# stemangiola/ppcseq

Hardware: AMD Instinct MI355X
Metric: effective samples/sec (whole node) for NB hierarchical fit (higher is better)
Workload: dtype f64; 1 GPU; BASELINE cfg3: synthetic 20000 genes x 200 samples (seed 20253), C=2, K=1000; NUTS (Stan defaults) warm-up 150 + 250 kept draws/chain, 8 chains per GPU (cfg3 names 8 chains; chains are the sharded unit, so N GPUs run 8N chains); mode=chains, chains_total=8, lanes_per_gene=4, loglik_workgroups=939, ess_estimator=rank-normalised split-chain bulk-ESS, min over 6 hyper-parameters and lp__, grad_evals=1471121, divergent_after_warmup=0, round_structure=pipelined: merged log-likelihood / state-machine launch + gene kernel, stream_groups=library default (3 from eight chains on, 2 from four), rounds_last_step_all_groups=115040

## Files before the change

### ppcseq_amd/_lib.py

```python
from __future__ import annotations

import ctypes as C
import os
from dataclasses import dataclass

import numpy as np

_HERE = os.path.dirname(os.path.abspath(__file__))
LIB_PATH = os.environ.get("PPCX_LIB", os.path.join(_HERE, "libppcx.so"))

EXPORTS = [
    "ppcx_version", "ppcx_device_count", "ppcx_last_error", "ppcx_model_create", "ppcx_model_set_exclusions",
    "ppcx_model_set_launch", "ppcx_model_get_launch", "ppcx_model_get_plan", "ppcx_model_dim", "ppcx_model_destroy", "ppcx_log_prob_grad",
    "ppcx_nuts_config_default", "ppcx_fit_nuts", "ppcx_fit_info", "ppcx_fit_from_draws", "ppcx_fit_get_draws", "ppcx_fit_get_columns",
    "ppcx_fit_get_diagnostics", "ppcx_fit_get_timing", "ppcx_fit_get_kernel_times", "ppcx_fit_ppc", "ppcx_fit_free", "ppcx_do_inference_C", "ppcx_model_set_rounds", "ppcx_model_get_rounds", "ppcx_model_set_progress",
    "ppcx_model_create_shard", "ppcx_model_create_shard_strided", "ppcx_fit_nuts_shards", "ppcx_comm_unique_id", "ppcx_comm_create", "ppcx_comm_destroy",
    "ppcx_fit_nuts_comm", "ppcx_advi_config_default", "ppcx_fit_advi", "ppcx_fit_advi_info", "ppcx_fit_advi_iterative",
    "ppcx_guard_decision", "ppcx_device_memory", "ppcx_fit_get_ppc_timing",
    "ppcx_xchg_create", "ppcx_xchg_handle", "ppcx_xchg_connect", "ppcx_xchg_connect_local", "ppcx_xchg_set_timeout", "ppcx_xchg_destroy",
    "ppcx_fit_nuts_xchg", "ppcx_fit_get_xchg_timing", "ppcx_fit_get_inv_metric", "ppcx_fit_summary",
    "ppcx_fit_get_approximation", "ppcx_fit_get_log_ratios", "ppcx_fit_psis", "ppcx_fit_get_log_lik", "ppcx_fit_loo",
    "ppcx_fit_loo_predict", "ppcx_fit_relative_eff", "ppcx_fit_loo_mcse", "ppcx_fit_loo_approx", "ppcx_fit_loo_predict_approx",
]
ABI_VERSION = 400
SUMMARY_FIELDS = ("mean", "sd", "q05", "q50", "q95", "rhat", "ess_bulk", "ess_tail")
LOO_FIELDS = ("elpd_loo", "p_loo", "looic", "khat")
LOO_MCSE_FIELDS = LOO_FIELDS + ("mcse_elpd_loo", "n_eff")
LOO_PREDICT_FIELDS = ("mean", "lower", "upper", "pit_lt", "pit_le", "khat")


class PpcxError(RuntimeError):
    pass


class NutsConfig(C.Structure):
    _fields_ = [("chains", C.c_int), ("iter", C.c_int), ("warmup", C.c_int), ("seed", C.c_ulonglong),
                ("adapt_delta", C.c_double), ("max_treedepth", C.c_int), ("init_radius", C.c_double),
                ("stepsize0", C.c_double), ("init_buffer", C.c_int), ("term_buffer", C.c_int), ("window", C.c_int),
                ("chain_id_offset", C.c_int)]


class AdviConfig(C.Structure):
    _fields_ = [("output_samples", C.c_int), ("iter", C.c_int), ("tol_rel_obj", C.c_double), ("grad_samples", C.c_int),
                ("elbo_samples", C.c_int), ("eval_elbo", C.c_int), ("adapt_iter", C.c_int), ("seed", C.c_ulonglong),
                ("init_radius", C.c_double)]


PROGRESS_FN = C.CFUNCTYPE(C.c_int, C.c_void_p, C.c_int, C.c_int, C.c_int, C.c_longlong, C.c_double)
_lib = None


def use_library(path=None):
    global _lib, LIB_PATH
    _lib = None
    LIB_PATH = path if path else os.environ.get("PPCX_LIB", os.path.join(_HERE, "libppcx.so"))


def load() -> C.CDLL:
    global _lib
    if _lib is not None:
        return _lib
    if not os.path.exists(LIB_PATH):
        raise PpcxError(f"{LIB_PATH} not found: run `python -m ppcseq_amd.build` (hipcc, gfx950) first; "
                        "there is no CPU fallback")
    lib = C.CDLL(LIB_PATH)
    lib.ppcx_version.restype = C.c_int
    if lib.ppcx_version() != ABI_VERSION:
        raise PpcxError(f"{LIB_PATH} has ABI version {lib.ppcx_version()}, this binding needs {ABI_VERSION}: rebuild it "
                        "(`python -m ppcseq_amd.build --force`)")
    dp, ip = C.POINTER(C.c_double), C.POINTER(C.c_int32)
    lib.ppcx_guard_decision.argtypes = [dp, C.c_int]
    lib.ppcx_device_memory.argtypes = [C.c_int, C.POINTER(C.c_ulonglong), C.POINTER(C.c_ulonglong)]
    lib.ppcx_fit_get_ppc_timing.argtypes = [C.c_void_p, dp, C.POINTER(C.c_longlong)]
    lib.ppcx_last_error.restype = C.c_char_p
    lib.ppcx_model_create.argtypes = [C.c_int] * 5 + [ip, dp, dp, C.c_double, C.c_int, ip, C.POINTER(C.c_void_p)]
    lib.ppcx_model_set_exclusions.argtypes = [C.c_void_p, C.c_int, ip]
    lib.ppcx_model_set_launch.argtypes = [C.c_void_p, C.c_int, C.c_int]
    lib.ppcx_model_get_launch.argtypes = [C.c_void_p, C.POINTER(C.c_int), C.POINTER(C.c_int)]
    lib.ppcx_model_get_plan.argtypes = [C.c_void_p, C.c_int, C.POINTER(C.c_int), C.POINTER(C.c_int), C.POINTER(C.c_int32), C.c_int]
    lib.ppcx_model_dim.argtypes = [C.c_void_p]
    lib.ppcx_model_destroy.argtypes = [C.c_void_p]
    lib.ppcx_model_destroy.restype = None
    lib.ppcx_log_prob_grad.argtypes = [C.c_void_p, C.c_int, dp, dp, dp]
    lib.ppcx_nuts_config_default.argtypes = [C.POINTER(NutsConfig)]
    lib.ppcx_nuts_config_default.restype = None
    lib.ppcx_fit_nuts.argtypes = [C.c_void_p, C.POINTER(NutsConfig), C.POINTER(C.c_void_p)]
    lib.ppcx_fit_info.argtypes = [C.c_void_p] + [C.POINTER(C.c_int)] * 4
    lib.ppcx_fit_from_draws.argtypes = [C.c_void_p, C.c_int, C.c_int, dp, C.POINTER(C.c_void_p)]
    lib.ppcx_fit_get_draws.argtypes = [C.c_void_p, dp]
    lib.ppcx_fit_get_columns.argtypes = [C.c_void_p, C.c_int, ip, dp]
    lib.ppcx_fit_summary.argtypes = [C.c_void_p, C.c_int, ip, dp]
    lib.ppcx_fit_get_approximation.argtypes = [C.c_void_p, dp, dp]
    lib.ppcx_fit_get_log_ratios.argtypes = [C.c_void_p, dp, dp]
    lib.ppcx_fit_psis.argtypes = [C.c_void_p, C.c_int, ip, dp]
    lib.ppcx_fit_get_log_lik.argtypes = [C.c_void_p, C.c_int, ip, dp]
    lib.ppcx_fit_loo.argtypes = [C.c_void_p, C.c_int, ip, dp, dp]
    lib.ppcx_fit_loo_mcse.argtypes = [C.c_void_p, C.c_int, ip, dp, dp]
    lib.ppcx_fit_loo_predict.argtypes = [C.c_void_p, C.c_int, ip, dp, C.c_double, C.c_double, C.c_double, C.c_ulonglong, dp]
    lib.ppcx_fit_relative_eff.argtypes = [C.c_void_p, C.c_int, ip, dp]
    lib.ppcx_fit_loo_approx.argtypes = [C.c_void_p, C.c_int, ip, dp]
    lib.ppcx_fit_loo_predict_approx.argtypes = [C.c_void_p, C.c_int, ip, C.c_double, C.c_double, C.c_double, C.c_ulonglong, dp]
    lib.ppcx_fit_get_diagnostics.argtypes = [C.c_void_p, dp, dp, ip, ip, ip, dp]
    lib.ppcx_fit_get_timing.argtypes = [C.c_void_p, dp, C.POINTER(C.c_longlong), dp, C.POINTER(C.c_longlong), dp]
    lib.ppcx_fit_get_kernel_times.argtypes = [C.c_void_p, dp, dp, dp, C.POINTER(C.c_longlong)]
    lib.ppcx_fit_get_inv_metric.argtypes = [C.c_void_p, dp]
    lib.ppcx_fit_ppc.argtypes = [C.c_void_p, C.c_double, C.c_double, C.c_double, C.c_ulonglong, C.c_int, C.c_int, dp, ip]
    lib.ppcx_fit_free.argtypes = [C.c_void_p]
    lib.ppcx_model_set_rounds.argtypes = [C.c_void_p, C.c_int, C.c_int]
    lib.ppcx_xchg_create.argtypes = [C.c_int, C.c_int, C.c_int, C.c_int, C.POINTER(C.c_void_p)]
    lib.ppcx_xchg_handle.argtypes = [C.c_void_p, C.c_char_p]
    lib.ppcx_xchg_connect.argtypes = [C.c_void_p, C.c_char_p]
    lib.ppcx_xchg_connect_local.argtypes = [C.POINTER(C.c_void_p), C.c_int]
    lib.ppcx_xchg_set_timeout.argtypes = [C.c_void_p, C.c_double]
    lib.ppcx_xchg_destroy.argtypes = [C.c_void_p]
    lib.ppcx_xchg_destroy.restype = None
    lib.ppcx_fit_nuts_xchg.argtypes = [C.c_void_p, C.POINTER(NutsConfig), C.c_void_p, C.POINTER(C.c_void_p)]
    lib.ppcx_fit_get_xchg_timing.argtypes = [C.c_void_p, dp, C.POINTER(C.c_longlong)]
    lib.ppcx_model_get_rounds.argtypes = [C.c_void_p, C.c_int, C.POINTER(C.c_int), C.POINTER(C.c_int)]
    lib.ppcx_model_set_progress.argtypes = [C.c_void_p, PROGRESS_FN, C.c_void_p, C.c_double]
    if hasattr(lib, "ppcx_testing_set"):
        lib.ppcx_testing_set.argtypes = [C.c_char_p, C.c_longlong]
        lib.ppcx_testing_set_nccl_provider.argtypes = [C.c_char_p]
        lib.ppcx_testing_bench_kernel.argtypes = [C.c_void_p, C.c_int, C.c_int, C.c_int, C.c_int, C.c_int, dp, C.POINTER(C.c_int)]
    if hasattr(lib, "ppcx_testing_eval_math"):
        lib.ppcx_testing_eval_math.argtypes = [C.c_int, C.c_int, dp, dp, ip, dp, dp]
    if hasattr(lib, "ppcx_testing_get_disp_table"):
        lib.ppcx_testing_get_disp_table.argtypes = [C.c_void_p, dp]
    if hasattr(lib, "ppcx_testing_psis"):
        lib.ppcx_testing_psis.argtypes = [C.c_int, C.c_int, dp, dp, dp]
    if hasattr(lib, "ppcx_testing_loo"):
        lib.ppcx_testing_loo.argtypes = [C.c_int, C.c_int, dp, ip, dp, dp]
    if hasattr(lib, "ppcx_testing_loo_mcse"):
        lib.ppcx_testing_loo_mcse.argtypes = [C.c_int, C.c_int, dp, ip, dp, dp]
    if hasattr(lib, "ppcx_testing_loo_predict"):
        lib.ppcx_testing_loo_predict.argtypes = [dp, ip, C.c_int, C.c_int, ip, ip, dp, C.c_double, C.c_double, dp]
    if hasattr(lib, "ppcx_testing_loo_approx"):
        lib.ppcx_testing_loo_approx.argtypes = [C.c_int, C.c_int, dp, dp, ip, dp]
        lib.ppcx_testing_loo_predict_approx.argtypes = [dp, dp, ip, C.c_int, C.c_int, ip, ip, C.c_double, C.c_double, dp]
    if hasattr(lib, "ppcx_testing_relative_eff"):
        lib.ppcx_testing_relative_eff.argtypes = [C.c_int, C.c_int, C.c_int, dp, dp]
    lib.ppcx_fit_free.restype = None
    lib.ppcx_advi_config_default.argtypes = [C.POINTER(AdviConfig)]
    lib.ppcx_advi_config_default.restype = None
    lib.ppcx_fit_advi.argtypes = [C.c_void_p, C.POINTER(AdviConfig), C.POINTER(C.c_void_p)]
    lib.ppcx_fit_advi_iterative.argtypes = [C.c_void_p, C.POINTER(AdviConfig), C.c_int, C.POINTER(C.c_void_p)]
    lib.ppcx_fit_advi_info.argtypes = [C.c_void_p, C.POINTER(C.c_int), C.POINTER(C.c_int), C.POINTER(C.c_double), C.POINTER(C.c_double)]
    lib.ppcx_model_create_shard.argtypes = [C.c_int] * 7 + [ip, dp, dp, C.c_double, C.c_int, ip, C.POINTER(C.c_void_p)]
    lib.ppcx_model_create_shard_strided.argtypes = [C.c_int] * 8 + [ip, dp, dp, C.c_double, C.c_int, ip, C.POINTER(C.c_void_p)]
    lib.ppcx_fit_nuts_shards.argtypes = [C.POINTER(C.c_void_p), C.c_int, C.POINTER(NutsConfig), C.POINTER(C.c_void_p)]
    lib.ppcx_comm_unique_id.argtypes = [C.c_char_p]
    lib.ppcx_comm_create.argtypes = [C.c_int, C.c_int, C.c_int, C.c_char_p, C.POINTER(C.c_void_p)]
    lib.ppcx_comm_destroy.argtypes = [C.c_void_p]
    lib.ppcx_comm_destroy.restype = None
    lib.ppcx_fit_nuts_comm.argtypes = [C.c_void_p, C.POINTER(NutsConfig), C.c_void_p, C.POINTER(C.c_void_p)]
    _lib = lib
    return lib


def _check(rc: int):
    if rc != 0:
        raise PpcxError(f"ppcx error {rc}: {load().ppcx_last_error().decode()}")


def _p(a, t):
    return a.ctypes.data_as(C.POINTER(t)) if a is not None else None


def testing_set(key: str, value: int):
    lib = load()
    if not hasattr(lib, "ppcx_testing_set"):
        raise PpcxError(f"{LIB_PATH} is not the testing build")
    _check(lib.ppcx_testing_set(key.encode(), int(value)))


def testing_set_nccl_provider(path: str):
    lib = load()
    if not hasattr(lib, "ppcx_testing_set_nccl_provider"):
        raise PpcxError(f"{LIB_PATH} is not the testing build")
    _check(lib.ppcx_testing_set_nccl_provider(path.encode() if path else None))


TESTING_MATH = ("fast_rcp", "fast_log", "fast_exp", "table_log", "window_log", "stirling_tails", "stirling_excess",
                "log_erfc_ratio", "cell", "cell_win", "cell_y", "cell_win_y")


def testing_eval_math(fn: str, a, b=None, y=None):
    lib = load()
    if not hasattr(lib, "ppcx_testing_eval_math"):
        raise PpcxError(f"{LIB_PATH} is not the testing build, or one built before ppcx_testing_math.hip existed: rebuild it "
                        "(`python -m ppcseq_amd.build --testing --force`)")
    a = np.ascontiguousarray(a, dtype=np.float64).ravel()
    n = a.size
    b = np.ascontiguousarray(np.zeros(n) if b is None else np.broadcast_to(b, (n,)), dtype=np.float64)
    y = np.ascontiguousarray(np.zeros(n) if y is None else np.broadcast_to(y, (n,)), dtype=np.int32)
    o0, o1 = np.zeros(n), np.zeros(n)
    rc = lib.ppcx_testing_eval_math(TESTING_MATH.index(fn), n, _p(a, C.c_double), _p(b, C.c_double), _p(y, C.c_int32),
                                    _p(o0, C.c_double), _p(o1, C.c_double))
    if rc != 0:
        raise PpcxError(f"ppcx_testing_eval_math({fn}) failed with code {rc}")
    return o0, o1


def testing_psis(lr, cols=None):
    lib = load()
    if not hasattr(lib, "ppcx_testing_psis"):
        raise PpcxError(f"{LIB_PATH} is not the testing build, or one built before ppcx_testing_psis existed: rebuild it "
                        "(`python -m ppcseq_amd.build --testing --force`)")
    lr = np.ascontiguousarray(lr, dtype=np.float64).ravel()
    n = lr.size
    cols = np.zeros((n, 0)) if cols is None else np.ascontiguousarray(cols, dtype=np.float64).reshape(n, -1)
    out = np.zeros(cols.shape[1] + 1)
    _check(lib.ppcx_testing_psis(n, int(cols.shape[1]), _p(lr, C.c_double), _p(cols, C.c_double) if cols.size else None,
                                 _p(out, C.c_double)))
    return out


def testing_loo(ll, excluded=None, r_eff=None):
    return _testing_loo("ppcx_testing_loo", LOO_FIELDS, ll, excluded, r_eff)


def testing_loo_mcse(ll, excluded=None, r_eff=None):
    return _testing_loo("ppcx_testing_loo_mcse", LOO_MCSE_FIELDS, ll, excluded, r_eff)


def _testing_loo(entry, fields, ll, excluded, r_eff):
    lib = load()
    if not hasattr(lib, entry):
        raise PpcxError(f"{LIB_PATH} is not the testing build, or one built before {entry} existed: rebuild it "
                        "(`python -m ppcseq_amd.build --testing --force`)")
    ll = np.asarray(ll, dtype=np.float64)
    ll = ll.reshape(ll.shape[0], -1)
    n, nc = ll.shape
    cols = np.ascontiguousarray(ll.T)
    ex = None if excluded is None else np.ascontiguousarray(excluded, dtype=np.int32).ravel()
    re = None if r_eff is None else np.ascontiguousarray(r_eff, dtype=np.float64).ravel()
    out = np.zeros((nc, len(fields)))
    _check(getattr(lib, entry)(n, nc, _p(cols, C.c_double), _p(ex, C.c_int32) if ex is not None else None,
                               _p(re, C.c_double) if re is not None else None, _p(out, C.c_double)))
    return out


def testing_loo_predict(ll, x, y, excluded=None, r_eff=None, p_lo=0.025, p_hi=0.975):
    lib = load()
    if not hasattr(lib, "ppcx_testing_loo_predict"):
        raise PpcxError(f"{LIB_PATH} is not the testing build, or one built before ppcx_testing_loo_predict existed: rebuild it "
                        "(`python -m ppcseq_amd.build --testing --force`)")
    ll = np.asarray(ll, dtype=np.float64)
    ll = ll.reshape(ll.shape[0], -1)
    n, nc = ll.shape
    cols = np.ascontiguousarray(ll.T)
    xs = np.ascontiguousarray(np.asarray(x).reshape(n, nc).T, dtype=np.int32)
    ys = np.ascontiguousarray(np.broadcast_to(np.asarray(y), (nc,)), dtype=np.int32)
    ex = None if excluded is None else np.ascontiguousarray(excluded, dtype=np.int32).ravel()
    re = None if r_eff is None else np.ascontiguousarray(r_eff, dtype=np.float64).ravel()
    out = np.zeros((nc, len(LOO_PREDICT_FIELDS)))
    _check(lib.ppcx_testing_loo_predict(_p(cols, C.c_double), _p(xs, C.c_int32), n, nc, _p(ys, C.c_int32),
                                        _p(ex, C.c_int32) if ex is not None else None,
                                        _p(re, C.c_double) if re is not None else None, float(p_lo), float(p_hi),
                                        _p(out, C.c_double)))
    return out


def _testing_approx_columns(entry, ll, log_ratio, excluded):
    lib = load()
    if not hasattr(lib, entry):
        raise PpcxError(f"{LIB_PATH} is not the testing build, or one built before {entry} existed: rebuild it "
                        "(`python -m ppcseq_amd.build --testing --force`)")
    ll = np.asarray(ll, dtype=np.float64)
    ll = ll.reshape(ll.shape[0], -1)
    lr = np.ascontiguousarray(log_ratio, dtype=np.float64).ravel()
    if lr.size != ll.shape[0]:
        raise ValueError("log_ratio must hold one value per draw")
    ex = None if excluded is None else np.ascontiguousarray(excluded, dtype=np.int32).ravel()
    return lib, np.ascontiguousarray(ll.T), lr, ex


def testing_loo_approx(ll, log_ratio, excluded=None):
    lib, cols, lr, ex = _testing_approx_columns("ppcx_testing_loo_approx", ll, log_ratio, excluded)
    nc, n = cols.shape
    out = np.zeros((nc, len(LOO_FIELDS)))
    _check(lib.ppcx_testing_loo_approx(n, nc, _p(cols, C.c_double), _p(lr, C.c_double),
                                       _p(ex, C.c_int32) if ex is not None else None, _p(out, C.c_double)))
    return out


def testing_loo_predict_approx(ll, log_ratio, x, y, excluded=None, p_lo=0.025, p_hi=0.975):
    lib, cols, lr, ex = _testing_approx_columns("ppcx_testing_loo_predict_approx", ll, log_ratio, excluded)
    nc, n = cols.shape
    xs = np.ascontiguousarray(np.asarray(x).reshape(n, nc).T, dtype=np.int32)
    ys = np.ascontiguousarray(np.broadcast_to(np.asarray(y), (nc,)), dtype=np.int32)
    out = np.zeros((nc, len(LOO_PREDICT_FIELDS)))
    _check(lib.ppcx_testing_loo_predict_approx(_p(cols, C.c_double), _p(lr, C.c_double), _p(xs, C.c_int32), n, nc, _p(ys, C.c_int32),
                                               _p(ex, C.c_int32) if ex is not None else None, float(p_lo), float(p_hi),
                                               _p(out, C.c_double)))
    return out


def testing_relative_eff(ll, chains):
    lib = load()
    if not hasattr(lib, "ppcx_testing_relative_eff"):
        raise PpcxError(f"{LIB_PATH} is not the testing build, or one built before ppcx_testing_relative_eff existed: rebuild it "
                        "(`python -m ppcseq_amd.build --testing --force`)")
    ll = np.asarray(ll, dtype=np.float64)
    ll = ll.reshape(ll.shape[0], -1)
    rows, nc = ll.shape
    chains = int(chains)
    if chains < 1 or rows % chains:
        raise ValueError("ll must hold chains * n rows")
    cols = np.ascontiguousarray(ll.T)
    out = np.zeros(nc)
    _check(lib.ppcx_testing_relative_eff(chains, rows // chains, nc, _p(cols, C.c_double), _p(out, C.c_double)))
    return out


def loo_estimates(pointwise, excluded):
    keep = ~np.asarray(excluded, bool)
    out = {}
    for name in LOO_FIELDS[:3]:
        v = np.asarray(pointwise[name], dtype=np.float64)[keep]
        se = float(np.sqrt(v.size * np.var(v, ddof=1))) if v.size > 1 else float("nan")
        out[name] = (float(np.sum(v)), se)
    return out


def device_count() -> int:
    return int(load().ppcx_device_count())


def device_memory(device=0):
    f, t = C.c_ulonglong(), C.c_ulonglong()
    _check(load().ppcx_device_memory(int(device), C.byref(f), C.byref(t)))
    return int(f.value), int(t.value)


def shard_genes(G_total, g0, stride):
    return list(range(int(g0), int(G_total), int(stride)))


class Model:

    def __init__(self, counts, X, exposure_rate, K, lambda_mu_mu=5.612671, excl=None, device=0, shard=None):
        lib = load()
        counts = np.ascontiguousarray(counts, dtype=np.int32)
        if counts.ndim != 2:
            raise ValueError("counts must be G x S")
        self.G, self.S = counts.shape
        X = np.asfortranarray(np.asarray(X, dtype=np.float64).reshape(self.S, -1))
        self.C = X.shape[1]
        self.K = int(K)
        exposure_rate = np.ascontiguousarray(exposure_rate, dtype=np.float64)
        if exposure_rate.shape != (self.S,):
            raise ValueError("exposure_rate must have length S")
        excl = np.ascontiguousarray(excl if excl is not None else np.zeros(0), dtype=np.int32)
        self.X, self.exposure_rate = X, exposure_rate
        self.excl = excl.copy()
        self.counts = counts
        h = C.c_void_p()
        self.shard = shard
        if shard is None:
            _check(lib.ppcx_model_create(int(device), self.G, self.S, self.C, self.K, _p(counts, C.c_int32),
                                         _p(X, C.c_double), _p(exposure_rate, C.c_double), float(lambda_mu_mu),
                                         int(excl.size), _p(excl, C.c_int32), C.byref(h)))
        else:
            if len(shard) == 5:
                Gt, Kt, g0, stride = int(shard[0]), int(shard[1]), int(shard[2]), int(shard[4])
                if len(shard_genes(Gt, g0, stride)) != self.G:
                    raise ValueError("counts must hold exactly the genes of the shard")
                self.K = len([g for g in shard_genes(Gt, g0, stride) if g < Kt])
                _check(lib.ppcx_model_create_shard_strided(int(device), Gt, self.S, self.C, Kt, g0, stride, self.G, _p(counts, C.c_int32),
                                                           _p(X, C.c_double), _p(exposure_rate, C.c_double), float(lambda_mu_mu),
                                                           int(excl.size), _p(excl, C.c_int32), C.byref(h)))
            else:
                Gt, Kt, g0, g1 = (int(v) for v in shard)
                if g1 - g0 != self.G:
                    raise ValueError("counts must hold exactly the genes of the shard")
                self.K = max(0, min(g1, Kt) - min(g0, Kt))
                _check(lib.ppcx_model_create_shard(int(device), Gt, self.S, self.C, Kt, g0, g1, _p(counts, C.c_int32),
                                                   _p(X, C.c_double), _p(exposure_rate, C.c_double), float(lambda_mu_mu),
                                                   int(excl.size), _p(excl, C.c_int32), C.byref(h)))
        self._h = h
        self.D = int(lib.ppcx_model_dim(h))

    def set_exclusions(self, excl):
        excl = np.ascontiguousarray(excl if excl is not None else np.zeros(0), dtype=np.int32)
        _check(load().ppcx_model_set_exclusions(self._h, int(excl.size), _p(excl, C.c_int32)))
        self.excl = excl.copy()

    def set_launch(self, lanes_per_gene=0, workgroups=0):
        _check(load().ppcx_model_set_launch(self._h, int(lanes_per_gene), int(workgroups)))

    def get_plan(self, nchains):
        lanes, nb = C.c_int(), C.c_int()
        _check(load().ppcx_model_get_plan(self._h, int(nchains), C.byref(lanes), C.byref(nb), None, 0))
        b = np.zeros(4 * nb.value + 1, np.int32)
        _check(load().ppcx_model_get_plan(self._h, int(nchains), C.byref(lanes), C.byref(nb), _p(b, C.c_int32), int(b.size)))
        return lanes.value, nb.value, b

    def get_launch(self):
        a, b = C.c_int(), C.c_int()
        _check(load().ppcx_model_get_launch(self._h, C.byref(a), C.byref(b)))
        return a.value, b.value

    def testing_disp_table(self):
        lib = load()
        if not hasattr(lib, "ppcx_testing_get_disp_table"):
            raise PpcxError(f"{LIB_PATH} is not the testing build, or one built before ppcx_testing_get_disp_table existed: "
                            "rebuild it (`python -m ppcseq_amd.build --testing --force`)")
        out = np.zeros((self.G, 32, 2, 12))
        _check(lib.ppcx_testing_get_disp_table(self._h, _p(out, C.c_double)))
        return out

    def log_prob_grad(self, u):
        u = np.ascontiguousarray(u, dtype=np.float64)
        one = u.ndim == 1
        u2 = u.reshape(-1, self.D)
        lp = np.zeros(u2.shape[0])
        g = np.zeros_like(u2)
        _check(load().ppcx_log_prob_grad(self._h, u2.shape[0], _p(u2, C.c_double), _p(lp, C.c_double), _p(g, C.c_double)))
        return (float(lp[0]), g[0]) if one else (lp, g)

    def fit_nuts(self, chains=3, iter=300, warmup=150, seed=1, adapt_delta=0.8, max_treedepth=10, init_radius=2.0,
                 stepsize0=1.0, init_buffer=75, term_buffer=50, window=25, chain_id_offset=0) -> "Fit":
        cfg = NutsConfig(chains, iter, warmup, seed, adapt_delta, max_treedepth, init_radius, stepsize0,
                         init_buffer, term_buffer, window, chain_id_offset)
        h = C.c_void_p()
        _check(load().ppcx_fit_nuts(self._h, C.byref(cfg), C.byref(h)))
        return Fit(self, h)

    def fit_advi(self, output_samples=1000, iter=50000, tol_rel_obj=0.005, elbo_samples=100, eval_elbo=100, adapt_iter=50,
                 seed=1, init_radius=2.0, max_attempts=1) -> "Fit":
        cfg = AdviConfig(output_samples, iter, tol_rel_obj, 1, elbo_samples, eval_elbo, adapt_iter, seed, init_radius)
        h = C.c_void_p()
        if max_attempts > 1:
            _check(load().ppcx_fit_advi_iterative(self._h, C.byref(cfg), int(max_attempts), C.byref(h)))
        else:
            _check(load().ppcx_fit_advi(self._h, C.byref(cfg), C.byref(h)))
        return Fit(self, h)

    def fit_from_draws(self, draws) -> "Fit":
        draws = np.ascontiguousarray(draws, dtype=np.float64)
        if draws.ndim != 3 or draws.shape[2] != self.D:
            raise ValueError("draws must be [chains, n_keep, D]")
        h = C.c_void_p()
        _check(load().ppcx_fit_from_draws(self._h, draws.shape[0], draws.shape[1], _p(draws, C.c_double), C.byref(h)))
        return Fit(self, h)

    def fit_nuts_comm(self, comm: "Comm", **kw) -> "Fit":
        cfg = _make_cfg(**kw)
        h = C.c_void_p()
        _check(load().ppcx_fit_nuts_comm(self._h, C.byref(cfg), comm._h, C.byref(h)))
        return Fit(self, h)

    def fit_nuts_xchg(self, xchg: "Xchg", **kw) -> "Fit":
        cfg = _make_cfg(**kw)
        h = C.c_void_p()
        _check(load().ppcx_fit_nuts_xchg(self._h, C.byref(cfg), xchg._h, C.byref(h)))
        return Fit(self, h)

    def set_rounds(self, pipelined=-2, stream_groups=-1):
        _check(load().ppcx_model_set_rounds(self._h, int(pipelined), int(stream_groups)))

    def set_progress(self, fn=None, every_seconds=1.0):
        self._progress_cb = PROGRESS_FN((lambda user, c0, n, done, rounds, sec: 1 if fn(c0, n, done, rounds, sec) else 0) if fn else 0)
        _check(load().ppcx_model_set_progress(self._h, self._progress_cb, None, float(every_seconds)))

    def get_rounds(self, nchains=1):
        a, b = C.c_int(), C.c_int()
        _check(load().ppcx_model_get_rounds(self._h, int(nchains), C.byref(a), C.byref(b)))
        return bool(a.value), b.value

    def bench_kernel(self, which=0, nchains=1, warm_rounds=40, reps=50, n_merge=1):
        lib = load()
        if not hasattr(lib, "ppcx_testing_bench_kernel"):
            raise PpcxError(f"{LIB_PATH} is not the testing build")
        ms, t = C.c_double(), C.c_int()
        _check(lib.ppcx_testing_bench_kernel(self._h, int(which), nchains, warm_rounds, reps, n_merge, C.byref(ms), C.byref(t)))
        return ms.value, t.value

    def close(self):
        if getattr(self, "_h", None):
            load().ppcx_model_destroy(self._h)
            self._h = None

    def __del__(self):
        try:
            self.close()
        except Exception:
            pass


def _make_cfg(chains=3, iter=300, warmup=150, seed=1, adapt_delta=0.8, max_treedepth=10, init_radius=2.0,
              stepsize0=1.0, init_buffer=75, term_buffer=50, window=25, chain_id_offset=0):
    return NutsConfig(chains, iter, warmup, seed, adapt_delta, max_treedepth, init_radius, stepsize0,
                      init_buffer, term_buffer, window, chain_id_offset)


def fit_nuts_shards(models, **kw):
    cfg = _make_cfg(**kw)
    n = len(models)
    hm = (C.c_void_p * n)(*[m._h for m in models])
    hf = (C.c_void_p * n)()
    _check(load().ppcx_fit_nuts_shards(hm, n, C.byref(cfg), hf))
    return [Fit(m, C.c_void_p(h)) for m, h in zip(models, hf)]


class Comm:

    @staticmethod
    def unique_id() -> bytes:
        buf = C.create_string_buffer(128)
        _check(load().ppcx_comm_unique_id(buf))
        return buf.raw

    def __init__(self, nranks, rank, unique_id: bytes, device=0):
        h = C.c_void_p()
        _check(load().ppcx_comm_create(int(device), int(nranks), int(rank), unique_id, C.byref(h)))
        self._h = h

    def close(self):
        if getattr(self, "_h", None):
            load().ppcx_comm_destroy(self._h)
            self._h = None


class Xchg:

    def __init__(self, nranks, rank, max_chains, device=0):
        h = C.c_void_p()
        _check(load().ppcx_xchg_create(int(device), int(nranks), int(rank), int(max_chains), C.byref(h)))
        self._h, self.nranks, self.rank = h, int(nranks), int(rank)

    def handle(self) -> bytes:
        buf = C.create_string_buffer(64)
        _check(load().ppcx_xchg_handle(self._h, buf))
        return buf.raw

    def connect(self, handles):
        blob = b"".join(handles)
        if len(blob) != 64 * self.nranks:
            raise ValueError("need one 64-byte handle per rank")
        _check(load().ppcx_xchg_connect(self._h, blob))

    @staticmethod
    def local_group(n, max_chains, devices=None):
        xs = [Xchg(n, k, max_chains, device=(devices[k] if devices else 0)) for k in range(n)]
        arr = (C.c_void_p * n)(*[x._h for x in xs])
        _check(load().ppcx_xchg_connect_local(arr, n))
        return xs

    def set_timeout(self, seconds):
        _check(load().ppcx_xchg_set_timeout(self._h, float(seconds)))

    def close(self):
        if getattr(self, "_h", None):
            load().ppcx_xchg_destroy(self._h)
            self._h = None


@dataclass
class Timing:
    seconds: float
    grad_evals: int
    gene_kernel_ms_mean: float
    gene_kernel_samples: int
# ... 201 lines not shown
```

### ppcseq_amd/build.py

```python
from __future__ import annotations

import os
import subprocess
import sys

HERE = os.path.dirname(os.path.abspath(__file__))
CSRC = os.path.join(HERE, "csrc")
LIB = os.path.join(HERE, "libppcx.so")
TESTING_LIB = os.path.join(os.path.dirname(HERE), "tests", "libppcx_testing.so")
SOURCES = ["ppcx_kernels.hip", "ppcx_summary.hip", "ppcx_psis.hip", "ppcx_loo.hip", "ppcx_loo_predict.hip", "ppcx_reff.hip", "ppcx_capi.hip"]
TESTING_SOURCES = ["ppcx_testing_math.hip"]
HEADERS = ["ppcx_math.h", "ppcx_disp.h", "ppcx_model.h", "ppcx_nuts.h", "ppcx_gene.h", "ppcx_kernels.h", "ppcx_summary.h", "ppcx_summary_dev.h", "ppcx_psis.h", "ppcx_psis_dev.h", "ppcx_loo.h", "ppcx_loo_ap.h", "ppcx_loo_dev.h", "ppcx_loo_predict.h", "ppcx_reff.h", "ppcx_block.h", "ppcx_columns.h", "ppcx_testing.h",
           os.path.join("..", "..", "include", "ppcx.h")]


CODEGEN_FLAGS = ["-fno-slp-vectorize"]


def _sources(extra):
    return SOURCES + (TESTING_SOURCES if "-DPPCX_TESTING" in extra else [])


def _stale(lib: str, extra=()) -> bool:
    if not os.path.exists(lib):
        return True
    t = os.path.getmtime(lib)
    return any(os.path.getmtime(os.path.join(CSRC, f)) > t for f in _sources(extra) + HEADERS)


def _compile(lib: str, extra, verbose: bool) -> None:
    hipcc = os.environ.get("HIPCC", "/opt/rocm/bin/hipcc")
    objs = []
    procs = []
    for s in _sources(extra):
        o = lib + "." + s + ".o"
        objs.append(o)
        cmd = [hipcc, "-O3", "-std=c++17", "--offload-arch=gfx950", "-fPIC", "-fvisibility=hidden", "-Wno-unused-result"] + CODEGEN_FLAGS + extra + \
              ["-c", "-o", o, os.path.join(CSRC, s)]
        if verbose:
            print(" ".join(cmd), file=sys.stderr)
        procs.append(subprocess.Popen(cmd))
    for p in procs:
        if p.wait() != 0:
            raise subprocess.CalledProcessError(p.returncode, p.args)
    subprocess.check_call([hipcc, "--offload-arch=gfx950", "-shared", "-fPIC", "-o", lib] + objs)
    for o in objs:
        os.remove(o)


def build(force: bool = False, verbose: bool = False) -> str:
    if force or _stale(LIB):
        _compile(LIB, [], verbose)
    return LIB


def build_testing(force: bool = False, verbose: bool = False) -> str:
    if force or _stale(TESTING_LIB, ["-DPPCX_TESTING"]):
        _compile(TESTING_LIB, ["-DPPCX_TESTING"], verbose)
    return TESTING_LIB


def build_all(force: bool = False, verbose: bool = False):
    import threading
    jobs = []
    if force or _stale(LIB):
        jobs.append((LIB, []))
    if force or _stale(TESTING_LIB, ["-DPPCX_TESTING"]):
        jobs.append((TESTING_LIB, ["-DPPCX_TESTING"]))
    errs = []

    def run(lib, extra):
        try:
            _compile(lib, extra, verbose)
        except Exception as e:
            errs.append(e)
    th = [threading.Thread(target=run, args=j) for j in jobs]
    for t in th:
        t.start()
    for t in th:
        t.join()
    if errs:
        raise errs[0]
    return LIB, TESTING_LIB


if __name__ == "__main__":
    if "--testing" in sys.argv:
        print(*build_all(force="--force" in sys.argv, verbose=True))
    else:
        print(build(force="--force" in sys.argv, verbose=True))
```

### ppcseq_amd/csrc/ppcx_capi.hip

```cpp
#include <hip/hip_runtime.h>
#include <math.h>
#include <stdio.h>
#include <string.h>
#include <algorithm>
#include <chrono>
#include <dlfcn.h>
#include <map>
#include <mutex>
#include <stdlib.h>
#include <string>
#include <thread>
#include <atomic>
#include <vector>
#include "../../include/ppcx.h"
#include "ppcx_kernels.h"
#include "ppcx_summary.h"
#include "ppcx_psis.h"
#include "ppcx_loo.h"
#include "ppcx_columns.h"

using namespace ppcx;

static thread_local std::string g_err;
static int fail(int code, const std::string& msg) { g_err = msg; return code; }
static int hip_fail(hipError_t e, const char* what) { return fail(PPCX_ERR_HIP, std::string(what) + ": " + hipGetErrorString(e)); }
#define HIPCHK(expr)                                                                       \
  do {                                                                                     \
    hipError_t e_ = (expr);                                                                \
    if (e_ != hipSuccess) return hip_fail(e_, #expr);                                      \
  } while (0)

#ifdef PPCX_TESTING
#include "ppcx_testing.h"
struct TestHooks {
  long long fail_at_round = 0; int fail_rank = -1;
  int force_generic = 0;
  int slope_cost_permille = 0;
  int trim_slack_permille = -1;
  int trim_extra_passes = 0;
  int psis_slots = 0;
  long long psis_scratch_bytes = 0;
  long long loo_scratch_bytes = 0;
  std::string rccl_lib;
};
static TestHooks g_test;
#endif

#ifdef PPCX_TRACE
static unsigned long long* g_trace_dev = nullptr;
#endif
struct ppcx_model {
  int device;
  Dims d;
  int CM, L = 64;
  int L_override = 0, wgs_override = 0;
  int n_cu = 256, wgs_per_cu = 4;
  int ls_wgs_per_cu = 0;
  int nblocks_chosen = 0;
  int opt_pipelined = -1, opt_stream_groups = 0;
  ppcx_progress_fn progress = nullptr; void* progress_user = nullptr; double progress_every = 1.0;
  std::vector<char> pos_slope;
  struct Plan { int nbpc = 0; int* d_bounds = nullptr; };
  std::map<std::pair<int, int>, Plan> plans;
  std::mutex plan_mutex;
  std::vector<int32_t> counts_host;
  std::vector<char> excluded_host;
  std::vector<double> X_host, expo_host;
  int* d_counts = nullptr;
  double *d_E = nullptr, *d_expo = nullptr, *d_X = nullptr, *d_Sy = nullptr, *d_SyE = nullptr, *d_SyX = nullptr, *d_SX = nullptr, *d_ncell = nullptr, *d_Lg1 = nullptr;
  double* d_disp = nullptr;
  unsigned char* d_gflags = nullptr;
  DispFit fit;
  double *d_logtab = nullptr, *d_wintab = nullptr;
  double e_min = 1.0, e_max = 1.0;
  int* d_order = nullptr;
  hipStream_t stream = nullptr;
  int live_fits = 0;
  bool destroy_requested = false;
};

struct ppcx_fit {
  ppcx_model* m;
  NutsConfig cfg;
  int chains, n_keep, iter;
  DeviceBuffer<double> d_draws;
  DeviceBuffer<double> d_lp, d_stepsize, d_accept;
  DeviceBuffer<int> d_treedepth, d_nleap, d_div;
  double seconds = 0; long long grad_evals = 0;
  double kA_ms_mean = 0; long long kA_samples = 0; double kA_chain_launches_mean = 0;
  double kC_ms_mean = 0, kU_ms_mean = 0; long long launch_triples = 0;
  double advi_elbo = 0, advi_eta = 0; int advi_converged = 0;
  double ppc_ms = 0; long long ppc_draws = 0;
  long long xchg_ticks = 0, xchg_count = 0;
  std::vector<double> inv_metric;
  bool advi = false;
  DeviceBuffer<double> d_mu, d_omega;
  DeviceBuffer<double> d_log_p, d_log_g, d_r;
};

extern "C" int ppcx_version(void) { return PPCX_VERSION; }
extern "C" int ppcx_device_count(void) { int n = 0; if (hipGetDeviceCount(&n) != hipSuccess) return 0; return n; }
extern "C" const char* ppcx_last_error(void) { return g_err.c_str(); }
extern "C" int ppcx_device_memory(int device, unsigned long long* free_bytes, unsigned long long* total_bytes) {
  int ndev = 0;
  HIPCHK(hipGetDeviceCount(&ndev));
  if (device < 0 || device >= ndev) return fail(PPCX_ERR_ARG, "no such HIP device");
  HIPCHK(hipSetDevice(device));
  size_t f = 0, t = 0;
  HIPCHK(hipMemGetInfo(&f, &t));
  if (free_bytes) *free_bytes = (unsigned long long)f;
  if (total_bytes) *total_bytes = (unsigned long long)t;
  return PPCX_OK;
}

static double pass_cost(const ppcx_model* m, int L, int p, int n) {
  const int S = m->d.S;
  bool slope = false;
  for (int i = p; i < p + n; ++i) slope = slope || m->pos_slope[i];
  double slope_w = m->d.C > 2 ? 1.0 : 1.15;
#ifdef PPCX_TESTING
  if (g_test.slope_cost_permille > 0) slope_w = 1e-3 * g_test.slope_cost_permille;
#endif
  double lin_w = 2.5;
#ifdef PPCX_TESTING
  if (g_test.slope_cost_permille > 0) lin_w = 1e-3 * g_test.slope_cost_permille;
#endif
  const double sweep = (double)((S + L - 1) / L) * (!m->d.x0_is_one ? 2.5 : (slope && !m->d.x1_binary ? lin_w : (slope ? slope_w : 1.0)));
  return 5.8 + sweep;
}
static int resident_workgroups(const ppcx_model* m, int reserve) {
  int n = m->wgs_override > 0 ? m->wgs_override : m->n_cu * (reserve > 0 ? m->ls_wgs_per_cu : m->wgs_per_cu);
  n -= reserve;
  return n < 1 ? 1 : n;
}
constexpr double kTrimSlack = 0.0;
static int workgroups_per_chain(const ppcx_model* m, int L, int nch, int n_res, bool whole_runs = true, bool trim = false) {
  int nbpc = n_res / (nch < 1 ? 1 : nch);
  if (nbpc >= 8 && whole_runs) nbpc = nbpc / 8 * 8;
  if (nbpc < 1) nbpc = 1;
  const int gpw = 64 / L, npass = (m->d.G + gpw - 1) / gpw;
  if (nbpc > (npass + 3) / 4) nbpc = (npass + 3) / 4;
  if (trim) {
    double slack = kTrimSlack;
#ifdef PPCX_TESTING
    if (g_test.trim_slack_permille >= 0) slack = 1e-3 * g_test.trim_slack_permille;
#endif
    int maxp = (npass + 4 * nbpc - 1) / (4 * nbpc);
#ifdef PPCX_TESTING
    maxp += g_test.trim_extra_passes;
#endif
    int nb2 = (int)ceil((double)npass * (1.0 + slack) / (4.0 * maxp));
    if (nb2 >= 8 && whole_runs) nb2 = (nb2 + 7) / 8 * 8;
    if (nb2 < nbpc) nbpc = nb2;
  }
  return nbpc;
}
static int default_stream_groups(int nch) { return nch >= 8 ? 3 : (nch >= 4 ? 2 : 1); }
static int fit_launch_chains(const ppcx_model* m, int nch) {
  int g = default_stream_groups(nch);
  if (m->opt_stream_groups >= 1) g = m->opt_stream_groups < nch ? m->opt_stream_groups : nch;
  return (nch + g - 1) / g;
}
static void choose_launch(ppcx_model* m, int nchains) {
  const int G = m->d.G, S = m->d.S;
  int bestL = 64; double best = 1e300;
  for (int L = 64; L >= 1; L >>= 1) {
    const int gpw = 64 / L;
    const double npass = ceil((double)G / gpw), c_pass = (8.0 + (double)((S + L - 1) / L)) * (L <= 2 ? 1.2 : 1.0);
    const int wpc = 4 * workgroups_per_chain(m, L, nchains, resident_workgroups(m, 0));
    const double t = ceil(npass / wpc) * c_pass;
    if (t < best) { best = t; bestL = L; }
  }
  const int L = m->L_override > 0 ? m->L_override : bestL;
  if (L != m->L) {
    std::lock_guard<std::mutex> lk(m->plan_mutex);
    for (auto& kv : m->plans) (void)hipFree(kv.second.d_bounds);
    m->plans.clear();
    m->L = L;
  }
  m->nblocks_chosen = workgroups_per_chain(m, m->L, nchains, resident_workgroups(m, 0)) * nchains;
}
static void drop_plans(ppcx_model* m) {
  std::lock_guard<std::mutex> lk(m->plan_mutex);
  for (auto& kv : m->plans) (void)hipFree(kv.second.d_bounds);
  m->plans.clear();
}
static int plan_launch(ppcx_model* m, int nch, int reserve, ppcx_model::Plan* out, bool trim = false) {
  std::lock_guard<std::mutex> lk(m->plan_mutex);
  const int n_res = resident_workgroups(m, reserve);
  const auto key = std::make_pair(nch, trim ? -n_res : n_res);
  auto it = m->plans.find(key);
  if (it != m->plans.end()) { *out = it->second; return PPCX_OK; }
  const int G = m->d.G, L = m->L, gpw = 64 / L;
  const int nbpc = workgroups_per_chain(m, L, nch, n_res, reserve == 0, trim), wpc = 4 * nbpc, npass = (G + gpw - 1) / gpw;
  std::vector<double> cost(npass);
  double total = 0;
  for (int k = 0; k < npass; ++k) {
    const int p = k * gpw;
    cost[k] = pass_cost(m, L, p, G - p < gpw ? G - p : gpw);
    total += cost[k];
  }
  std::vector<int> bounds(wpc + 1, G);
  bounds[0] = 0;
  {
    int k = 0; double cum = 0.0;
    for (int j = 1; j < wpc; ++j) {
      const double target = total * (double)j / (double)wpc;
      while (k < npass && cum + 0.5 * cost[k] < target) cum += cost[k++];
      bounds[j] = k * gpw < G ? k * gpw : G;
    }
  }
  {
    const long pmax = ((long)(npass + wpc - 1) / wpc) * gpw;
    for (int j = 0; j < wpc; ++j) if (bounds[j + 1] - bounds[j] > pmax) bounds[j + 1] = (int)(bounds[j] + pmax);
    bounds[wpc] = G;
    for (int j = wpc - 1; j >= 0; --j) if (bounds[j + 1] - bounds[j] > pmax) bounds[j] = (int)(bounds[j + 1] - pmax);
  }
  ppcx_model::Plan pl; pl.nbpc = nbpc;
  HIPCHK(hipMalloc(&pl.d_bounds, sizeof(int) * (size_t)(wpc + 1)));
  HIPCHK(hipMemcpy(pl.d_bounds, bounds.data(), sizeof(int) * (size_t)(wpc + 1), hipMemcpyHostToDevice));
  m->plans[key] = pl;
  *out = pl;
  return PPCX_OK;
}

static int upload_counts(ppcx_model* m, int n_excl, const int32_t* excl) {
  const int G = m->d.G, S = m->d.S, C = m->d.C;
  std::vector<int32_t> cnt(m->counts_host);
  for (int e = 0; e < n_excl; ++e) {
    if (excl[e] < 0 || excl[e] >= G * S) return fail(PPCX_ERR_ARG, "excluded cell id out of range");
    cnt[excl[e]] = -1;
  }
  std::vector<double> Sy(G, 0.0), SyE(G, 0.0), SyX((size_t)C * G, 0.0), SX((size_t)C * G, 0.0), ncell(G, 0.0), Lg1(G, 0.0);
  std::vector<unsigned char> gflags(G, 0);
  for (int g = 0; g < G; ++g) {
    double sy = 0, sye = 0, nc = 0, lg1 = 0;
    for (int s = 0; s < S; ++s) {
      const int y = cnt[(size_t)g * S + s];
      if (y < 0) { gflags[g] |= 1; continue; }
      sy += y; sye += (double)y * m->expo_host[s]; nc += 1.0; lg1 += lgamma((double)y + 1.0);
      for (int c = 0; c < C; ++c) { SyX[(size_t)c * G + g] += (double)y * m->X_host[(size_t)c * S + s]; SX[(size_t)c * G + g] += m->X_host[(size_t)c * S + s]; }
    }
    Sy[g] = sy; SyE[g] = sye; ncell[g] = nc; Lg1[g] = lg1;
  }
  HIPCHK(hipMemcpy(m->d_gflags, gflags.data(), (size_t)G, hipMemcpyHostToDevice));
  {
    std::vector<int> ord(G);
    for (int g = 0; g < G; ++g) ord[g] = g;
    const int K = m->d.K;
    std::stable_sort(ord.begin(), ord.end(), [&](int a, int b) {
      const bool sa = a < K && C >= 2, sb = b < K && C >= 2;
      if (sa != sb) return sa;
      return gflags[a] > gflags[b];
    });
    {
      int ns = 0;
      while (ns < G && ord[ns] < K && C >= 2) ++ns;
      constexpr int kOrderBlock = 16;
      const int nbs = (ns + kOrderBlock - 1) / kOrderBlock, nb = (G + kOrderBlock - 1) / kOrderBlock;
      const bool dear_slopes = m->d.x0_is_one && !m->d.x1_binary;
      if (ns > 0 && ns < G && nbs < nb && dear_slopes) {
        std::vector<int> mixed; mixed.reserve(G);
        int is = 0, ip = ns, sb = 0;
        for (int b = 0; b < nb; ++b) {
          const bool slope_block = sb < nbs && b == (int)((long long)sb * nb / nbs);
          if (slope_block && is < ns) { for (int k = 0; k < kOrderBlock && is < ns; ++k) mixed.push_back(ord[is++]); ++sb; }
          else { for (int k = 0; k < kOrderBlock && ip < G; ++k) mixed.push_back(ord[ip++]); }
        }
        while (is < ns) mixed.push_back(ord[is++]);
        while (ip < G) mixed.push_back(ord[ip++]);
        ord.swap(mixed);
      }
    }
    HIPCHK(hipMemcpy(m->d_order, ord.data(), sizeof(int) * (size_t)G, hipMemcpyHostToDevice));
    m->pos_slope.resize(G);
    for (int p = 0; p < G; ++p) m->pos_slope[p] = ord[p] < K && C >= 2;
    drop_plans(m);
  }
  HIPCHK(hipMemcpy(m->d_counts, cnt.data(), sizeof(int32_t) * cnt.size(), hipMemcpyHostToDevice));
  m->excluded_host.assign(cnt.size(), 0);
  for (size_t i = 0; i < cnt.size(); ++i) m->excluded_host[i] = cnt[i] < 0;
  {
    const hipError_t e = launch_disp_build_kernel(m->d_counts, G, S, nullptr, G, m->fit, m->d_disp, m->stream);
    if (e != hipSuccess) return fail(PPCX_ERR_HIP, std::string("dispersion-table kernel: ") + hipGetErrorString(e));
  }
  HIPCHK(hipMemcpy(m->d_Sy, Sy.data(), sizeof(double) * G, hipMemcpyHostToDevice));
  HIPCHK(hipMemcpy(m->d_SyE, SyE.data(), sizeof(double) * G, hipMemcpyHostToDevice));
  HIPCHK(hipMemcpy(m->d_SyX, SyX.data(), sizeof(double) * SyX.size(), hipMemcpyHostToDevice));
  HIPCHK(hipMemcpy(m->d_SX, SX.data(), sizeof(double) * SX.size(), hipMemcpyHostToDevice));
  HIPCHK(hipMemcpy(m->d_ncell, ncell.data(), sizeof(double) * G, hipMemcpyHostToDevice));
  HIPCHK(hipMemcpy(m->d_Lg1, Lg1.data(), sizeof(double) * G, hipMemcpyHostToDevice));
  HIPCHK(hipStreamSynchronize(m->stream));
  return PPCX_OK;
}

extern "C" int ppcx_model_create(int device, int G, int S, int C, int K, const int32_t* counts, const double* X,
                                 const double* exposure, double lambda_mu_mu, int n_excl, const int32_t* excl,
                                 ppcx_model** out) {
  if (!out) return fail(PPCX_ERR_ARG, "out is NULL");
  *out = nullptr;
  if (G < 1 || S < 1 || C < 1 || K < 0 || K > G) return fail(PPCX_ERR_ARG, "need G>=1, S>=1, C>=1, 0<=K<=G");
  if (C > kMaxC) return fail(PPCX_ERR_LIMIT, "C exceeds the 16 design columns this build supports");
  if ((long long)G * S > 2000000000LL) return fail(PPCX_ERR_LIMIT, "G*S exceeds int32 cell ids");
  if (!counts || !X || !exposure || (n_excl > 0 && !excl)) return fail(PPCX_ERR_ARG, "NULL input buffer");
  for (long long i = 0; i < (long long)G * S; ++i) if (counts[i] < 0) return fail(PPCX_ERR_ARG, "negative count");
  int ndev = 0;
  HIPCHK(hipGetDeviceCount(&ndev));
  if (device < 0 || device >= ndev) return fail(PPCX_ERR_ARG, "no such HIP device");
  HIPCHK(hipSetDevice(device));
  ppcx_model* m = new ppcx_model();
  m->device = device;
  m->d = make_dims(G, S, C, K, lambda_mu_mu);
  m->CM = C <= 2 ? 2 : (C <= 4 ? 4 : (C <= 8 ? 8 : 16));
  {
    hipDeviceProp_t prop;
    HIPCHK(hipGetDeviceProperties(&prop, device));
    m->n_cu = prop.multiProcessorCount > 0 ? prop.multiProcessorCount : 256;
  }
  m->counts_host.assign(counts, counts + (size_t)G * S);
  m->X_host.assign(X, X + (size_t)S * C);
  m->expo_host.assign(exposure, exposure + S);
  int x0 = 1;
  for (int s = 0; s < S; ++s) if (X[s] != 1.0) x0 = 0;
  m->d.x0_is_one = x0;
  int x1b = (C >= 2);
  for (size_t i = (size_t)S; i < (size_t)S * C && x1b; ++i) if (X[i] != 0.0 && X[i] != 1.0) x1b = 0;
#ifdef PPCX_TESTING
  if (g_test.force_generic) x1b = 0;
#endif
  m->d.x1_binary = x1b;
  m->d.raw_consts = (!x0 || (C >= 2 && K > 0 && !x1b)) ? 1 : 0;
  if (C > 8 && (!x0 || (K > 0 && !x1b))) {
    delete m;
    return fail(PPCX_ERR_LIMIT, "more than 8 design columns are supported for designs of a column of ones and 0 / 1 indicator columns only");
  }
  if (const char* e = getenv("PPCX_PIPELINE")) if (atoi(e) == 0) m->opt_pipelined = 0;
  if (const char* e = getenv("PPCX_STREAM_GROUPS")) { const int v = atoi(e); if (v >= 1) m->opt_stream_groups = v; }
  if (loglik_lds_bytes(m->d) > 160u * 1024u) {
    delete m;
    return fail(PPCX_ERR_LIMIT, "the per-sample constants (S * C doubles; S * (2 + C) for a design without a column of ones) do not fit the 160 KB of LDS of a compute unit beside the 20 KB of tables");
  }
  m->wgs_per_cu = loglik_resident_workgroups_per_cu(m->CM, m->d);
  if (m->wgs_per_cu < 1) { delete m; return fail(PPCX_ERR_LIMIT, "the log-likelihood kernel cannot be resident with S * (2 + C) doubles of per-sample constants in LDS"); }
  m->ls_wgs_per_cu = ls_resident_workgroups_per_cu(m->CM, m->d);
  std::vector<double> E(S);
  for (int s = 0; s < S; ++s) E[s] = exp(exposure[s]);
#define MCHK(expr) do { int rc_ = (expr); if (rc_ != PPCX_OK) { ppcx_model_destroy(m); return rc_; } } while (0)
#define MHIP(expr) do { hipError_t e_ = (expr); if (e_ != hipSuccess) { ppcx_model_destroy(m); return fail(PPCX_ERR_HIP, std::string(#expr) + ": " + hipGetErrorString(e_)); } } while (0)
  MHIP(hipStreamCreateWithFlags(&m->stream, hipStreamNonBlocking));
  MHIP(hipMalloc(&m->d_counts, sizeof(int32_t) * ((size_t)G * S + 512)));
  MHIP(hipMemset(m->d_counts, 0, sizeof(int32_t) * ((size_t)G * S + 512)));
  MHIP(hipMalloc(&m->d_E, sizeof(double) * S));
  MHIP(hipMalloc(&m->d_expo, sizeof(double) * S));
  MHIP(hipMalloc(&m->d_X, sizeof(double) * (size_t)S * C));
  MHIP(hipMalloc(&m->d_Sy, sizeof(double) * G));
  MHIP(hipMalloc(&m->d_SyE, sizeof(double) * G));
  MHIP(hipMalloc(&m->d_SyX, sizeof(double) * (size_t)C * G));
  MHIP(hipMalloc(&m->d_SX, sizeof(double) * (size_t)C * G));
  MHIP(hipMalloc(&m->d_ncell, sizeof(double) * G));
  MHIP(hipMalloc(&m->d_disp, sizeof(double) * (size_t)G * kDispGeneDoubles));
  MHIP(hipMalloc(&m->d_gflags, (size_t)G));
  disp_fit_init(m->fit);
  MHIP(hipMalloc(&m->d_Lg1, sizeof(double) * G));
  MHIP(hipMalloc(&m->d_logtab, sizeof(double) * 2 * kLogTabSize));
  { double tab[2 * kLogTabSize]; fill_log_table(tab); MHIP(hipMemcpy(m->d_logtab, tab, sizeof(tab), hipMemcpyHostToDevice)); }
  MHIP(hipMalloc(&m->d_wintab, sizeof(double) * 2 * kWinTabSize));
  { std::vector<double> wt(2 * kWinTabSize); fill_window_log_table(wt.data()); MHIP(hipMemcpy(m->d_wintab, wt.data(), sizeof(double) * wt.size(), hipMemcpyHostToDevice)); }
  m->e_min = m->e_max = E[0];
  for (int s = 1; s < S; ++s) { if (E[s] < m->e_min) m->e_min = E[s]; if (E[s] > m->e_max) m->e_max = E[s]; }
  MHIP(hipMalloc(&m->d_order, sizeof(int) * (size_t)G));
  MHIP(hipMemcpy(m->d_E, E.data(), sizeof(double) * S, hipMemcpyHostToDevice));
  MHIP(hipMemcpy(m->d_expo, exposure, sizeof(double) * S, hipMemcpyHostToDevice));
  MHIP(hipMemcpy(m->d_X, X, sizeof(double) * (size_t)S * C, hipMemcpyHostToDevice));
  MCHK(upload_counts(m, n_excl, excl));
  choose_launch(m, 1);
  *out = m;
  return PPCX_OK;
}

extern "C" int ppcx_model_set_exclusions(ppcx_model* m, int n_excl, const int32_t* excl) {
  if (!m || (n_excl > 0 && !excl) || n_excl < 0) return fail(PPCX_ERR_ARG, "bad arguments");
  HIPCHK(hipSetDevice(m->device));
  return upload_counts(m, n_excl, excl);
}
extern "C" int ppcx_model_set_launch(ppcx_model* m, int lanes_per_gene, int workgroups) {
  if (!m) return fail(PPCX_ERR_ARG, "model is NULL");
  if (lanes_per_gene != 0 && (lanes_per_gene < 1 || lanes_per_gene > 64 || (lanes_per_gene & (lanes_per_gene - 1))))
    return fail(PPCX_ERR_ARG, "lanes_per_gene must be 0 or a power of two <= 64");
  if (workgroups < 0 || workgroups > (1 << 20)) return fail(PPCX_ERR_ARG, "workgroups must be 0 (automatic) or a positive count");
  HIPCHK(hipSetDevice(m->device));
  m->L_override = lanes_per_gene; m->wgs_override = workgroups;
  drop_plans(m);
  choose_launch(m, 1);
  return PPCX_OK;
}
extern "C" int ppcx_model_set_rounds(ppcx_model* m, int pipelined, int stream_groups) {
  if (!m) return fail(PPCX_ERR_ARG, "model is NULL");
  if (pipelined < -2 || pipelined > 1 || stream_groups < -1 || stream_groups > 64) return fail(PPCX_ERR_ARG, "pipelined must be -2 .. 1 and stream_groups -1 .. 64");
  if (pipelined != -2) m->opt_pipelined = pipelined;
  if (stream_groups != -1) m->opt_stream_groups = stream_groups;
  return PPCX_OK;
}
static bool model_pipelines(const ppcx_model* m) {
  return m->opt_pipelined != 0 && m->ls_wgs_per_cu >= 1;
}
extern "C" int ppcx_model_set_progress(ppcx_model* m, ppcx_progress_fn fn, void* user, double every_seconds) {
  if (!m || !(every_seconds >= 0)) return fail(PPCX_ERR_ARG, "bad arguments");
  m->progress = fn; m->progress_user = user; m->progress_every = every_seconds;
  return PPCX_OK;
}
extern "C" int ppcx_model_get_rounds(const ppcx_model* m, int nchains, int* pipelined, int* stream_groups) {
  if (!m || nchains < 1) return fail(PPCX_ERR_ARG, "bad arguments");
  if (pipelined) *pipelined = model_pipelines(m) ? 1 : 0;
  if (stream_groups) {
    int g = default_stream_groups(nchains);
    if (m->opt_stream_groups >= 1) g = m->opt_stream_groups < nchains ? m->opt_stream_groups : nchains;
    *stream_groups = g;
  }
  return PPCX_OK;
}
extern "C" int ppcx_model_get_launch(const ppcx_model* m, int* lanes_per_gene, int* nblocks) {
  if (!m) return fail(PPCX_ERR_ARG, "model is NULL");
  if (lanes_per_gene) *lanes_per_gene = m->L;
  if (nblocks) *nblocks = m->nblocks_chosen;
  return PPCX_OK;
}
extern "C" int ppcx_model_get_plan(ppcx_model* m, int nchains, int* lanes_per_gene, int* workgroups_per_chain, int* bounds, int cap) {
  if (!m || nchains == 0) return fail(PPCX_ERR_ARG, "bad arguments");
  HIPCHK(hipSetDevice(m->device));
  const bool trim = nchains < 0;
  if (trim) nchains = -nchains; else choose_launch(m, nchains);
  ppcx_model::Plan pl;
  const int rc = plan_launch(m, nchains, 0, &pl, trim);
  if (rc != PPCX_OK) return rc;
  if (lanes_per_gene) *lanes_per_gene = m->L;
  if (workgroups_per_chain) *workgroups_per_chain = pl.nbpc;
  if (bounds) {
    const int n = 4 * pl.nbpc + 1;
    if (cap < n) return fail(PPCX_ERR_ARG, "bounds buffer too small");
    HIPCHK(hipMemcpy(bounds, pl.d_bounds, sizeof(int) * (size_t)n, hipMemcpyDeviceToHost));
  }
  return PPCX_OK;
}
extern "C" int ppcx_model_dim(const ppcx_model* m) { return m ? m->d.D : PPCX_ERR_ARG; }
extern "C" void ppcx_model_destroy(ppcx_model* m) {
  if (!m) return;
  if (m->live_fits > 0) { m->destroy_requested = true; return; }
  (void)hipSetDevice(m->device);
  drop_plans(m);
  (void)hipFree(m->d_counts); (void)hipFree(m->d_E); (void)hipFree(m->d_expo); (void)hipFree(m->d_X);
  (void)hipFree(m->d_Sy); (void)hipFree(m->d_SyE); (void)hipFree(m->d_SyX); (void)hipFree(m->d_SX); (void)hipFree(m->d_ncell); (void)hipFree(m->d_disp); (void)hipFree(m->d_gflags); (void)hipFree(m->d_Lg1); (void)hipFree(m->d_logtab); (void)hipFree(m->d_wintab); (void)hipFree(m->d_order);
  if (m->stream) (void)hipStreamDestroy(m->stream);
  delete m;
}

extern "C" void ppcx_nuts_config_default(ppcx_nuts_config* c) {
  if (!c) return;
  c->chains = 3; c->iter = 300; c->warmup = 150; c->seed = 1; c->adapt_delta = 0.8; c->max_treedepth = 10;
  c->init_radius = 2.0; c->stepsize0 = 1.0; c->init_buffer = 75; c->term_buffer = 50; c->window = 25;
  c->chain_id_offset = 0;
}

struct Work {
  double *vecs = nullptr, *hyper_vecs[2] = {nullptr, nullptr}, *partials = nullptr, *t0[2] = {nullptr, nullptr}, *sums = nullptr, *red = nullptr;
  Cmd* cmds[2] = {nullptr, nullptr}; ChainState* states[2] = {nullptr, nullptr}; int* done = nullptr;
  int* done_host = nullptr;
  long Dpad = 0; int nb_update = 1, nb_close = 1; long launches = 0;
  hipStream_t stream = nullptr; bool own_stream = false;
  bool pipelined = false;
  bool shared_chip = false;
  std::atomic<int>* stop = nullptr;
  int *active = nullptr, *active_host = nullptr; int n_active = 0;
  const XchgArgs* xchg = nullptr; int xchg_chain0 = 0;
  ~Work() {
    (void)hipFree(vecs); (void)hipFree(partials); (void)hipFree(done); (void)hipFree(sums); (void)hipFree(red);
    for (int i = 0; i < 2; ++i) { (void)hipFree(hyper_vecs[i]); (void)hipFree(t0[i]); (void)hipFree(cmds[i]); (void)hipFree(states[i]); }
    if (done_host) (void)hipHostFree(done_host);
    (void)hipFree(active); if (active_host) (void)hipHostFree(active_host);
    if (own_stream && stream) (void)hipStreamDestroy(stream);
  }
};

static int work_alloc(Work& w, ppcx_model* m, int nchains) {
  const int D = m->d.D;
  if (!w.stream) w.stream = m->stream;
  w.Dpad = ((long)D + 31) / 32 * 32;
  w.nb_update = (D + 255) / 256;
  if (w.nb_update > 80) w.nb_update = 80;
  if (w.nb_update < 1) w.nb_update = 1;
  HIPCHK(hipMalloc(&w.vecs, sizeof(double) * (size_t)nchains * V_COUNT * w.Dpad));
  w.nb_close = (m->d.G + 255) / 256;
  HIPCHK(hipMalloc(&w.partials, sizeof(double) * (size_t)nchains * w.nb_close * PT_COUNT));
  HIPCHK(hipMalloc(&w.sums, sizeof(double) * (size_t)nchains * (3 + m->CM) * m->d.G));
  HIPCHK(hipMemsetAsync(w.sums, 0, sizeof(double) * (size_t)nchains * (3 + m->CM) * m->d.G, w.stream));
  HIPCHK(hipMalloc(&w.done, sizeof(int) * nchains));
  HIPCHK(hipMalloc(&w.red, sizeof(double) * (size_t)nchains * PT_COUNT));
  HIPCHK(hipMemsetAsync(w.red, 0, sizeof(double) * (size_t)nchains * PT_COUNT, w.stream));
  HIPCHK(hipHostMalloc(&w.done_host, sizeof(int) * 2 * nchains));
  HIPCHK(hipHostMalloc(&w.active_host, sizeof(int) * nchains));
  HIPCHK(hipMalloc(&w.active, sizeof(int) * nchains));
  for (int i = 0; i < 2; ++i) {
    HIPCHK(hipMalloc(&w.hyper_vecs[i], sizeof(double) * (size_t)nchains * V_COUNT * 8));
    HIPCHK(hipMalloc(&w.t0[i], sizeof(double) * (size_t)nchains * w.nb_update));
    HIPCHK(hipMalloc(&w.cmds[i], sizeof(Cmd) * nchains));
    HIPCHK(hipMalloc(&w.states[i], sizeof(ChainState) * nchains));
    HIPCHK(hipMemsetAsync(w.hyper_vecs[i], 0, sizeof(double) * (size_t)nchains * V_COUNT * 8, w.stream));
    HIPCHK(hipMemsetAsync(w.t0[i], 0, sizeof(double) * (size_t)nchains * w.nb_update, w.stream));
    HIPCHK(hipMemsetAsync(w.cmds[i], 0, sizeof(Cmd) * nchains, w.stream));
    HIPCHK(hipMemsetAsync(w.states[i], 0, sizeof(ChainState) * nchains, w.stream));
  }
  HIPCHK(hipMemsetAsync(w.vecs, 0, sizeof(double) * (size_t)nchains * V_COUNT * w.Dpad, w.stream));
  HIPCHK(hipMemsetAsync(w.partials, 0, sizeof(double) * (size_t)nchains * w.nb_close * PT_COUNT, w.stream));
  HIPCHK(hipMemsetAsync(w.done, 0, sizeof(int) * nchains, w.stream));
  for (int c = 0; c < nchains; ++c) {
    HIPCHK(launch_fill_kernel(w.vecs + ((size_t)c * V_COUNT + V_MINV) * w.Dpad, w.Dpad, 1.0, w.stream));
    HIPCHK(launch_fill_kernel(w.hyper_vecs[0] + ((size_t)c * V_COUNT + V_MINV) * 8, 8, 1.0, w.stream));
  }
  w.launches = 0;
  HIPCHK(hipStreamSynchronize(w.stream));
  return PPCX_OK;
}

struct RunIO {
  double* draws = nullptr; long draws_stride = 0; int n_keep = 0, iter = 0;
  double *lp = nullptr, *stepsize = nullptr, *accept = nullptr; int *treedepth = nullptr, *nleap = nullptr, *div = nullptr;
};

static void step_args(ppcx_model* m, Work& w, const RunIO& io, int phases, bool with_update, StepArgs* o) {
  const int in = (int)(w.launches & 1), out = in ^ 1;
  StepArgs& sa = *o;
  sa.d = m->d; sa.phases = phases;
  sa.states_in = w.states[in]; sa.states_out = w.states[out];
  sa.cmds_in = w.cmds[in]; sa.cmds_out = w.cmds[out];
  sa.hyper_in = w.hyper_vecs[in]; sa.hyper_out = w.hyper_vecs[out];
  sa.partials = w.partials; sa.nblocks_close = w.nb_close; sa.slab_stride = w.nb_close; sa.t0 = w.t0[in]; sa.nblocks_update = w.nb_update; sa.red = w.red;
  sa.draws = io.draws; sa.draws_chain_stride = io.draws_stride; sa.n_keep = io.n_keep; sa.iter = io.iter;
  sa.out_lp = io.lp; sa.out_stepsize = io.stepsize; sa.out_treedepth = io.treedepth; sa.out_n_leapfrog = io.nleap;
  sa.out_divergent = io.div; sa.out_accept = io.accept; sa.done = w.done;
  sa.upd_vecs = nullptr; sa.upd_Dpad = 0; sa.upd_t0_out = nullptr;
  sa.x = XchgArgs();
  if (w.xchg) {
    sa.x = *w.xchg;
    sa.x.chain0 = w.xchg_chain0;
  }
  if (with_update && (phases & STEP_ADVANCE)) { sa.upd_vecs = w.vecs; sa.upd_Dpad = w.Dpad; sa.upd_t0_out = w.t0[out]; }
}
static int launch_step(ppcx_model* m, Work& w, int nchains, const RunIO& io, int phases, bool with_update = false) {
  StepArgs sa;
  step_args(m, w, io, phases, with_update, &sa);
  hipError_t e = launch_step_kernel(sa, w.nb_update, nchains, w.stream);
  if (e != hipSuccess) return fail(PPCX_ERR_HIP, std::string("step kernel: ") + hipGetErrorString(e));
  if (phases & STEP_ADVANCE) w.launches++;
  return PPCX_OK;
}
static int launch_update(ppcx_model* m, Work& w, int nchains, const RunIO& io) {
  UpdateArgs ua;
  ua.d = m->d; ua.cmds = w.cmds[w.launches & 1]; ua.vecs = w.vecs; ua.Dpad = w.Dpad;
  ua.draws = io.draws; ua.draws_chain_stride = io.draws_stride; ua.t0_out = w.t0[w.launches & 1];
  hipError_t e = launch_update_kernel(ua, w.nb_update, nchains, w.stream);
  if (e != hipSuccess) return fail(PPCX_ERR_HIP, std::string("update kernel: ") + hipGetErrorString(e));
  return PPCX_OK;
}
static int step_runs(int nchains, int nact) { return (nchains + nact - 1) / nact; }
static int loglik_args(ppcx_model* m, Work& w, int nchains, int reserve, LoglikArgs* out) {
  const int nact = w.n_active > 0 ? w.n_active : nchains;
  ppcx_model::Plan pl;
  int rc = plan_launch(m, nact, reserve, &pl, w.shared_chip);
  if (rc != PPCX_OK) return rc;
  LoglikArgs& la = *out;
  la.d = m->d; la.cd.counts = m->d_counts; la.cd.disp = m->d_disp; la.cd.gflags = m->d_gflags; la.cd.Sy = m->d_Sy; la.cd.ncell = m->d_ncell; la.cd.e_min = m->e_min; la.cd.e_max = m->e_max; la.sampleE = m->d_E; la.exposure = m->d_expo; la.X = m->d_X;
  la.vecs = w.vecs; la.Dpad = w.Dpad; la.cmds = w.cmds[w.launches & 1]; la.sums = w.sums; la.logtab = m->d_logtab; la.wintab = m->d_wintab; la.order = m->d_order;
  la.lgL = 0; while ((1 << la.lgL) < m->L) ++la.lgL;
  la.nchains = nact; la.active = w.n_active > 0 ? w.active : nullptr; la.nbpc = pl.nbpc; la.bounds = pl.d_bounds;
#ifdef PPCX_TRACE
  la.trace = g_trace_dev;
#endif
  return PPCX_OK;
}
static int launch_loglik(ppcx_model* m, Work& w, int nchains) {
  LoglikArgs la;
  int rc = loglik_args(m, w, nchains, 0, &la);
  if (rc != PPCX_OK) return rc;
  hipError_t e = launch_loglik_kernel(m->CM, la, w.stream);
  if (e != hipSuccess) return fail(PPCX_ERR_HIP, std::string("loglik kernel: ") + hipGetErrorString(e));
  return PPCX_OK;
}
static void close_args(ppcx_model* m, Work& w, CloseArgs* o);
static int launch_ls(ppcx_model* m, Work& w, int nchains, const RunIO& io, hipEvent_t ev_start = nullptr, hipEvent_t ev_stop = nullptr) {
  const int nact = w.n_active > 0 ? w.n_active : nchains;
  const int n_srun = step_runs(nchains, nact);
  LoglikArgs la;
  int rc = loglik_args(m, w, nchains, n_srun * nact, &la);
  if (rc != PPCX_OK) return rc;
  StepArgs sa;
  step_args(m, w, io, STEP_REDUCE | STEP_ADVANCE, false, &sa);
  hipError_t e = launch_ls_kernel(m->CM, la, sa, n_srun, nchains, 1, w.stream, ev_start, ev_stop);
  if (e != hipSuccess) return fail(PPCX_ERR_HIP, std::string("merged log-likelihood / step kernel: ") + hipGetErrorString(e));
  w.launches++;
  return PPCX_OK;
}
static int launch_gene_round(ppcx_model* m, Work& w, int nchains, const RunIO& io, int spec = 1) {
  GeneArgs ga;
  close_args(m, w, &ga.c);
  ga.draws = io.draws; ga.draws_chain_stride = io.draws_stride; ga.spec = spec;
  hipError_t e = launch_gene_kernel(m->CM, ga, w.nb_close, nchains, w.stream);
  if (e != hipSuccess) return fail(PPCX_ERR_HIP, std::string("gene kernel: ") + hipGetErrorString(e));
  return PPCX_OK;
}
static void close_args(ppcx_model* m, Work& w, CloseArgs* o) {
  CloseArgs& ca = *o;
  ca.d = m->d; ca.Sy = m->d_Sy; ca.SyE = m->d_SyE; ca.SyX = m->d_SyX; ca.SX = m->d_SX; ca.ncell = m->d_ncell; ca.Lg1 = m->d_Lg1;
  ca.sums = w.sums; ca.vecs = w.vecs; ca.Dpad = w.Dpad; ca.cmds = w.cmds[w.launches & 1]; ca.partials = w.partials;
}
static int launch_close(ppcx_model* m, Work& w, int nchains) {
  CloseArgs ca;
  ca.d = m->d; ca.Sy = m->d_Sy; ca.SyE = m->d_SyE; ca.SyX = m->d_SyX; ca.SX = m->d_SX; ca.ncell = m->d_ncell; ca.Lg1 = m->d_Lg1;
  ca.sums = w.sums; ca.vecs = w.vecs; ca.Dpad = w.Dpad; ca.cmds = w.cmds[w.launches & 1]; ca.partials = w.partials;
  hipError_t e = launch_close_kernel(m->CM, ca, w.nb_close, nchains, w.stream);
  if (e != hipSuccess) return fail(PPCX_ERR_HIP, std::string("close kernel: ") + hipGetErrorString(e));
  return PPCX_OK;
}
static int launch_gene(ppcx_model* m, Work& w, int nchains) {
  int rc = launch_loglik(m, w, nchains);
  return rc != PPCX_OK ? rc : launch_close(m, w, nchains);
}
static ChainState* current_states(Work& w) { return w.states[w.launches & 1]; }
static double* current_hyper(Work& w) { return w.hyper_vecs[w.launches & 1]; }

struct PumpStats { double kA_ms_sum = 0, kC_ms_sum = 0, kU_ms_sum = 0; long long kA_samples = 0; double chain_launches = 0; long long pairs = 0; };

typedef struct ncclComm* ncclComm_t;
typedef struct { char internal[128]; } ncclUniqueId_t;
struct RcclApi {
  void* h = nullptr;
  int (*GetUniqueId)(ncclUniqueId_t*) = nullptr;
  int (*CommInitRank)(ncclComm_t*, int, ncclUniqueId_t, int) = nullptr;
  int (*CommDestroy)(ncclComm_t) = nullptr;
  int (*AllReduce)(const void*, void*, size_t, int, int, ncclComm_t, hipStream_t) = nullptr;
  const char* (*GetErrorString)(int) = nullptr;
};
static RcclApi g_rccl;
static int rccl_load() {
  if (g_rccl.h) return PPCX_OK;
#ifdef PPCX_TESTING
  if (!g_test.rccl_lib.empty()) {
    g_rccl.h = dlopen(g_test.rccl_lib.c_str(), RTLD_NOW | RTLD_LOCAL);
    if (!g_rccl.h) return fail(PPCX_ERR_HIP, std::string("cannot load the nccl provider ") + g_test.rccl_lib + ": " + dlerror());
  }
#endif
  if (!g_rccl.h) {
    const char* names[] = {"librccl.so.1", "librccl.so", "/opt/rocm/lib/librccl.so.1"};
    for (const char* n : names) { g_rccl.h = dlopen(n, RTLD_NOW | RTLD_GLOBAL); if (g_rccl.h) break; }
  }
  if (!g_rccl.h) return fail(PPCX_ERR_HIP, "cannot load librccl.so");
  g_rccl.GetUniqueId = (int (*)(ncclUniqueId_t*))dlsym(g_rccl.h, "ncclGetUniqueId");
  g_rccl.CommInitRank = (int (*)(ncclComm_t*, int, ncclUniqueId_t, int))dlsym(g_rccl.h, "ncclCommInitRank");
  g_rccl.CommDestroy = (int (*)(ncclComm_t))dlsym(g_rccl.h, "ncclCommDestroy");
  g_rccl.AllReduce = (int (*)(const void*, void*, size_t, int, int, ncclComm_t, hipStream_t))dlsym(g_rccl.h, "ncclAllReduce");
  g_rccl.GetErrorString = (const char* (*)(int))dlsym(g_rccl.h, "ncclGetErrorString");
  if (!g_rccl.GetUniqueId || !g_rccl.CommInitRank || !g_rccl.CommDestroy || !g_rccl.AllReduce) return fail(PPCX_ERR_HIP, "librccl.so lacks the expected symbols");
  return PPCX_OK;
}
struct ppcx_comm { ncclComm_t comm = nullptr; int nranks = 1, rank = 0, device = 0; double* d_guard = nullptr; double* h_guard = nullptr; };
static int guard_decision(const double* g, int local_rc);
static int comm_guard(ppcx_comm* c, hipStream_t st, long long pairs, int n_done, int local_rc, int* all_rc) {
  double* v = c->h_guard;
  v[0] = (double)pairs; v[1] = -(double)pairs; v[2] = (double)n_done; v[3] = -(double)n_done; v[4] = local_rc != PPCX_OK ? (double)(-local_rc) : 0.0;
  const std::string local_msg = g_err;
  hipError_t he = hipMemcpyAsync(c->d_guard, v, sizeof(double) * 5, hipMemcpyHostToDevice, st);
  const int e = g_rccl.AllReduce(c->d_guard, c->d_guard, 5,  8,  2, c->comm, st);
  if (e != 0) return fail(PPCX_ERR_HIP, std::string("ncclAllReduce (guard): ") + (g_rccl.GetErrorString ? g_rccl.GetErrorString(e) : "error"));
  if (he == hipSuccess) he = hipMemcpyAsync(c->h_guard + 8, c->d_guard, sizeof(double) * 5, hipMemcpyDeviceToHost, st);
  if (he == hipSuccess) he = hipStreamSynchronize(st);
  if (he != hipSuccess) return fail(PPCX_ERR_HIP, std::string("guard exchange: ") + hipGetErrorString(he));
  const int d = guard_decision(c->h_guard + 8, local_rc);
  *all_rc = d;
  if (d != PPCX_OK) {
    if (local_rc != PPCX_OK) g_err = local_msg;
    else if (d == PPCX_ERR_STALL) g_err = "the ranks of the gene-sharded run disagree on the rounds issued or the chains finished";
    else g_err = "another rank of the gene-sharded run reported an error";
  }
  return PPCX_OK;
}

struct Shard { ppcx_model* m; Work* w; RunIO io; };

static int guard_decision(const double* g, int local_rc) {
  if (g[4] != 0.0) return local_rc != PPCX_OK ? local_rc : -(int)g[4];
  if (g[0] != -g[1] || g[2] != -g[3]) return PPCX_ERR_STALL;
  return PPCX_OK;
}
extern "C" int ppcx_guard_decision(const double* reduced5, int local_rc) { return reduced5 ? guard_decision(reduced5, local_rc) : PPCX_ERR_ARG; }

static int pump(std::vector<Shard>& sh, int nchains, ppcx_comm* comm, long long max_pairs, bool time_kernels,
                PumpStats* stats) {
  const int ns = (int)sh.size();
  hipStream_t st = sh[0].w->stream;
  int rc = PPCX_OK;
  const bool guarded = comm && comm->comm && comm->nranks > 1;
  const bool piped = ns == 1 && !(comm && comm->comm) && sh[0].w->pipelined;
  int local_rc = PPCX_OK;
#define PUMP_TRY(expr) do { if (local_rc == PPCX_OK) { const int r_ = (expr); if (r_ != PPCX_OK) { if (!guarded) return r_; local_rc = r_; } } } while (0)
#define PUMP_HIP(expr) do { if (local_rc == PPCX_OK) { const hipError_t e_ = (expr); if (e_ != hipSuccess) { const int r_ = fail(PPCX_ERR_HIP, std::string(#expr) + ": " + hipGetErrorString(e_)); if (!guarded) return r_; local_rc = r_; } } } while (0)
  if (!piped) for (int k = 0; k < ns; ++k) {
    PUMP_TRY(launch_step(sh[k].m, *sh[k].w, nchains, sh[k].io, STEP_REDUCE | STEP_ADVANCE));
    PUMP_TRY(launch_update(sh[k].m, *sh[k].w, nchains, sh[k].io));
  }
  const int batch = 32, sample_every = 16;
  struct Events {
    hipEvent_t e[6] = {nullptr, nullptr, nullptr, nullptr, nullptr, nullptr};
    ~Events() { for (hipEvent_t x : e) if (x) (void)hipEventDestroy(x); }
  } evs;
  if (time_kernels) for (int i = 0; i < 4; ++i) if (hipEventCreate(&evs.e[i]) != hipSuccess) { evs.e[i] = nullptr; time_kernels = false; }
  hipEvent_t &ev0 = evs.e[0], &ev1 = evs.e[1], &ev2 = evs.e[2], &ev3 = evs.e[3];
  bool lookahead = piped && !guarded;
  if (lookahead) for (int i = 4; i < 6; ++i) if (hipEventCreateWithFlags(&evs.e[i], hipEventDisableTiming) != hipSuccess) { evs.e[i] = nullptr; lookahead = false; }
  long long pairs = 0; int n_done = 0, n_done_applied = 0;
  const auto t_start = std::chrono::steady_clock::now(); auto t_report = t_start;
  Work& w0 = *sh[0].w;
  int cur = 0; bool have_prev = false, sampled_prev = false;
  while (true) {
    bool sampled = false;
    for (int i = 0; i < batch; ++i, ++pairs) {
// ... 47 lines not shown
    }
    if (sampled_chk && n_done == 0 && local_rc == PPCX_OK) {
      float ms = 0;
      if (hipEventElapsedTime(&ms, ev0, ev1) == hipSuccess) {
        stats->kA_ms_sum += ms; stats->kA_samples++; stats->chain_launches += nchains;
        if (hipEventElapsedTime(&ms, ev1, ev2) == hipSuccess) stats->kC_ms_sum += ms;
        if (hipEventElapsedTime(&ms, ev2, ev3) == hipSuccess) stats->kU_ms_sum += ms;
      }
    }
    n_done = 0;
    rc = local_rc;
    if (local_rc == PPCX_OK) for (int c = 0; c < nchains; ++c) {
      if (flags[c]) ++n_done;
      if (flags[c] == 2) rc = fail(PPCX_ERR_INIT, "no finite initial point after 100 attempts");
      if (flags[c] == 3) rc = fail(PPCX_ERR_STEPSIZE, "step-size heuristic diverged");
      if (flags[c] == 5) rc = fail(PPCX_ERR_STALL, "gene-shard exchange: a peer rank left the fit or did not arrive within the timeout");
    }
    if (pairs > max_pairs && n_done < nchains && rc == PPCX_OK) rc = fail(PPCX_ERR_STALL, "launch budget exhausted before the chains finished");
    if (guarded) {
      int all_rc = PPCX_OK;
      const int grc = comm_guard(comm, st, pairs, n_done, rc, &all_rc);
      if (grc != PPCX_OK) return grc;
      if (all_rc != PPCX_OK) { rc = all_rc; break; }
    } else if (rc != PPCX_OK) break;
    if (sh[0].m->progress && local_rc == PPCX_OK) {
      const auto now = std::chrono::steady_clock::now();
      if (std::chrono::duration<double>(now - t_report).count() >= sh[0].m->progress_every || n_done == nchains) {
        t_report = now;
        const int stop = sh[0].m->progress(sh[0].m->progress_user, sh[0].w->xchg_chain0, nchains, n_done, pairs, std::chrono::duration<double>(now - t_start).count());
        if (stop != 0 && n_done < nchains) {
          local_rc = fail(PPCX_ERR_CANCELLED, "the progress callback ended the fit");
          if (w0.stop) w0.stop->store(1);
          if (!guarded) { rc = local_rc; break; }
        }
      }
    }
    if (w0.stop && w0.stop->load() && local_rc == PPCX_OK && n_done < nchains) {
      local_rc = fail(PPCX_ERR_CANCELLED, "the progress callback ended the fit");
      if (!guarded) { rc = local_rc; break; }
    }
    if (n_done == nchains) break;
    if (n_done > n_done_applied) {
      if (lookahead) {
        PUMP_HIP(hipStreamSynchronize(st));
        flags = w0.done_host + cur * nchains;
        have_prev = false;
      }
      int na = 0;
      for (int c = 0; c < nchains; ++c) if (!flags[c]) w0.active_host[na++] = c;
      n_done_applied = nchains - na;
      if (na == 0) { n_done = nchains; break; }
      for (int k = 0; k < ns; ++k) {
        Work& wk = *sh[k].w;
        PUMP_HIP(hipMemcpyAsync(wk.active, w0.active_host, sizeof(int) * na, hipMemcpyHostToDevice, st));
        wk.n_active = na;
      }
      PUMP_HIP(hipStreamSynchronize(st));
    }
    if (lookahead) cur ^= 1;
  }
  if (lookahead) (void)hipStreamSynchronize(st);
#undef PUMP_TRY
#undef PUMP_HIP
  stats->pairs = pairs;
  return rc;
}
static int pump(ppcx_model* m, Work& w, int nchains, const RunIO& io, long long max_pairs, bool time_kernels,
                PumpStats* stats, ppcx_comm* comm = nullptr) {
  std::vector<Shard> sh(1);
  sh[0].m = m; sh[0].w = &w; sh[0].io = io;
  return pump(sh, nchains, comm, max_pairs, time_kernels, stats);
}

extern "C" int ppcx_log_prob_grad(ppcx_model* m, int n_points, const double* u, double* lp, double* grad) {
  if (!m || n_points < 1 || !u || !lp) return fail(PPCX_ERR_ARG, "bad arguments");
  HIPCHK(hipSetDevice(m->device));
  const int D = m->d.D;
  const int maxb = 256;
  for (int p0 = 0; p0 < n_points; p0 += maxb) {
    const int nb = n_points - p0 < maxb ? n_points - p0 : maxb;
    choose_launch(m, nb);
    Work w;
    int rc = work_alloc(w, m, nb);
    if (rc != PPCX_OK) return rc;
    std::vector<ChainState> states(nb);
    NutsConfig cfg; memset(&cfg, 0, sizeof cfg);
    cfg.chains = nb; cfg.iter = 0; cfg.warmup = 0; cfg.seed = 0; cfg.adapt_delta = 0.8; cfg.max_treedepth = 10;
    cfg.init_radius = 2; cfg.stepsize0 = 1; cfg.init_buffer = 75; cfg.term_buffer = 50; cfg.window = 25; cfg.chain_id_offset = 0;
    for (int c = 0; c < nb; ++c) state_init(states[c], cfg, c, 1);
    HIPCHK(hipMemcpyAsync(w.states[0], states.data(), sizeof(ChainState) * nb, hipMemcpyHostToDevice, m->stream));
    std::vector<double> hq((size_t)nb * V_COUNT * 8, 0.0);
    for (int c = 0; c < nb; ++c) {
      const double* uc = u + (size_t)(p0 + c) * D;
      HIPCHK(hipMemcpyAsync(w.vecs + ((size_t)c * V_COUNT + V_Q1) * w.Dpad, uc, sizeof(double) * D, hipMemcpyHostToDevice, m->stream));
      for (int k = 0; k < 6; ++k) hq[((size_t)c * V_COUNT + V_Q1) * 8 + k] = uc[hyper_index(m->d, k)];
      for (int k = 0; k < 8; ++k) hq[((size_t)c * V_COUNT + V_MINV) * 8 + k] = 1.0;
    }
    HIPCHK(hipMemcpyAsync(w.hyper_vecs[0], hq.data(), sizeof(double) * hq.size(), hipMemcpyHostToDevice, m->stream));
    RunIO io;
    PumpStats ps;
    rc = pump(m, w, nb, io, 64, false, &ps);
    if (rc != PPCX_OK) return rc;
    HIPCHK(hipMemcpy(states.data(), current_states(w), sizeof(ChainState) * nb, hipMemcpyDeviceToHost));
    HIPCHK(hipMemcpy(hq.data(), current_hyper(w), sizeof(double) * hq.size(), hipMemcpyDeviceToHost));
    for (int c = 0; c < nb; ++c) {
      lp[p0 + c] = states[c].sc.lp_eval;
      if (grad) {
        double* gc = grad + (size_t)(p0 + c) * D;
        HIPCHK(hipMemcpy(gc, w.vecs + ((size_t)c * V_COUNT + V_G1) * w.Dpad, sizeof(double) * D, hipMemcpyDeviceToHost));
        for (int k = 0; k < 6; ++k) gc[hyper_index(m->d, k)] = hq[((size_t)c * V_COUNT + V_G1) * 8 + k];
      }
    }
  }
  return PPCX_OK;
}

#ifdef PPCX_TESTING
extern "C" int ppcx_testing_set(const char* key, long long value) {
  if (!key) return fail(PPCX_ERR_ARG, "key is NULL");
  const std::string k(key);
  if (k == "fail_at_round") g_test.fail_at_round = value;
  else if (k == "fail_rank") g_test.fail_rank = (int)value;
  else if (k == "force_generic") g_test.force_generic = (int)value;
  else if (k == "slope_cost_permille") g_test.slope_cost_permille = (int)value;
  else if (k == "trim_slack_permille") g_test.trim_slack_permille = (int)value;
  else if (k == "trim_extra_passes") g_test.trim_extra_passes = (int)value;
  else if (k == "psis_slots") g_test.psis_slots = (int)value;
  else if (k == "psis_scratch_bytes") g_test.psis_scratch_bytes = value;
  else if (k == "loo_scratch_bytes") g_test.loo_scratch_bytes = value;
  else return fail(PPCX_ERR_ARG, "unknown test hook " + k);
  return PPCX_OK;
}
extern "C" int ppcx_testing_set_nccl_provider(const char* path) {
  if (g_rccl.h) return fail(PPCX_ERR_ARG, "the nccl entry points are bound already");
  g_test.rccl_lib = path ? path : "";
  return PPCX_OK;
}
static std::mutex g_sm_mutex; static long long g_sm_ticks[6] = {0, 0, 0, 0, 0, 0}; static long long g_sm_rounds = 0;
extern "C" int ppcx_testing_sm_trace(double* out6) {
  std::lock_guard<std::mutex> lk(g_sm_mutex);
  for (int k = 0; k < 5; ++k) out6[k] = g_sm_rounds ? 1e-2 * (double)g_sm_ticks[k] / (double)g_sm_rounds : 0.0;
  out6[5] = (double)g_sm_rounds;
  for (int k = 0; k < 6; ++k) g_sm_ticks[k] = 0;
  g_sm_rounds = 0;
  return PPCX_OK;
}
extern "C" int ppcx_testing_get_disp_table(ppcx_model* m, double* out) {
  if (!m || !out) return fail(PPCX_ERR_ARG, "bad arguments");
  HIPCHK(hipSetDevice(m->device));
  HIPCHK(hipStreamSynchronize(m->stream));
  HIPCHK(hipMemcpy(out, m->d_disp, sizeof(double) * (size_t)m->d.G * kDispGeneDoubles, hipMemcpyDeviceToHost));
  return PPCX_OK;
}
extern "C" int ppcx_testing_bench_kernel(ppcx_model* m, int which, int nchains, int warm_rounds, int reps, int n_merge,
                                         double* ms_per_launch, int* cmd_type) {
  if (!m || nchains < 1 || reps < 1 || !ms_per_launch || which < 0 || which > PPCX_BENCH_GENE_NEW_TRANSITION) return fail(PPCX_ERR_ARG, "bad arguments");
  HIPCHK(hipSetDevice(m->device));
  choose_launch(m, nchains);
  Work w;
  int rc = work_alloc(w, m, nchains);
  if (rc != PPCX_OK) return rc;
  NutsConfig nc; memset(&nc, 0, sizeof nc);
  nc.chains = nchains; nc.iter = 1000000; nc.warmup = 1000000; nc.seed = 1; nc.adapt_delta = 0.8; nc.max_treedepth = 10;
  nc.init_radius = 2; nc.stepsize0 = 1; nc.init_buffer = 75; nc.term_buffer = 50; nc.window = 25;
  std::vector<ChainState> states(nchains);
  for (int c = 0; c < nchains; ++c) state_init(states[c], nc, c, 0);
  HIPCHK(hipMemcpyAsync(w.states[0], states.data(), sizeof(ChainState) * nchains, hipMemcpyHostToDevice, m->stream));
  RunIO io; io.iter = nc.iter;
  hipStream_t st = m->stream;
  if ((rc = launch_step(m, w, nchains, io, STEP_REDUCE | STEP_ADVANCE)) != PPCX_OK) return rc;
  if ((rc = launch_update(m, w, nchains, io)) != PPCX_OK) return rc;
  for (int i = 0; i < warm_rounds; ++i) {
    if ((rc = launch_gene(m, w, nchains)) != PPCX_OK) return rc;
    if ((rc = launch_step(m, w, nchains, io, STEP_REDUCE | STEP_ADVANCE)) != PPCX_OK) return rc;
    if ((rc = launch_update(m, w, nchains, io)) != PPCX_OK) return rc;
  }
  HIPCHK(hipStreamSynchronize(st));
  Cmd* dcmds = w.cmds[w.launches & 1];
  std::vector<Cmd> cmds(nchains);
  HIPCHK(hipMemcpy(cmds.data(), dcmds, sizeof(Cmd) * nchains, hipMemcpyDeviceToHost));
  if (cmd_type) *cmd_type = cmds[0].type;
  if (n_merge >= 0) for (int c = 0; c < nchains; ++c) {
    if (which >= PPCX_BENCH_GENE && cmds[c].type == CMD_EPS_TRY) { cmds[c].type = CMD_LEAF; cmds[c].pre_dir = cmds[c].dir; cmds[c].next_dir = cmds[c].dir; cmds[c].leaf_n = 1; }
    if (cmds[c].type != CMD_LEAF) continue;
    cmds[c].n_merge = n_merge; cmds[c].subtree_complete = 0;
    cmds[c].eps *= 1e-3;
  }
  if (which >= PPCX_BENCH_GENE) for (int c = 0; c < nchains; ++c) {
    cmds[c].evaluated = 1; cmds[c].updated = 0;
    if (cmds[c].type == CMD_LEAF) { cmds[c].pre_flags = PRE_PROP; cmds[c].prop_slot = n_merge >= 0 ? n_merge : 0; cmds[c].prop_src = -1; }
    if (which == PPCX_BENCH_GENE_NEW_TRANSITION && cmds[c].type == CMD_LEAF) { cmds[c].pre_flags = PRE_NEW_TRANSITION | PRE_SAVE_NEAR; cmds[c].rng_c1 = 7; }
    if (which == PPCX_BENCH_GENE_NO_PROP) cmds[c].pre_flags &= ~PRE_PROP;
    if (which == PPCX_BENCH_GENE_UPDATE_ONLY) cmds[c].evaluated = 0;
  }
  HIPCHK(hipMemcpy(dcmds, cmds.data(), sizeof(Cmd) * nchains, hipMemcpyHostToDevice));
  auto one = [&]() -> int {
    switch (which) {
      case PPCX_BENCH_CLOSE: return launch_close(m, w, nchains);
      case PPCX_BENCH_LOGLIK_CLOSE: return launch_gene(m, w, nchains);
      case PPCX_BENCH_STEP: return launch_step(m, w, nchains, io, STEP_REDUCE | STEP_ADVANCE);
      case PPCX_BENCH_UPDATE: return launch_update(m, w, nchains, io);
      case PPCX_BENCH_STEP_REDUCE: return launch_step(m, w, nchains, io, STEP_REDUCE);
      case PPCX_BENCH_STEP_ADVANCE: return launch_step(m, w, nchains, io, STEP_ADVANCE);
      case PPCX_BENCH_STEP_UPDATE: return launch_step(m, w, nchains, io, STEP_REDUCE | STEP_ADVANCE, true);
      case PPCX_BENCH_GENE: case PPCX_BENCH_GENE_NO_PROP: case PPCX_BENCH_GENE_UPDATE_ONLY: case PPCX_BENCH_GENE_NEW_TRANSITION:
        return launch_gene_round(m, w, nchains, io);
      case PPCX_BENCH_GENE_NO_SPEC: return launch_gene_round(m, w, nchains, io, 0);
      default: return launch_loglik(m, w, nchains);
    }
  };
  struct Ev { hipEvent_t e0 = nullptr, e1 = nullptr; ~Ev() { if (e0) (void)hipEventDestroy(e0); if (e1) (void)hipEventDestroy(e1); } } ev;
  HIPCHK(hipEventCreate(&ev.e0)); HIPCHK(hipEventCreate(&ev.e1));
  for (int i = 0; i < 3; ++i) if ((rc = launch_gene(m, w, nchains)) != PPCX_OK) return rc;
  HIPCHK(hipEventRecord(ev.e0, st));
  for (int i = 0; i < reps; ++i) if ((rc = one()) != PPCX_OK) return rc;
  HIPCHK(hipEventRecord(ev.e1, st));
  HIPCHK(hipStreamSynchronize(st));
  float ms = 0; HIPCHK(hipEventElapsedTime(&ms, ev.e0, ev.e1));
  *ms_per_launch = (double)ms / reps;
#ifdef PPCX_TRACE
  if (const char* path = getenv("PPCX_TRACE_FILE")) {
    const size_t n = (size_t)kTraceBlocks * 4 * kTracePasses * kTraceStamps;
    HIPCHK(hipMalloc(&g_trace_dev, sizeof(unsigned long long) * n));
    HIPCHK(hipMemset(g_trace_dev, 0, sizeof(unsigned long long) * n));
    rc = one();
    HIPCHK(hipStreamSynchronize(st));
    std::vector<unsigned long long> h(n);
    HIPCHK(hipMemcpy(h.data(), g_trace_dev, sizeof(unsigned long long) * n, hipMemcpyDeviceToHost));
    (void)hipFree(g_trace_dev); g_trace_dev = nullptr;
    if (FILE* f = fopen(path, "wb")) { fwrite(h.data(), sizeof(unsigned long long), n, f); fclose(f); }
    if (rc != PPCX_OK) return rc;
  }
#endif
  return PPCX_OK;
}
#endif

static void fit_attach(ppcx_fit* f, ppcx_model* m) { f->m = m; m->live_fits++; }
extern "C" void ppcx_fit_free(ppcx_fit* f) {
  if (!f) return;
  ppcx_model* m = f->m;
  (void)hipSetDevice(m->device);
  delete f;
  if (--m->live_fits == 0 && m->destroy_requested) ppcx_model_destroy(m);
}

struct ppcx_xchg {
  int device = 0, nranks = 1, rank = 0, max_chains = 0;
  void* local = nullptr; size_t bytes = 0;
  void* peer[kMaxRanks] = {};
  bool opened[kMaxRanks] = {};
  bool connected = false;
  unsigned epoch = 0;
  double timeout_s = 20.0;
  std::mutex* mu = nullptr;
};
static size_t xchg_bytes(int nranks, int max_chains) { return sizeof(double) * xchg_recv_doubles(nranks, max_chains) + sizeof(unsigned long long) * xchg_flag_words(nranks, max_chains); }
extern "C" int ppcx_xchg_create(int device, int nranks, int rank, int max_chains, ppcx_xchg** out) {
  if (!out || nranks < 1 || nranks > kMaxRanks || rank < 0 || rank >= nranks || max_chains < 1 || max_chains > 1024)
    return fail(PPCX_ERR_ARG, "need 1 <= nranks <= 16, 0 <= rank < nranks, 1 <= max_chains <= 1024");
  *out = nullptr;
  HIPCHK(hipSetDevice(device));
  ppcx_xchg* x = new ppcx_xchg();
  x->device = device; x->nranks = nranks; x->rank = rank; x->max_chains = max_chains; x->bytes = xchg_bytes(nranks, max_chains);
  hipError_t e = hipExtMallocWithFlags(&x->local, x->bytes, hipDeviceMallocUncached);
  if (e == hipSuccess) e = hipMemset(x->local, 0, x->bytes);
  if (e == hipSuccess) e = hipDeviceSynchronize();
  if (e != hipSuccess) { (void)hipFree(x->local); delete x; return fail(PPCX_ERR_HIP, std::string("exchange buffer: ") + hipGetErrorString(e)); }
  x->peer[rank] = x->local;
  if (nranks == 1) x->connected = true;
  *out = x;
  return PPCX_OK;
}
extern "C" int ppcx_xchg_handle(ppcx_xchg* x, char* out64) {
  if (!x || !out64) return fail(PPCX_ERR_ARG, "NULL argument");
  HIPCHK(hipSetDevice(x->device));
  hipIpcMemHandle_t h;
  HIPCHK(hipIpcGetMemHandle(&h, x->local));
  static_assert(sizeof(h) == 64, "hipIpcMemHandle_t is 64 bytes");
  memcpy(out64, &h, 64);
  return PPCX_OK;
}
extern "C" int ppcx_xchg_connect(ppcx_xchg* x, const char* handles) {
  if (!x || !handles) return fail(PPCX_ERR_ARG, "NULL argument");
  if (x->connected) return fail(PPCX_ERR_ARG, "the exchange group is connected already");
  HIPCHK(hipSetDevice(x->device));
  for (int k = 0; k < x->nranks; ++k) {
    if (k == x->rank) continue;
    hipIpcMemHandle_t h; memcpy(&h, handles + (size_t)k * 64, 64);
    void* p = nullptr;
    hipError_t e = hipIpcOpenMemHandle(&p, h, hipIpcMemLazyEnablePeerAccess);
    if (e != hipSuccess) return fail(PPCX_ERR_HIP, "hipIpcOpenMemHandle (rank " + std::to_string(k) + "): " + hipGetErrorString(e));
    x->peer[k] = p; x->opened[k] = true;
  }
  x->connected = true;
  return PPCX_OK;
}
extern "C" int ppcx_xchg_connect_local(ppcx_xchg** group, int n) {
  if (!group || n < 1 || n > kMaxRanks) return fail(PPCX_ERR_ARG, "bad group");
  for (int k = 0; k < n; ++k) if (!group[k] || group[k]->nranks != n || group[k]->rank != k || group[k]->connected || group[k]->max_chains != group[0]->max_chains)
    return fail(PPCX_ERR_ARG, "group[k] must be the unconnected rank k of n, all with the same max_chains");
  for (int k = 0; k < n; ++k) {
    for (int j = 0; j < n; ++j) {
      if (group[k]->device != group[j]->device) {
        (void)hipSetDevice(group[k]->device);
        hipError_t e = hipDeviceEnablePeerAccess(group[j]->device, 0);
// ... 1043 lines not shown
```

### ppcseq_amd/csrc/ppcx_gene.h

```cpp
#pragma once
#include "ppcx_nuts.h"


namespace ppcx {

template <int CM>
struct GeneCtx {
  static constexpr int NCM = CM + 1;
  int gg, ncoord;
  bool active, has_slopes, fast, two;
  int idx[NCM];
  double q[NCM];
  GeneParams<CM> gp;
};

PPCX_HD void coord_consts(const Dims& d, const VecRef& v, int i, double q) {
  if (i >= d.off_sigma_raw && i < d.off_tail) {
    v.at(V_C0, i) = fast_exp(-q); v.at(V_C2, i) = q;
  } else if (i >= d.off_intercept && i < d.off_sigma_raw) {
    v.at(V_C0, i) = fast_exp(q);
    if (d.raw_consts) v.at(V_C2, i) = q;
  }
}

template <int CM>
PPCX_HD void gene_index(const Dims& d, int g, GeneCtx<CM>& x) {
  constexpr int NCM = CM + 1;
  x.active = g < d.G;
  x.gg = x.active ? g : 0;
  const int C = d.C;
  const int nslope = x.gg < d.K ? (C - 1 > 1 ? C - 1 : 1) : 0;
  x.ncoord = x.active ? 2 + nslope : 0;
#pragma unroll
  for (int j = 0; j < NCM; ++j)
    x.idx[j] = j == 0 ? d.off_intercept + x.gg : (j == 1 ? d.off_sigma_raw + x.gg : coef_index(d, j - 1, x.gg));
  x.has_slopes = x.active && x.gg < d.K && C >= 2;
  x.two = x.has_slopes && d.x0_is_one && d.x1_binary;
  x.fast = d.x0_is_one && (!x.has_slopes || x.two);
}
template <int CM>
PPCX_HD void gene_params(const Dims& d, const VecRef& v, GeneCtx<CM>& x) {
  x.gp.coef[0] = x.q[0];
#pragma unroll
  for (int cc = 1; cc < CM; ++cc) x.gp.coef[cc] = (x.has_slopes && cc < d.C) ? x.q[cc + 1] : 0.0;
  x.gp.sigma_raw = x.q[1];
  x.gp.phi = x.active ? v.at(V_C0, x.idx[1]) : 1.0;
  x.gp.invphi = 0.0;
}
template <int CM>
PPCX_HD void gene_load(const Dims& d, const Cmd& c, const VecRef& v, int g, GeneCtx<CM>& x) {
  constexpr int NCM = CM + 1;
  gene_index<CM>(d, g, x);
#pragma unroll
  for (int j = 0; j < NCM; ++j) x.q[j] = j < x.ncoord ? v.at(V_Q0 + 3 * c.dir, x.idx[j]) : 0.0;
  gene_params<CM>(d, v, x);
}

struct CellData {
  const int* counts;
  const double* disp;
  const unsigned char* gflags;
  const double* Sy;
  const double* ncell;
  double e_min, e_max;
};

struct GenePre { double phi, sigma, a0, Sy, n; int flags; };
PPCX_HD GenePre gene_pre_load(const Dims& d, const VecRef& v, const CellData& m, int g) {
  GenePre r;
  r.phi = v.at(V_C0, d.off_sigma_raw + g);
  r.sigma = v.at(V_C2, d.off_sigma_raw + g);
  r.a0 = v.at(V_C0, d.off_intercept + g);
  r.Sy = m.Sy[g]; r.n = m.ncell[g]; r.flags = m.gflags[g];
  return r;
}
template <int L> struct DispDeal {
  static constexpr int NL = L >= 8 ? 4 : (L >= 4 ? 2 : 1);
  static constexpr int CH = kDispStride / NL;
};

template <int CM, int L, int MODE, bool MASKED, bool WIN>
PPCX_HD void sweep_cells(int S, const int* row, const double* sE, const double* sX1, int sub, double A, double A1, double one,
                         const GeneParams<CM>& gp, const double* tab, CellAcc<CM>& acc, const double* ec = nullptr, int C = 2) {
  const int nmin = S / L;
  const int nlane = nmin + (sub < S - nmin * L ? 1 : 0);
  const int* p = row + sub;
  const double* q = sE + sub;
  const double* qx = sX1 + sub;
  int y0 = p[0], y1 = p[L], y2 = p[2 * L], y3 = p[3 * L];
  int k = 0;
#define PPCX_SWEEP_CELL(Y, E, XB, OFF, COND)                                                    \
  if ((COND) && (!MASKED || (Y) >= 0)) {                                                        \
    if (MODE == 1) { const double a1_ = (XB) != 0.0 ? A1 : A;                                   \
                     const double rho_ = WIN ? cell_eval_win<CM, true>(Y, E, a1_, one, gp, tab, acc) : cell_eval<CM, true>(Y, E, a1_, gp, tab, acc); \
                     acc.Tx[1] = fma(XB, rho_, acc.Tx[1]); }                                    \
    else if (MODE == 2) {                                                                       \
      double a_ = (XB) != 0.0 ? A1 : A; double xk_[CM];                                         \
      _Pragma("unroll") for (int cc = 2; cc < CM; ++cc) { xk_[cc] = cc < C ? qx[(cc - 1) * S + (OFF)] : 0.0; a_ = xk_[cc] != 0.0 ? a_ * ec[cc] : a_; } \
      const double rho_ = WIN ? cell_eval_win<CM, true>(Y, E, a_, one, gp, tab, acc) : cell_eval<CM, true>(Y, E, a_, gp, tab, acc); \
      acc.Tx[1] = fma(XB, rho_, acc.Tx[1]);                                                     \
      _Pragma("unroll") for (int cc = 2; cc < CM; ++cc) acc.Tx[cc] = fma(xk_[cc], rho_, acc.Tx[cc]); \
    }                                                                                           \
    else if (MODE == 3) {                                                                       \
      double t_ = (XB) * ec[1]; double xk_[CM];                                                 \
      _Pragma("unroll") for (int cc = 2; cc < CM; ++cc) { xk_[cc] = cc < C ? qx[(cc - 1) * S + (OFF)] : 0.0; t_ = fma(xk_[cc], ec[cc], t_); } \
      const double rho_ = cell_eval<CM, true>(Y, E, A * fast_exp(t_), gp, tab, acc);           \
      acc.Tx[1] = fma(XB, rho_, acc.Tx[1]);                                                     \
      _Pragma("unroll") for (int cc = 2; cc < CM; ++cc) acc.Tx[cc] = fma(xk_[cc], rho_, acc.Tx[cc]); \
    }                                                                                           \
    else if (WIN) (void)cell_eval_win<CM, false>(Y, E, A, one, gp, tab, acc);                   \
    else (void)cell_eval<CM, false>(Y, E, A, gp, tab, acc);                                     \
  }
  for (; k + 4 <= nmin; k += 4) {
    const double e0 = q[0], e1 = q[L], e2 = q[2 * L], e3 = q[3 * L];
    double x0 = 0.0, x1 = 0.0, x2 = 0.0, x3 = 0.0;
    if (MODE != 0) { x0 = qx[0]; x1 = qx[L]; x2 = qx[2 * L]; x3 = qx[3 * L]; }
    p += 4 * L; q += 4 * L; qx += 4 * L;
    const int n0 = p[0], n1 = p[L], n2 = p[2 * L], n3 = p[3 * L];
    if (MODE == 0 && !MASKED && WIN) {
      CellMidWin c0, c1, c2, c3;
      (void)cell_front_win<CM, false>(y0, e0, A, one, gp, tab, acc, c0);
      (void)cell_front_win<CM, false>(y1, e1, A, one, gp, tab, acc, c1);
      (void)cell_front_win<CM, false>(y2, e2, A, one, gp, tab, acc, c2);
      (void)cell_front_win<CM, false>(y3, e3, A, one, gp, tab, acc, c3);
#if defined(__HIP_DEVICE_COMPILE__)
      __builtin_amdgcn_sched_barrier(0);
#endif
      cell_back_win<CM>(c0, acc); cell_back_win<CM>(c1, acc); cell_back_win<CM>(c2, acc); cell_back_win<CM>(c3, acc);
    } else if (MODE == 0 && !MASKED) {
      CellMid c0, c1, c2, c3;
      (void)cell_front<CM, false>(y0, e0, A, gp, tab, acc, c0);
      (void)cell_front<CM, false>(y1, e1, A, gp, tab, acc, c1);
      (void)cell_front<CM, false>(y2, e2, A, gp, tab, acc, c2);
      (void)cell_front<CM, false>(y3, e3, A, gp, tab, acc, c3);
#if defined(__HIP_DEVICE_COMPILE__)
      __builtin_amdgcn_sched_barrier(0);
#endif
      cell_back<CM>(c0, acc); cell_back<CM>(c1, acc); cell_back<CM>(c2, acc); cell_back<CM>(c3, acc);
    } else {
      PPCX_SWEEP_CELL(y0, e0, x0, -4 * L, true)
      PPCX_SWEEP_CELL(y1, e1, x1, -3 * L, true)
      PPCX_SWEEP_CELL(y2, e2, x2, -2 * L, true)
      PPCX_SWEEP_CELL(y3, e3, x3, -L, true)
    }
    y0 = n0; y1 = n1; y2 = n2; y3 = n3;
  }
  if (k < nlane) {
    const double e0 = q[0], e1 = q[L], e2 = q[2 * L], e3 = q[3 * L];
    double x0 = 0.0, x1 = 0.0, x2 = 0.0, x3 = 0.0;
    if (MODE != 0) { x0 = qx[0]; x1 = qx[L]; x2 = qx[2 * L]; x3 = qx[3 * L]; }
    PPCX_SWEEP_CELL(y0, e0, x0, 0, true)
    PPCX_SWEEP_CELL(y1, e1, x1, L, k + 1 < nlane)
    PPCX_SWEEP_CELL(y2, e2, x2, 2 * L, k + 2 < nlane)
    PPCX_SWEEP_CELL(y3, e3, x3, 3 * L, k + 3 < nlane)
  }
#undef PPCX_SWEEP_CELL
}

template <int CM, int L>
PPCX_HD void generic_cells(const Dims& d, const Cmd& c, const VecRef& v, int g, bool has_slopes, const int* row,
                           const double* sExpo, const double* sX, int sub, GeneParams<CM>& gp, const double* tab,
                           CellAcc<CM>& acc) {
  const int S = d.S, C = d.C;
  gp.coef[0] = v.at(V_C2, d.off_intercept + g);
#pragma unroll
  for (int cc = 1; cc < CM; ++cc) gp.coef[cc] = (has_slopes && cc < C) ? v.at(V_C2, coef_index(d, cc, g)) : 0.0;
  (void)c;
  for (int s = sub; s < S; s += L) {
    const int y = row[s];
    if (y >= 0) {
      double t = sExpo[s] + gp.sigma_raw;
#pragma unroll
      for (int cc = 0; cc < CM; ++cc) if (cc < C) t += sX[cc * S + s] * gp.coef[cc];
      const double u = fast_exp(t);
      const double rho = cell_eval<CM, true>(y, u, 1.0, gp, tab, acc);
#pragma unroll
      for (int cc = 0; cc < CM; ++cc) if (cc < C) acc.Tx[cc] = fma(sX[cc * S + s], rho, acc.Tx[cc]);
    }
  }
}

template <int CM, int L, int GEN = 3>
PPCX_HD void lane_gene_sums(const Dims& d, const Cmd& c, const VecRef& v, const CellData& m, int g, const GenePre& pre, int sub,
                            const double* sE, const double* sExpo, const double* sX, const double* tab, const double* wtab,
                            GeneSumsV<CM>& o
#ifdef PPCX_TRACE
                            , unsigned long long* trace_stamps = nullptr
#endif
                            ) {
#if defined(PPCX_TRACE) && defined(__HIP_DEVICE_COMPILE__)
#define PPCX_GSTAMP(k) do { if (trace_stamps) trace_stamps[k] = __builtin_readcyclecounter(); } while (0)
#else
#define PPCX_GSTAMP(k) ((void)0)
#endif
  const int S = d.S;
  const bool has_slopes = g < d.K && d.C >= 2;
  const bool two = has_slopes && d.x0_is_one && d.x1_binary;
  const bool lin = (GEN & 1) && d.x0_is_one && has_slopes && !two;
  const bool generic = (GEN & 2) && !d.x0_is_one;
  GeneParams<CM> gp;
  gp.phi = pre.phi;
  const double sigma = pre.sigma;
  gp.sigma_raw = sigma;
  gp.invphi = fast_rcp(gp.phi);
  const double A = pre.a0 * gp.invphi;
  const bool masked = (pre.flags & 1) != 0;
  const int* row = m.counts + (long)g * S;
  constexpr int NL = DispDeal<L>::NL, CH = DispDeal<L>::CH;
  const DispRef dr = disp_ref(sigma);
  const int fn = L == 1 ? 0 : sub / NL, jch = L == 1 ? 0 : sub - fn * NL;
  const bool tab_lane = dr.in && (L == 1 || fn < 2);
  const double* pc = m.disp + (((long)g * kDispPanels + dr.panel) * 2 + (fn & 1)) * kDispStride + jch * CH;
  double cf[CH], cf2[L == 1 ? CH : 1];
#pragma unroll
  for (int k = 0; k < CH; ++k) cf[k] = 0.0;
  cf2[0] = 0.0;
  if (tab_lane) {
#pragma unroll
    for (int k = 0; k < CH; ++k) cf[k] = pc[k];
    if (L == 1) {
#pragma unroll
      for (int k = 0; k < CH; ++k) cf2[k] = pc[kDispStride + k];
    }
  }
  CellAcc<CM> acc; acc.zero();
  PPCX_GSTAMP(5);
  if (GEN & 2) {
// ... 313 lines not shown
```

### ppcseq_amd/csrc/ppcx_kernels.h

```cpp
#pragma once
#include <hip/hip_runtime.h>
#include "ppcx_gene.h"

namespace ppcx {

constexpr int kLdsPad = 256;
struct LoglikArgs {
  Dims d;
  CellData cd;
  const double* sampleE;
  const double* exposure;
  const double* X;
  double* vecs;
  long Dpad;
  const Cmd* cmds;
  double* sums;
  const double* logtab;
  const double* wintab;
  const int* order;
  int lgL;
  int nchains;
  const int* active;
  int nbpc;
  const int* bounds;
#ifdef PPCX_TRACE
  unsigned long long* trace;
#endif
};
#ifdef PPCX_TRACE
constexpr int kTraceBlocks = 64, kTracePasses = 8, kTraceStamps = 8;
#endif

struct CloseArgs {
  Dims d;
  const double* Sy;
  const double* SyE;
  const double* SyX;
  const double* SX;
  const double* ncell;
  const double* Lg1;
  const double* sums;
  double* vecs; long Dpad;
  const Cmd* cmds;
  double* partials;
};

struct GeneArgs {
  CloseArgs c;
  double* draws; long draws_chain_stride;
  int spec;
};

constexpr int kMaxRanks = 16;
struct XchgArgs {
  int nranks = 1, rank = 0, max_chains = 0;
  int chain0 = 0;
  unsigned epoch = 0;
  long long timeout_ticks = 0;
  double* recv[kMaxRanks];
  unsigned long long* flags[kMaxRanks];
};
PPCX_HD long xchg_recv_index(const XchgArgs& x, int slot, int src, int chain) { return (((long)slot * x.nranks + src) * x.max_chains + x.chain0 + chain) * PT_COUNT; }
PPCX_HD long xchg_flag_index(const XchgArgs& x, int slot, int src, int chain) { return ((long)slot * x.nranks + src) * x.max_chains + x.chain0 + chain; }
PPCX_HD long xchg_abort_index(const XchgArgs& x, int src) { return 2L * x.nranks * x.max_chains + src; }
PPCX_HD size_t xchg_recv_doubles(int nranks, int max_chains) { return (size_t)2 * nranks * max_chains * PT_COUNT; }
PPCX_HD size_t xchg_flag_words(int nranks, int max_chains) { return (size_t)2 * nranks * max_chains + nranks; }

enum StepPhase : int { STEP_REDUCE = 1, STEP_ADVANCE = 2 };
struct StepArgs {
  Dims d;
  int phases;
  const ChainState* states_in; ChainState* states_out;
  const Cmd* cmds_in; Cmd* cmds_out;
  const double* hyper_in; double* hyper_out;
  const double* partials; int nblocks_close;
  int slab_stride;
  const double* t0; int nblocks_update;
  double* red;
  double* draws; long draws_chain_stride;
  int n_keep, iter;
  double* out_lp; double* out_stepsize; int* out_treedepth; int* out_n_leapfrog; int* out_divergent; double* out_accept;
  int* done;
  double* upd_vecs; long upd_Dpad; double* upd_t0_out;
  XchgArgs x;
};

constexpr int kMaxShards = 16;
struct ShardSumArgs { double* bufs[kMaxShards]; int n_shards; int n; };

struct UpdateArgs {
  Dims d;
  const Cmd* cmds;
  double* vecs; long Dpad;
  double* draws; long draws_chain_stride;
  double* t0_out;
};

enum AdviOp : int { ADVI_DRAW = 0, ADVI_RESET = 1, ADVI_STEP = 2 };
struct AdviArgs {
  Dims d;
  double* vecs; long Dpad;
  double* hyper;
  Cmd* cmds;
  const double* red;
  int op, n_slots, first_iter;
  double eta_scaled;
  uint32_t k0, prev_draw, draw_base;
  double* out_draws; int out_row0;
  double* omega_part;
};
struct AdviElboArgs { Dims d; const Cmd* cmds; const double* red; int n_slots; double* acc; const double* omega_part; int n_omega_parts; };

struct PpcArgs {
  Dims d;
  const double* draws;
  long n_draws;
  const double* exposure; const double* X;
  double truncation_compensation, p_lo, p_hi;
  uint32_t k0;
  int n_gen, resample, n_cells;
  double* ci;
  int* counts_rng;
  int* scratch;
};

hipError_t launch_loglik_kernel(int CM, const LoglikArgs& a, hipStream_t st);
int loglik_resident_workgroups_per_cu(int CM, const Dims& d);
size_t loglik_lds_bytes(const Dims& d);
hipError_t launch_close_kernel(int CM, const CloseArgs& a, int nblocks, int nchains, hipStream_t st);
hipError_t launch_ls_kernel(int CM, const LoglikArgs& a, const StepArgs& sa, int n_srun, int n_chains_total, int spec, hipStream_t st,
                            hipEvent_t ev_start = nullptr, hipEvent_t ev_stop = nullptr);
int ls_resident_workgroups_per_cu(int CM, const Dims& d);
hipError_t launch_gene_kernel(int CM, const GeneArgs& a, int nblocks, int nchains, hipStream_t st);
hipError_t launch_step_kernel(const StepArgs& a, int nblocks, int nchains, hipStream_t st);
hipError_t launch_sum_shards_kernel(const ShardSumArgs& a, hipStream_t st);
hipError_t launch_update_kernel(const UpdateArgs& a, int nblocks, int nchains, hipStream_t st);
hipError_t launch_advi_kernel(const AdviArgs& a, int nblocks, hipStream_t st);
hipError_t launch_advi_elbo_kernel(const AdviElboArgs& a, hipStream_t st);
hipError_t launch_ppc_kernel(const PpcArgs& a, const double* T, int nblocks, hipStream_t st);
size_t ppc_wave_lds_bytes(int n_gen);
int ppc_wave_max_draws();
hipError_t launch_ppc_table_kernel(const double* draws, long n_draws, const Dims& d, double tc, double* T, hipStream_t st);
hipError_t launch_ppc_wave_kernel(const PpcArgs& a, const double* T, int nblocks, hipStream_t st);
hipError_t launch_disp_build_kernel(const int* counts, int G, int S, const int* genes, int n_genes, const DispFit& fit, double* table, hipStream_t st);
hipError_t launch_gather_kernel(const double* draws, long n_rows, int D, const int* cols, int n_cols, double* out, hipStream_t st);
hipError_t launch_fill_kernel(double* p, long n, double val, hipStream_t st);

constexpr int kSummaryLdsDraws = 8192;
constexpr int kSummaryMaxChains = 128;
struct SummaryArgs {
  const double* x;
  int n_cols, M, n;
  int npad;
  double* out;
  double* scratch; long slice;
};
int summary_npad(int M, int n);
long summary_slice_doubles(int M, int n);
size_t summary_lds_bytes(int M, int n);
hipError_t launch_summary_gather_kernel(const double* draws, const double* lp, long rows, int D, const int* cols, int n_cols, double* out, hipStream_t st);
hipError_t launch_summary_kernel(const SummaryArgs& a, int nblocks, hipStream_t st);
constexpr size_t kSummaryScratchBytes = (size_t)256 << 20;
hipError_t summary_columns(const double* draws, const double* lp, int M, int n, int D, int n_cols, const int* cols, double* out,
                           size_t scratch_bytes, hipStream_t st);

constexpr int kPsisLdsDraws = 4096;
constexpr int kPsisMaxSel = 4096;
constexpr size_t kPsisScratchBytes = (size_t)256 << 20;
struct PsisArgs {
  double* x;
  const double* r;
  const int* cols;
  int n_cols; long n;
  int sel_pad;
  double* out;
};
int psis_sel_pad(long n);
hipError_t launch_psis_approx_kernel(const Dims& d, const double* sq, const double* sg, const double* hyper, double* mu, double* omega,
                                     hipStream_t st);
hipError_t launch_psis_stage_kernel(const Dims& d, const double* draws, long row0, int n_slots, double* vecs, long Dpad, Cmd* cmds,
                                    hipStream_t st);
hipError_t launch_psis_record_kernel(const Dims& d, const Cmd* cmds, const double* red, int n_slots, double* log_p, hipStream_t st);
hipError_t launch_psis_log_g_kernel(const double* draws, long rows, int D, const double* mu, const double* omega, const double* log_p,
                                    double* log_g, double* r, hipStream_t st);
hipError_t launch_psis_kernel(const PsisArgs& a, hipStream_t st);
hipError_t psis_columns(const double* draws, const double* r, long n, int D, int n_cols, const int* cols, double* khat,
                        size_t scratch_bytes, hipStream_t st);
struct LooArgs {
  const double* T = nullptr;
  const int* y = nullptr;
  const double* expo = nullptr;
  const double* X = nullptr;
  int S = 1, C = 1;
  const double* cols = nullptr;
  const int* excl = nullptr;
  const double* r_eff = nullptr;
  const double* lr = nullptr;
  long n = 0;
  int cell0 = 0, n_cells = 0;
  double* scratch = nullptr;
  int sel_pad = 0;
  double* out = nullptr;
};
int loo_sel_pad(long n, double r_eff_min);
hipError_t launch_loo_table_kernel(const double* draws, long n_draws, const Dims& d, const int* genes, int n_genes, double* T,
                                   hipStream_t st);
struct FitCells {
  const double* draws = nullptr;
  long n = 0;
  int chains = 0, n_keep = 0;
  Dims d{};
  const double* expo = nullptr;
  const double* X = nullptr;
  int n_genes = 0;
  const int* genes = nullptr;
  const int* yenc = nullptr;
  const double* r_eff = nullptr;
  double r_eff_min = 1.0;
  const double* log_ratio = nullptr;
};
struct GivenCells {
  const double* cols = nullptr; long n = 0; int n_cols = 0;
  int chains = 0, n_keep = 0;
  const int* excl = nullptr;
  const double* r_eff = nullptr; double r_eff_min = 1.0;
  const double* log_ratio = nullptr;
};
hipError_t loo_fit_cells(const FitCells& fc, int fields, double* out, size_t scratch_bytes, hipStream_t st);
hipError_t loo_columns(const GivenCells& gc, int fields, double* out, size_t scratch_bytes, hipStream_t st);
hipError_t loo_fit_log_lik(const FitCells& fc, double* out, size_t scratch_bytes, hipStream_t st);
hipError_t loo_predict_fit_cells(const FitCells& fc, double tc, double p_lo, double p_hi, uint32_t k0, double* out,
                                 size_t scratch_bytes, hipStream_t st);
hipError_t loo_predict_columns(const GivenCells& gc, const int* x, const int* y, double p_lo, double p_hi, double* out,
                               size_t scratch_bytes, hipStream_t st);
struct ReffArgs { LooArgs l; int chains = 0, n_keep = 0; };
hipError_t reff_fit_cells(const FitCells& fc, double* out, size_t scratch_bytes, hipStream_t st);
hipError_t reff_columns(const GivenCells& gc, double* out, size_t scratch_bytes, hipStream_t st);
hipError_t launch_xchg_abort_kernel(const XchgArgs& x, hipStream_t st);

}
```

### ppcseq_amd/csrc/ppcx_kernels.hip

```cpp
#include <hip/hip_runtime.h>
#include <hip/hip_ext.h>
#include "ppcx_gene.h"
#include "ppcx_kernels.h"

namespace ppcx {

typedef int __attribute__((may_alias)) word_t;
typedef double2 __attribute__((may_alias)) dpair_t;

#ifndef PPCX_LOGLIK_OCC
#define PPCX_LOGLIK_OCC 2
#endif
#ifndef PPCX_LOGLIK_OCC_FAST
#define PPCX_LOGLIK_OCC_FAST 4
#endif
__device__ __forceinline__ double wave_xor_add_rt(double v, int lane_xor_mask) {
  const int src = (int)((threadIdx.x ^ (unsigned)lane_xor_mask) & 63u) << 2;
  const int lo = __builtin_amdgcn_ds_bpermute(src, __double2loint(v));
  const int hi = __builtin_amdgcn_ds_bpermute(src, __double2hiint(v));
  return v + __hiloint2double(hi, lo);
}
template <int CTRL, int ROW_MASK>
__device__ __forceinline__ double dpp_take(double v) {
  const int lo = __builtin_amdgcn_update_dpp(0, __double2loint(v), CTRL, ROW_MASK, 0xf, true);
  const int hi = __builtin_amdgcn_update_dpp(0, __double2hiint(v), CTRL, ROW_MASK, 0xf, true);
  return __hiloint2double(hi, lo);
}
template <int L>
__device__ __forceinline__ double group_sum(double v) {
  if (L >= 2) v += dpp_take<0xB1, 0xf>(v);
  if (L >= 4) v += dpp_take<0x4E, 0xf>(v);
  if (L >= 8) v += dpp_take<0x141, 0xf>(v);
  if (L >= 16) v += dpp_take<0x140, 0xf>(v);
  if (L >= 32) v = wave_xor_add_rt(v, 16);
  if (L >= 64) v = wave_xor_add_rt(v, 32);
  return v;
}
template <int CM, int LG, int GEN>
__device__ __forceinline__ void loglik_passes(const LoglikArgs& a, const Cmd& c, const VecRef& v, double* sums, int p0, int p1,
                                              const double* stab, const double* swin, const double* sE, const double* sExpo, const double* sX,
                                              int lane, bool any_generic) {
  constexpr int L = 1 << LG, GPW = 64 >> LG;
  const Dims& d = a.d;
  const int sub = lane & (L - 1), gl = lane >> LG;
  int g_cur = a.order[p0 + gl < p1 ? p0 + gl : p1 - 1];
  int g_next = a.order[p0 + GPW + gl < p1 ? p0 + GPW + gl : p1 - 1];
  GenePre pre_cur = gene_pre_load(d, v, a.cd, g_cur);
#ifdef PPCX_TRACE
  unsigned long long* tr = nullptr;
  if (a.trace && lane == 0 && (blockIdx.x % 16) == 0 && blockIdx.x / 16 < kTraceBlocks)
    tr = a.trace + (((long)(blockIdx.x / 16) * 4 + (threadIdx.x >> 6)) * kTracePasses) * kTraceStamps;
  int tpass = 0;
#define PPCX_STAMP(k) do { if (tr && tpass < kTracePasses) tr[tpass * kTraceStamps + (k)] = __builtin_readcyclecounter(); } while (0)
#else
#define PPCX_STAMP(k) ((void)0)
#endif
  for (int p = p0; p < p1; p += GPW) {
    PPCX_STAMP(0);
#ifdef PPCX_TRACE
    if (tr && tpass < kTracePasses) tr[tpass * kTraceStamps + 7] = __builtin_amdgcn_s_memrealtime();
#endif
#ifdef PPCX_PRIO_BALANCE
    {
      const int rem = (p1 - p + GPW - 1) / GPW;
      if (rem >= 4) __builtin_amdgcn_s_setprio(3); else if (rem == 3) __builtin_amdgcn_s_setprio(2); else if (rem == 2) __builtin_amdgcn_s_setprio(1); else __builtin_amdgcn_s_setprio(0);
    }
#endif
    const bool act = p + gl < p1;
    const int g = g_cur;
    const GenePre pre = pre_cur;
    if (p + GPW < p1) {
      g_cur = g_next;
      pre_cur = gene_pre_load(d, v, a.cd, g_next);
      const int pn = p + 2 * GPW + gl;
      g_next = a.order[pn < p1 ? pn : p1 - 1];
    }
    if (CM > 2 && d.x0_is_one && !PPCX_WAVE_ANY(g < d.K)) {
      GeneSumsV<2> o2;
      lane_gene_sums<2, L, 0>(d, c, v, a.cd, g, pre, sub, sE, sExpo, sX, stab, swin, o2);
      o2.lik = group_sum<L>(o2.lik); o2.dph = group_sum<L>(o2.dph); o2.Sr = group_sum<L>(o2.Sr);
      if (act && sub == 0) { const long G = d.G; sums[0 * G + g] = o2.lik; sums[1 * G + g] = o2.dph; sums[2 * G + g] = o2.Sr; }
      continue;
    }
    GeneSumsV<CM> o;
    PPCX_STAMP(1);
#ifdef PPCX_TRACE
    lane_gene_sums<CM, L, GEN>(d, c, v, a.cd, g, pre, sub, sE, sExpo, sX, stab, swin, o, (tr && tpass < kTracePasses) ? tr + tpass * kTraceStamps : nullptr);
#else
    lane_gene_sums<CM, L, GEN>(d, c, v, a.cd, g, pre, sub, sE, sExpo, sX, stab, swin, o);
#endif
    PPCX_STAMP(2);
    const bool with_tx = any_generic && (!d.x0_is_one || PPCX_WAVE_ANY(g < d.K));
    o.lik = group_sum<L>(o.lik); o.dph = group_sum<L>(o.dph); o.Sr = group_sum<L>(o.Sr);
    PPCX_STAMP(3);
    if (with_tx) {
#pragma unroll
      for (int cc = 0; cc < CM; ++cc) if (cc < d.C) o.Tx[cc] = group_sum<L>(o.Tx[cc]);
    }
    if (act && sub == 0) {
      const long G = d.G;
      sums[0 * G + g] = o.lik; sums[1 * G + g] = o.dph; sums[2 * G + g] = o.Sr;
      if (with_tx) {
#pragma unroll
        for (int cc = 0; cc < CM; ++cc) if (cc < d.C) sums[(3 + cc) * G + g] = o.Tx[cc];
      }
    }
    PPCX_STAMP(4);
#ifdef PPCX_TRACE
    ++tpass;
#endif
  }
#undef PPCX_STAMP
}

template <int CM, int GEN, bool PIPE>
__device__ __forceinline__ void loglik_role(const LoglikArgs& a, int jb, int col, double* lds) {
  if (jb >= a.nbpc) return;
  constexpr int NS = GeneSums<CM>::N;
  const Dims& d = a.d;
  const int S = d.S, C = d.C;
  const int tid = threadIdx.x;
  const int wave = tid >> 6, lane = tid & 63;
  static_assert(2 * kLogTabSize == 2 * 256, "one 16-byte request per thread fills the table");
  const bool any_generic = !d.x0_is_one || (C >= 2 && d.K > 0);
  const bool evenS = (S & 1) == 0;
  const int p0 = a.bounds[jb * 4 + wave], p1 = a.bounds[jb * 4 + wave + 1];
  const double2 f_tab = reinterpret_cast<const dpair_t*>(a.logtab)[tid];
  static_assert(2 * kWinTabSize == 4 * 2 * 256, "four 16-byte requests per thread fill the window table");
  double2 f_win[4];
#pragma unroll
  for (int k = 0; k < 4; ++k) f_win[k] = reinterpret_cast<const dpair_t*>(a.wintab)[tid + 256 * k];
  double2 f_e = {0.0, 0.0};
  if (evenS) { if (tid < S / 2) f_e = reinterpret_cast<const dpair_t*>(a.sampleE)[tid]; }
  else if (tid < S) f_e.x = a.sampleE[tid];
  double f_x = 0.0;
  if (GEN != 2 && any_generic && tid < S) f_x = a.X[S + tid];
  const int chain = a.active ? a.active[col] : col;
  const Cmd& c = a.cmds[chain];
  if (c.type == CMD_DONE || c.type == CMD_FLUSH) return;
  if (PIPE) {
    if (c.evaluated && c.type != CMD_LEAF) return;
  }
  double* stab = lds;
  double* swin = lds + 2 * kLogTabSize;
  double* sE = swin + 2 * kWinTabSize;
  double* sExpo = GEN == 2 ? sE + S + kLdsPad : nullptr;
  double* sX = GEN == 2 ? sExpo + S : sE + kLdsPad;
  const VecRef v{a.vecs + (long)chain * V_COUNT * a.Dpad, a.Dpad};
  double* sums = a.sums + (long)chain * NS * d.G;
  reinterpret_cast<dpair_t*>(stab)[tid] = f_tab;
#pragma unroll
  for (int k = 0; k < 4; ++k) reinterpret_cast<dpair_t*>(swin)[tid + 256 * k] = f_win[k];
  if (evenS) {
    if (tid < S / 2) reinterpret_cast<dpair_t*>(sE)[tid] = f_e;
    for (int i = tid + 256; i < S / 2; i += 256) reinterpret_cast<dpair_t*>(sE)[i] = reinterpret_cast<const dpair_t*>(a.sampleE)[i];
  } else {
    if (tid < S) sE[tid] = f_e.x;
    for (int i = tid + 256; i < S; i += 256) sE[i] = a.sampleE[i];
  }
  if (any_generic) {
    if (GEN == 2) {
      for (int i = tid; i < S; i += 256) sExpo[i] = a.exposure[i];
      for (int i = tid; i < S * C; i += 256) sX[i] = a.X[i];
    } else {
      if (tid < S) sX[S + tid] = f_x;
      for (int i = tid + 256; i < S; i += 256) sX[S + i] = a.X[S + i];
      for (int i = 2 * S + tid; i < S * C; i += 256) sX[i] = a.X[i];
    }
  }
  __syncthreads();
  if (p0 >= p1) return;
  switch (a.lgL) {
    case 0: loglik_passes<CM, 0, GEN>(a, c, v, sums, p0, p1, stab, swin, sE, sExpo, sX, lane, any_generic); break;
    case 1: loglik_passes<CM, 1, GEN>(a, c, v, sums, p0, p1, stab, swin, sE, sExpo, sX, lane, any_generic); break;
    case 2: loglik_passes<CM, 2, GEN>(a, c, v, sums, p0, p1, stab, swin, sE, sExpo, sX, lane, any_generic); break;
    case 3: loglik_passes<CM, 3, GEN>(a, c, v, sums, p0, p1, stab, swin, sE, sExpo, sX, lane, any_generic); break;
    case 4: loglik_passes<CM, 4, GEN>(a, c, v, sums, p0, p1, stab, swin, sE, sExpo, sX, lane, any_generic); break;
    case 5: loglik_passes<CM, 5, GEN>(a, c, v, sums, p0, p1, stab, swin, sE, sExpo, sX, lane, any_generic); break;
    default: loglik_passes<CM, 6, GEN>(a, c, v, sums, p0, p1, stab, swin, sE, sExpo, sX, lane, any_generic); break;
  }
}

template <int CM, int GEN>
__global__ __launch_bounds__(256, GEN ? PPCX_LOGLIK_OCC : PPCX_LOGLIK_OCC_FAST) void ppcx_loglik_kernel(LoglikArgs a) {
  extern __shared__ double lds[];
  const int nch = a.nchains;
  const int lin = blockIdx.x, run = lin / (8 * nch), r = lin - run * (8 * nch);
  loglik_role<CM, GEN, false>(a, run * 8 + (r & 7), r >> 3, lds);
}

__device__ __forceinline__ double wave_sum_to_lane63(double v) {
  v += dpp_take<0x111, 0xf>(v);
  v += dpp_take<0x112, 0xf>(v);
  v += dpp_take<0x114, 0xf>(v);
  v += dpp_take<0x118, 0xf>(v);
  v += dpp_take<0x142, 0xa>(v);
  v += dpp_take<0x143, 0xc>(v);
  return v;
}
template <int N>
__device__ __forceinline__ void block_accumulate(double* vals, double* wacc, int wave, int lane) {
#pragma unroll
  for (int k = 0; k < N; ++k) vals[k] = wave_sum_to_lane63(vals[k]);
  if (lane == 63) {
#pragma unroll
    for (int k = 0; k < N; ++k) wacc[wave * PT_COUNT + k] = vals[k];
  }
}

constexpr int kRowStride = 65, kPartStride = 16, kRowsPerWave = 16;
template <int N>
__device__ __forceinline__ void wave_sums_lds(const double* vals, double* rows, double* out , int lane) {
  static_assert(N >= 1 && N <= kRowsPerWave, "one batch");
#pragma unroll
  for (int k = 0; k < N; ++k) rows[k * kRowStride + lane + (kPartStride - 16) * (lane >> 4)] = vals[k];
  __builtin_amdgcn_fence(__ATOMIC_RELEASE, "wavefront");
  __builtin_amdgcn_wave_barrier();
  const int k = lane >> 2, part = lane & 3;
  double t = 0.0;
  if (k < N) {
    const double* r = rows + k * kRowStride + kPartStride * part;
    double b[8];
#pragma unroll
    for (int j = 0; j < 8; ++j) b[j] = r[2 * j + 1] + r[2 * j];
    t = ((b[7] + b[6]) + (b[5] + b[4])) + ((b[3] + b[2]) + (b[1] + b[0]));
  }
  t += dpp_take<0xB1, 0xf>(t);
  t += dpp_take<0x4E, 0xf>(t);
// ... 801 lines not shown
    for (int msk = 1; msk < 64; msk <<= 1) { const int o = __shfl_xor(vmax, msk, 64); vmax = o > vmax ? o : vmax; }
    if ((tid & 63) == 0) s_cnt[tid >> 6] = vmax;
    __syncthreads();
    vmax = s_cnt[0];
#pragma unroll
    for (int w = 1; w < kPpcWaves; ++w) vmax = max(vmax, s_cnt[w]);
    __syncthreads();
    double q[2];
    const double pr[2] = {a.p_lo, a.p_hi};
    for (int k = 0; k < 2; ++k) {
      double h = (double)(n - 1) * pr[k];
      PPCX_OPAQUE(h);
      int lo = (int)floor(h);
      if (lo > n - 1) lo = n - 1;
      if (lo < 0) lo = 0;
      int v0, v1;
      block_select_pair(vals, n, lo, vmax, s_cnt, tid, &v0, &v1);
      q[k] = lo >= n - 1 ? (double)v0 : fma(h - (double)lo, (double)v1 - (double)v0, (double)v0);
    }
    if (tid == 0) {
      double* o = a.ci + (long)cell * 4;
      o[0] = mean; o[1] = sd; o[2] = q[0]; o[3] = q[1];
    }
    __syncthreads();
  }
}

constexpr int kPpcWaveMaxDraws = 4096;
__global__ __launch_bounds__(256) void ppcx_ppc_table_kernel(const double* draws, long n_draws, Dims d, double tc, double* T) {
  __shared__ double tile[32][33];
  const int tx = threadIdx.x & 31, ty = threadIdx.x >> 5;
  const long j0 = (long)blockIdx.x * 32; const int g0 = blockIdx.y * 32;
  const int ncol = d.C + 1;
  for (int c = 0; c < ncol; ++c) {
    for (int r = ty; r < 32; r += 8) {
      const long j = j0 + r; const int g = g0 + tx;
      double v = 0.0;
      if (j < n_draws && g < d.K) {
        const double* u = draws + j * (long)d.D;
        if (c == 0) v = u[d.off_intercept + g];
        else if (c < d.C) v = u[coef_index(d, c, g)];
        else v = exp(-u[d.off_sigma_raw + g]) * tc;
      }
      tile[r][tx] = v;
    }
    __syncthreads();
    for (int r = ty; r < 32; r += 8) {
      const int g = g0 + r; const long j = j0 + tx;
      if (j < n_draws && g < d.K) T[((long)g * ncol + c) * n_draws + j] = tile[tx][r];
    }
    __syncthreads();
  }
}
__device__ __forceinline__ int wave_sum_int(int v) {
#pragma unroll
  for (int msk = 1; msk < 64; msk <<= 1) v += __shfl_xor(v, msk, 64);
  return v;
}
__device__ __forceinline__ int wave_count_le(const int* vals, int n, int v, int lane) {
  int c = 0;
  for (int j = lane; j < n; j += 64) c += vals[j] <= v ? 1 : 0;
  return wave_sum_int(c);
}
__device__ __forceinline__ void wave_select_pair(const int* vals, int n, int r, int vmax, int lane, int* v_r, int* v_r1) {
  int lo = 0, hi = vmax;
  while (lo < hi) {
    const int mid = lo + ((hi - lo) >> 1);
    if (wave_count_le(vals, n, mid, lane) >= r + 1) hi = mid; else lo = mid + 1;
  }
  *v_r = lo;
  int nxt = lo;
  if (r + 1 < n && wave_count_le(vals, n, lo, lane) < r + 2) {
    int mn = 2147483647;
    for (int j = lane; j < n; j += 64) { const int x = vals[j]; mn = (x > lo && x < mn) ? x : mn; }
#pragma unroll
    for (int msk = 1; msk < 64; msk <<= 1) { const int o = __shfl_xor(mn, msk, 64); mn = o < mn ? o : mn; }
    nxt = mn;
  }
  *v_r1 = nxt;
}
__device__ __forceinline__ double wave_sum_double(double v) {
#pragma unroll
  for (int msk = 1; msk < 64; msk <<= 1) v += __shfl_xor(v, msk, 64);
  return v;
}

__global__ __launch_bounds__(256) void ppcx_ppc_wave_kernel(PpcArgs a, const double* T) {
  extern __shared__ int ldsw[];
  const int lane = threadIdx.x & 63, wave = threadIdx.x >> 6;
  const int n = a.n_gen;
  int* vals = ldsw + (long)wave * ((n + 1) & ~1);
  for (int cell = blockIdx.x * 4 + wave; cell < a.n_cells; cell += gridDim.x * 4) {
    double sum = 0.0; int vmax = 0;
    cell_draws(a, T, cell, vals, lane, 64, &sum, &vmax);
    __builtin_amdgcn_fence(__ATOMIC_RELEASE, "wavefront");
    __builtin_amdgcn_wave_barrier();
    const double mean = wave_sum_double(sum) / (double)n;
    double ss = 0.0;
    for (int j = lane; j < n; j += 64) { const double t = (double)vals[j] - mean; ss += t * t; }
    const double sd = n > 1 ? sqrt(wave_sum_double(ss) / (double)(n - 1)) : NAN;
#pragma unroll
    for (int msk = 1; msk < 64; msk <<= 1) { const int o = __shfl_xor(vmax, msk, 64); vmax = o > vmax ? o : vmax; }
    double q[2];
    const double pr[2] = {a.p_lo, a.p_hi};
    for (int k = 0; k < 2; ++k) {
      double h = (double)(n - 1) * pr[k];
      PPCX_OPAQUE(h);
      int lo = (int)floor(h);
      if (lo > n - 1) lo = n - 1;
      if (lo < 0) lo = 0;
      int v0, v1;
      wave_select_pair(vals, n, lo, vmax, lane, &v0, &v1);
      q[k] = lo >= n - 1 ? (double)v0 : fma(h - (double)lo, (double)v1 - (double)v0, (double)v0);
    }
    if (lane == 0) {
      double* o = a.ci + (long)cell * 4;
      o[0] = mean; o[1] = sd; o[2] = q[0]; o[3] = q[1];
    }
    __builtin_amdgcn_wave_barrier();
  }
}

constexpr int kDispThreads = 384;
__global__ __launch_bounds__(kDispThreads) void ppcx_disp_build_kernel(const int* counts, int G, int S, const int* genes, int n_genes,
                                                                        DispFit fit, double* table) {
  extern __shared__ int s_row[];
  const int gi = blockIdx.x;
  if (gi >= n_genes) return;
  const int g = genes ? genes[gi] : gi;
  const int tid = threadIdx.x;
  double* s_val = reinterpret_cast<double*>(s_row + ((S + 1) & ~1));
  for (int s = tid; s < S; s += kDispThreads) s_row[s] = counts[(long)g * S + s];
  __syncthreads();
  constexpr int NN = kDispPanels * kDispN;
  for (int t = tid; t < NN; t += kDispThreads) {
    const int p = t / kDispN, k = t - p * kDispN;
    double lo;
    const double sg = disp_node_sigma(fit, p, k, &lo);
    const DispPoint pt = disp_point(sg, lo);
    double F, D;
    disp_row(s_row, S, 0, 1, pt, &F, &D);
    s_val[(p * 2 + 0) * kDispN + k] = F; s_val[(p * 2 + 1) * kDispN + k] = D;
  }
  __syncthreads();
  for (int t = tid; t < 2 * kDispPanels; t += kDispThreads) {
    double out[kDispStride];
    disp_fit_panel(fit, s_val + t * kDispN, out);
    double* dst = table + (long)g * kDispGeneDoubles + (long)t * kDispStride;
#pragma unroll
    for (int m = 0; m < kDispStride; ++m) dst[m] = out[m];
  }
}

__global__ void ppcx_gather_kernel(const double* draws, long n_rows, int D, const int* cols, int n_cols, double* out) {
  const long i = (long)blockIdx.x * blockDim.x + threadIdx.x;
  if (i >= n_rows * n_cols) return;
  const long r = i / n_cols; const int cidx = (int)(i % n_cols);
  out[i] = draws[r * D + cols[cidx]];
}

__global__ void ppcx_xchg_abort_kernel(XchgArgs x) {
  const int k = threadIdx.x;
  if (k < x.nranks) sys_store(x.flags[k] + xchg_abort_index(x, x.rank), (unsigned long long)x.epoch);
  __threadfence_system();
}

__global__ void ppcx_fill_kernel(double* p, long n, double val) {
  const long i = (long)blockIdx.x * blockDim.x + threadIdx.x;
  if (i < n) p[i] = val;
}

static int loglik_generic_possible(const Dims& d) { return !d.x0_is_one ? 2 : ((d.C >= 2 && d.K > 0 && !d.x1_binary) ? 1 : 0); }
size_t loglik_lds_bytes(const Dims& d) {
  const size_t per_sample = loglik_generic_possible(d) == 2 ? (size_t)(2 + d.C) : (size_t)(d.C < 1 ? 1 : d.C);
  return sizeof(double) * (2 * kLogTabSize + 2 * kWinTabSize + (size_t)d.S * per_sample + 2 * kLdsPad);
}
#define PPCX_BY_CM_GEN(KERNEL, CM, GEN, EXPR)                                                                     \
  do {                                                                                                            \
    if ((CM) <= 2) { if ((GEN) == 0) { auto k_ = KERNEL<2, 0>; EXPR; } else if ((GEN) == 1) { auto k_ = KERNEL<2, 1>; EXPR; } else { auto k_ = KERNEL<2, 2>; EXPR; } } \
    else if ((CM) <= 4) { if ((GEN) == 0) { auto k_ = KERNEL<4, 0>; EXPR; } else if ((GEN) == 1) { auto k_ = KERNEL<4, 1>; EXPR; } else { auto k_ = KERNEL<4, 2>; EXPR; } } \
    else if ((CM) <= 8) { if ((GEN) == 0) { auto k_ = KERNEL<8, 0>; EXPR; } else if ((GEN) == 1) { auto k_ = KERNEL<8, 1>; EXPR; } else { auto k_ = KERNEL<8, 2>; EXPR; } } \
    else { auto k_ = KERNEL<16, 0>; EXPR; }    \
  } while (0)
static const void* loglik_kernel_ptr(int CM, int gen) {
  const void* f = nullptr;
  PPCX_BY_CM_GEN(ppcx_loglik_kernel, CM, gen, f = (const void*)k_);
  return f;
}
int loglik_resident_workgroups_per_cu(int CM, const Dims& d) {
  int n = 0;
  const size_t lds_bytes = loglik_lds_bytes(d);
  const int gen = loglik_generic_possible(d);
  const void* f = loglik_kernel_ptr(CM, gen);
  if (lds_bytes > 64u * 1024u) {
    if (hipFuncSetAttribute(f, hipFuncAttributeMaxDynamicSharedMemorySize, (int)lds_bytes) != hipSuccess) { (void)hipGetLastError(); return 0; }
  }
  hipError_t e = hipSuccess;
  PPCX_BY_CM_GEN(ppcx_loglik_kernel, CM, gen, e = hipOccupancyMaxActiveBlocksPerMultiprocessor(&n, k_, 256, lds_bytes));
  if (e != hipSuccess) { (void)hipGetLastError(); return 0; }
  return n;
}
hipError_t launch_loglik_kernel(int CM, const LoglikArgs& a, hipStream_t st) {
  const size_t lds_bytes = loglik_lds_bytes(a.d);
  const dim3 grid((unsigned)((a.nbpc + 7) / 8 * 8) * (unsigned)a.nchains);
  LoglikArgs args = a;
  void* params[] = {&args};
  return hipLaunchKernel(loglik_kernel_ptr(CM, loglik_generic_possible(a.d)), grid, dim3(256), params, lds_bytes, st);
}
hipError_t launch_close_kernel(int CM, const CloseArgs& a, int nblocks, int nchains, hipStream_t st) {
  const dim3 grid(nblocks, nchains);
  if (CM <= 2) hipLaunchKernelGGL((ppcx_close_kernel<2>), grid, dim3(256), 0, st, a);
  else if (CM <= 4) hipLaunchKernelGGL((ppcx_close_kernel<4>), grid, dim3(256), 0, st, a);
  else if (CM <= 8) hipLaunchKernelGGL((ppcx_close_kernel<8>), grid, dim3(256), 0, st, a);
  else hipLaunchKernelGGL((ppcx_close_kernel<16>), grid, dim3(256), 0, st, a);
  return hipGetLastError();
}
static const void* ls_kernel_ptr(int CM, int gen) {
  const void* f = nullptr;
  PPCX_BY_CM_GEN(ppcx_ls_kernel, CM, gen, f = (const void*)k_);
  return f;
}
static size_t ls_lds_bytes(const Dims& d) { const size_t a = loglik_lds_bytes(d); return a > sizeof(StepShared) ? a : sizeof(StepShared); }
int ls_resident_workgroups_per_cu(int CM, const Dims& d) {
  int n = 0;
  const size_t lds_bytes = ls_lds_bytes(d);
  const int gen = loglik_generic_possible(d);
  if (lds_bytes > 64u * 1024u) {
    if (hipFuncSetAttribute(ls_kernel_ptr(CM, gen), hipFuncAttributeMaxDynamicSharedMemorySize, (int)lds_bytes) != hipSuccess) { (void)hipGetLastError(); return 0; }
  }
  hipError_t e = hipSuccess;
  PPCX_BY_CM_GEN(ppcx_ls_kernel, CM, gen, e = hipOccupancyMaxActiveBlocksPerMultiprocessor(&n, k_, 256, lds_bytes));
  if (e != hipSuccess) { (void)hipGetLastError(); return 0; }
  return n;
}
hipError_t launch_ls_kernel(int CM, const LoglikArgs& a, const StepArgs& sa, int n_srun, int n_chains_total, int spec, hipStream_t st,
                            hipEvent_t ev_start, hipEvent_t ev_stop) {
  const size_t lds_bytes = ls_lds_bytes(a.d);
  int runs = n_srun;
  if (a.nbpc > 7 * n_srun) runs += (a.nbpc - 7 * n_srun + 7) / 8;
  const dim3 grid((unsigned)runs * 8u * (unsigned)a.nchains);
  LoglikArgs args = a; StepArgs sargs = sa;
  void* params[] = {&args, &sargs, &n_srun, &n_chains_total, &spec};
  if (ev_start && ev_stop)
    return hipExtLaunchKernel(ls_kernel_ptr(CM, loglik_generic_possible(a.d)), grid, dim3(256), params, lds_bytes, st, ev_start, ev_stop, 0);
  return hipLaunchKernel(ls_kernel_ptr(CM, loglik_generic_possible(a.d)), grid, dim3(256), params, lds_bytes, st);
}
hipError_t launch_gene_kernel(int CM, const GeneArgs& a, int nblocks, int nchains, hipStream_t st) {
  const dim3 grid(nblocks, nchains);
  if (CM <= 2) hipLaunchKernelGGL((ppcx_gene_kernel<2>), grid, dim3(256), 0, st, a);
  else if (CM <= 4) hipLaunchKernelGGL((ppcx_gene_kernel<4>), grid, dim3(256), 0, st, a);
  else if (CM <= 8) hipLaunchKernelGGL((ppcx_gene_kernel<8>), grid, dim3(256), 0, st, a);
  else hipLaunchKernelGGL((ppcx_gene_kernel<16>), grid, dim3(256), 0, st, a);
  return hipGetLastError();
}
hipError_t launch_step_kernel(const StepArgs& a, int nblocks, int nchains, hipStream_t st) {
  hipLaunchKernelGGL(ppcx_step_kernel, dim3(a.upd_vecs ? nblocks : 1, nchains), dim3(256), 0, st, a);
  return hipGetLastError();
}
hipError_t launch_sum_shards_kernel(const ShardSumArgs& a, hipStream_t st) {
  hipLaunchKernelGGL(ppcx_sum_shards_kernel, dim3((a.n + 255) / 256), dim3(256), 0, st, a);
  return hipGetLastError();
}
hipError_t launch_update_kernel(const UpdateArgs& a, int nblocks, int nchains, hipStream_t st) {
  hipLaunchKernelGGL(ppcx_update_kernel, dim3(nblocks, nchains), dim3(256), 0, st, a);
  return hipGetLastError();
}
hipError_t launch_advi_kernel(const AdviArgs& a, int nblocks, hipStream_t st) {
  hipLaunchKernelGGL(ppcx_advi_kernel, dim3(nblocks), dim3(256), 0, st, a);
  return hipGetLastError();
}
hipError_t launch_advi_elbo_kernel(const AdviElboArgs& a, hipStream_t st) {
  hipLaunchKernelGGL(ppcx_advi_elbo_kernel, dim3(1), dim3(64), 0, st, a);
  return hipGetLastError();
}
hipError_t launch_ppc_kernel(const PpcArgs& a, const double* T, int nblocks, hipStream_t st) {
  hipLaunchKernelGGL(ppcx_ppc_kernel, dim3(nblocks), dim3(kPpcThreads), a.scratch ? 0 : sizeof(int) * (size_t)a.n_gen, st, a, T);
  return hipGetLastError();
}
size_t ppc_wave_lds_bytes(int n_gen) { return sizeof(int) * 4 * (size_t)((n_gen + 1) & ~1); }
int ppc_wave_max_draws() { return kPpcWaveMaxDraws; }
hipError_t launch_ppc_table_kernel(const double* draws, long n_draws, const Dims& d, double tc, double* T, hipStream_t st) {
  const dim3 grid((unsigned)((n_draws + 31) / 32), (unsigned)((d.K + 31) / 32));
  hipLaunchKernelGGL(ppcx_ppc_table_kernel, grid, dim3(256), 0, st, draws, n_draws, d, tc, T);
  return hipGetLastError();
}
hipError_t launch_ppc_wave_kernel(const PpcArgs& a, const double* T, int nblocks, hipStream_t st) {
  const size_t lds = ppc_wave_lds_bytes(a.n_gen);
  if (lds > 64u * 1024u) {
    hipError_t e = hipFuncSetAttribute((const void*)ppcx_ppc_wave_kernel, hipFuncAttributeMaxDynamicSharedMemorySize, (int)lds);
    if (e != hipSuccess) return e;
  }
  hipLaunchKernelGGL(ppcx_ppc_wave_kernel, dim3(nblocks), dim3(256), lds, st, a, T);
  return hipGetLastError();
}
size_t disp_build_lds_bytes(int S) { return sizeof(int) * (size_t)((S + 1) & ~1) + sizeof(double) * 2 * kDispPanels * kDispN; }
hipError_t launch_disp_build_kernel(const int* counts, int G, int S, const int* genes, int n_genes, const DispFit& fit, double* table, hipStream_t st) {
  const size_t lds = disp_build_lds_bytes(S);
  if (lds > 64u * 1024u) {
    hipError_t e = hipFuncSetAttribute((const void*)ppcx_disp_build_kernel, hipFuncAttributeMaxDynamicSharedMemorySize, (int)lds);
    if (e != hipSuccess) return e;
  }
  hipLaunchKernelGGL(ppcx_disp_build_kernel, dim3((unsigned)n_genes), dim3(kDispThreads), lds, st, counts, G, S, genes, n_genes, fit, table);
  return hipGetLastError();
}
hipError_t launch_gather_kernel(const double* draws, long n_rows, int D, const int* cols, int n_cols, double* out, hipStream_t st) {
  const long n = n_rows * n_cols;
  hipLaunchKernelGGL(ppcx_gather_kernel, dim3((unsigned)((n + 255) / 256)), dim3(256), 0, st, draws, n_rows, D, cols, n_cols, out);
  return hipGetLastError();
}
hipError_t launch_xchg_abort_kernel(const XchgArgs& x, hipStream_t st) {
  hipLaunchKernelGGL(ppcx_xchg_abort_kernel, dim3(1), dim3(64), 0, st, x);
  return hipGetLastError();
}
hipError_t launch_fill_kernel(double* p, long n, double val, hipStream_t st) {
  hipLaunchKernelGGL(ppcx_fill_kernel, dim3((unsigned)((n + 255) / 256)), dim3(256), 0, st, p, n, val);
  return hipGetLastError();
}

}
```

### ppcseq_amd/csrc/ppcx_testing.h

```cpp
#ifndef PPCX_TESTING_H
#define PPCX_TESTING_H
#include "../../include/ppcx.h"
#ifdef __cplusplus
extern "C" {
#endif
PPCX_API int ppcx_testing_set(const char* key, long long value);
PPCX_API int ppcx_testing_set_nccl_provider(const char* path);
enum { PPCX_BENCH_LOGLIK = 0, PPCX_BENCH_CLOSE = 1, PPCX_BENCH_LOGLIK_CLOSE = 2, PPCX_BENCH_STEP = 3, PPCX_BENCH_UPDATE = 4,
       PPCX_BENCH_STEP_REDUCE = 5, PPCX_BENCH_STEP_ADVANCE = 6, PPCX_BENCH_STEP_UPDATE = 7,
       PPCX_BENCH_GENE = 8,
       PPCX_BENCH_GENE_NO_PROP = 9,
       PPCX_BENCH_GENE_NO_SPEC = 10,
       PPCX_BENCH_GENE_UPDATE_ONLY = 11,
       PPCX_BENCH_GENE_NEW_TRANSITION = 12 };
PPCX_API int ppcx_testing_bench_kernel(ppcx_model* m, int which, int nchains, int warm_rounds, int reps, int n_merge,
                                       double* ms_per_launch, int* cmd_type);
PPCX_API int ppcx_testing_sm_trace(double* out6);
enum { PPCX_MATH_FAST_RCP = 0, PPCX_MATH_FAST_LOG = 1, PPCX_MATH_FAST_EXP = 2, PPCX_MATH_TABLE_LOG = 3, PPCX_MATH_WINDOW_LOG = 4,
       PPCX_MATH_STIRLING_TAILS = 5, PPCX_MATH_STIRLING_EXCESS = 6, PPCX_MATH_LOG_ERFC_RATIO = 7, PPCX_MATH_CELL = 8,
       PPCX_MATH_CELL_WIN = 9, PPCX_MATH_CELL_Y = 10, PPCX_MATH_CELL_WIN_Y = 11, PPCX_MATH_COUNT = 12 };
PPCX_API int ppcx_testing_eval_math(int fn, int n, const double* a, const double* b, const int* y, double* out0, double* out1);
PPCX_API int ppcx_testing_get_disp_table(ppcx_model* m, double* out);
PPCX_API int ppcx_testing_psis(int n, int n_cols, const double* lr, const double* cols, double* khat);
PPCX_API int ppcx_testing_loo(int n, int n_cols, const double* ll, const int32_t* excluded, const double* r_eff, double* out);
PPCX_API int ppcx_testing_loo_mcse(int n, int n_cols, const double* ll, const int32_t* excluded, const double* r_eff, double* out);
PPCX_API int ppcx_testing_loo_predict(const double* ll, const int32_t* x, int n, int n_cols, const int32_t* y, const int32_t* excluded,
                                      const double* r_eff, double p_lo, double p_hi, double* out);
PPCX_API int ppcx_testing_loo_approx(int n, int n_cols, const double* ll, const double* log_ratio, const int32_t* excluded, double* out);
PPCX_API int ppcx_testing_loo_predict_approx(const double* ll, const double* log_ratio, const int32_t* x, int n, int n_cols,
                                             const int32_t* y, const int32_t* excluded, double p_lo, double p_hi, double* out);
PPCX_API int ppcx_testing_relative_eff(int chains, int n, int n_cols, const double* ll, double* out);
#ifdef __cplusplus
}
#endif
#endif
```

Before: 451.1 ESS/s.

## Replace per-sample sweeps with per-gene polynomial tables for intercept-only genes

Genes without a slope term (positions past the first K in the order) no longer sweep all S samples. Their likelihood, dispersion gradient and rate-gradient sums come from per-gene Chebyshev-style panel tables over the linear predictor, built once at data load. Lanes whose predictor falls outside the tabulated range fall back to the exact sweep through a redo path. The launch planner and pass-cost model now count table passes as cheap units of 64 genes. This trades a much cheaper log-likelihood for added setup cost, extra memory, and approximation error bounded by the table fit.

```diff
diff --git a/ppcseq_amd/_lib.py b/ppcseq_amd/_lib.py
--- a/ppcseq_amd/_lib.py
+++ b/ppcseq_amd/_lib.py
@@ -126,6 +126,8 @@
         lib.ppcx_testing_eval_math.argtypes = [C.c_int, C.c_int, dp, dp, ip, dp, dp]
     if hasattr(lib, "ppcx_testing_get_disp_table"):
         lib.ppcx_testing_get_disp_table.argtypes = [C.c_void_p, dp]
+    if hasattr(lib, "ppcx_testing_get_sample_table"):
+        lib.ppcx_testing_get_sample_table.argtypes = [C.c_void_p, dp, dp, C.POINTER(C.c_int)]
     if hasattr(lib, "ppcx_testing_psis"):
         lib.ppcx_testing_psis.argtypes = [C.c_int, C.c_int, dp, dp, dp]
     if hasattr(lib, "ppcx_testing_loo"):
@@ -410,6 +412,14 @@
         _check(lib.ppcx_testing_get_disp_table(self._h, _p(out, C.c_double)))
         return out
 
+    def testing_sample_table(self):
+        lib = load()
+        if not hasattr(lib, "ppcx_testing_get_sample_table"):
+            raise PpcxError(f"{LIB_PATH} is not the testing build, or one built before ppcx_testing_get_sample_table existed")
+        out = np.zeros((self.G, 32, 4, 12)); centre = np.zeros(self.G); t0 = C.c_int()
+        _check(lib.ppcx_testing_get_sample_table(self._h, _p(out, C.c_double), _p(centre, C.c_double), C.byref(t0)))
+        return out, centre, t0.value
+
     def log_prob_grad(self, u):
         u = np.ascontiguousarray(u, dtype=np.float64)
         one = u.ndim == 1
diff --git a/ppcseq_amd/build.py b/ppcseq_amd/build.py
--- a/ppcseq_amd/build.py
+++ b/ppcseq_amd/build.py
@@ -10,7 +10,7 @@
 TESTING_LIB = os.path.join(os.path.dirname(HERE), "tests", "libppcx_testing.so")
 SOURCES = ["ppcx_kernels.hip", "ppcx_summary.hip", "ppcx_psis.hip", "ppcx_loo.hip", "ppcx_loo_predict.hip", "ppcx_reff.hip", "ppcx_capi.hip"]
 TESTING_SOURCES = ["ppcx_testing_math.hip"]
-HEADERS = ["ppcx_math.h", "ppcx_disp.h", "ppcx_model.h", "ppcx_nuts.h", "ppcx_gene.h", "ppcx_kernels.h", "ppcx_summary.h", "ppcx_summary_dev.h", "ppcx_psis.h", "ppcx_psis_dev.h", "ppcx_loo.h", "ppcx_loo_ap.h", "ppcx_loo_dev.h", "ppcx_loo_predict.h", "ppcx_reff.h", "ppcx_block.h", "ppcx_columns.h", "ppcx_testing.h",
+HEADERS = ["ppcx_math.h", "ppcx_disp.h", "ppcx_sample.h", "ppcx_model.h", "ppcx_nuts.h", "ppcx_gene.h", "ppcx_kernels.h", "ppcx_summary.h", "ppcx_summary_dev.h", "ppcx_psis.h", "ppcx_psis_dev.h", "ppcx_loo.h", "ppcx_loo_ap.h", "ppcx_loo_dev.h", "ppcx_loo_predict.h", "ppcx_reff.h", "ppcx_block.h", "ppcx_columns.h", "ppcx_testing.h",
            os.path.join("..", "..", "include", "ppcx.h")]
 
 
diff --git a/ppcseq_amd/csrc/ppcx_capi.hip b/ppcseq_amd/csrc/ppcx_capi.hip
--- a/ppcseq_amd/csrc/ppcx_capi.hip
+++ b/ppcseq_amd/csrc/ppcx_capi.hip
@@ -70,6 +70,8 @@
   double *d_E = nullptr, *d_expo = nullptr, *d_X = nullptr, *d_Sy = nullptr, *d_SyE = nullptr, *d_SyX = nullptr, *d_SX = nullptr, *d_ncell = nullptr, *d_Lg1 = nullptr;
   double* d_disp = nullptr;
   unsigned char* d_gflags = nullptr;
+  double *d_samp = nullptr, *d_samp_centre = nullptr;
+  int opt_sample_tables = 1, tab_from = 0;
   DispFit fit;
   double *d_logtab = nullptr, *d_wintab = nullptr;
   double e_min = 1.0, e_max = 1.0;
@@ -128,6 +130,14 @@
   const double sweep = (double)((S + L - 1) / L) * (!m->d.x0_is_one ? 2.5 : (slope && !m->d.x1_binary ? lin_w : (slope ? slope_w : 1.0)));
   return 5.8 + sweep;
 }
+constexpr double kTablePassCost = 10.0;
+static int swept_positions(const ppcx_model* m) { return m->d_samp && m->tab_from < m->d.G ? m->tab_from : m->d.G; }
+static int launch_passes(const ppcx_model* m, int L, int* n_sweep = nullptr) {
+  const int gpw = 64 / L, ns = swept_positions(m);
+  const int nsw = (ns + gpw - 1) / gpw;
+  if (n_sweep) *n_sweep = nsw;
+  return nsw + (m->d.G - ns + 63) / 64;
+}
 static int resident_workgroups(const ppcx_model* m, int reserve) {
   int n = m->wgs_override > 0 ? m->wgs_override : m->n_cu * (reserve > 0 ? m->ls_wgs_per_cu : m->wgs_per_cu);
   n -= reserve;
@@ -138,7 +148,7 @@
   int nbpc = n_res / (nch < 1 ? 1 : nch);
   if (nbpc >= 8 && whole_runs) nbpc = nbpc / 8 * 8;
   if (nbpc < 1) nbpc = 1;
-  const int gpw = 64 / L, npass = (m->d.G + gpw - 1) / gpw;
+  const int npass = launch_passes(m, L);
   if (nbpc > (npass + 3) / 4) nbpc = (npass + 3) / 4;
   if (trim) {
     double slack = kTrimSlack;
@@ -168,7 +178,15 @@
     const int gpw = 64 / L;
     const double npass = ceil((double)G / gpw), c_pass = (8.0 + (double)((S + L - 1) / L)) * (L <= 2 ? 1.2 : 1.0);
     const int wpc = 4 * workgroups_per_chain(m, L, nchains, resident_workgroups(m, 0));
-    const double t = ceil(npass / wpc) * c_pass;
+    double t = ceil(npass / wpc) * c_pass;
+    int nsw = 0;
+    const int nall = launch_passes(m, L, &nsw);
+    if (nall > nsw) {
+      const double total = nsw * c_pass + (nall - nsw) * kTablePassCost;
+      const double simd = total * nchains / (4.0 * m->n_cu);
+      const double longest = nsw > 0 ? (c_pass > kTablePassCost ? c_pass : kTablePassCost) : kTablePassCost;
+      t = simd > longest ? simd : longest;
+    }
     if (t < best) { best = t; bestL = L; }
   }
   const int L = m->L_override > 0 ? m->L_override : bestL;
@@ -192,30 +210,35 @@
   auto it = m->plans.find(key);
   if (it != m->plans.end()) { *out = it->second; return PPCX_OK; }
   const int G = m->d.G, L = m->L, gpw = 64 / L;
-  const int nbpc = workgroups_per_chain(m, L, nch, n_res, reserve == 0, trim), wpc = 4 * nbpc, npass = (G + gpw - 1) / gpw;
+  int nsw = 0;
+  const int npass = launch_passes(m, L, &nsw), ns = swept_positions(m);
+  const int nbpc = workgroups_per_chain(m, L, nch, n_res, reserve == 0, trim), wpc = 4 * nbpc;
+  auto start = [&](int k) { const long p = k <= nsw ? (long)k * gpw : (long)ns + (long)(k - nsw) * 64; return (int)(p < G ? p : G); };
   std::vector<double> cost(npass);
   double total = 0;
   for (int k = 0; k < npass; ++k) {
-    const int p = k * gpw;
-    cost[k] = pass_cost(m, L, p, G - p < gpw ? G - p : gpw);
+    const int p = start(k);
+    cost[k] = k < nsw ? pass_cost(m, L, p, ns - p < gpw ? ns - p : gpw) : kTablePassCost;
     total += cost[k];
   }
-  std::vector<int> bounds(wpc + 1, G);
-  bounds[0] = 0;
+  std::vector<int> ub(wpc + 1, npass);
+  ub[0] = 0;
   {
     int k = 0; double cum = 0.0;
     for (int j = 1; j < wpc; ++j) {
       const double target = total * (double)j / (double)wpc;
       while (k < npass && cum + 0.5 * cost[k] < target) cum += cost[k++];
-      bounds[j] = k * gpw < G ? k * gpw : G;
+      ub[j] = k;
     }
   }
   {
-    const long pmax = ((long)(npass + wpc - 1) / wpc) * gpw;
-    for (int j = 0; j < wpc; ++j) if (bounds[j + 1] - bounds[j] > pmax) bounds[j + 1] = (int)(bounds[j] + pmax);
-    bounds[wpc] = G;
-    for (int j = wpc - 1; j >= 0; --j) if (bounds[j + 1] - bounds[j] > pmax) bounds[j] = (int)(bounds[j + 1] - pmax);
-  }
+    const int umax = (npass + wpc - 1) / wpc;
+    for (int j = 0; j < wpc; ++j) if (ub[j + 1] - ub[j] > umax) ub[j + 1] = ub[j] + umax;
+    ub[wpc] = npass;
+    for (int j = wpc - 1; j >= 0; --j) if (ub[j + 1] - ub[j] > umax) ub[j] = ub[j + 1] - umax;
+  }
+  std::vector<int> bounds(wpc + 1, G);
+  for (int j = 0; j <= wpc; ++j) bounds[j] = start(ub[j]);
   ppcx_model::Plan pl; pl.nbpc = nbpc;
   HIPCHK(hipMalloc(&pl.d_bounds, sizeof(int) * (size_t)(wpc + 1)));
   HIPCHK(hipMemcpy(pl.d_bounds, bounds.data(), sizeof(int) * (size_t)(wpc + 1), hipMemcpyHostToDevice));
@@ -275,6 +298,12 @@
     HIPCHK(hipMemcpy(m->d_order, ord.data(), sizeof(int) * (size_t)G, hipMemcpyHostToDevice));
     m->pos_slope.resize(G);
     for (int p = 0; p < G; ++p) m->pos_slope[p] = ord[p] < K && C >= 2;
+    {
+      int ns = 0;
+      while (ns < G && m->pos_slope[ns]) ++ns;
+      const long t0 = ((long)ns + 63) / 64 * 64;
+      m->tab_from = m->d_samp && t0 < G ? (int)t0 : G;
+    }
     drop_plans(m);
   }
   HIPCHK(hipMemcpy(m->d_counts, cnt.data(), sizeof(int32_t) * cnt.size(), hipMemcpyHostToDevice));
@@ -283,6 +312,14 @@
   {
     const hipError_t e = launch_disp_build_kernel(m->d_counts, G, S, nullptr, G, m->fit, m->d_disp, m->stream);
     if (e != hipSuccess) return fail(PPCX_ERR_HIP, std::string("dispersion-table kernel: ") + hipGetErrorString(e));
+  }
+  if (m->d_samp) {
+    std::vector<double> E(S), centre(G);
+    for (int s = 0; s < S; ++s) E[s] = exp(m->expo_host[s]);
+    for (int g = 0; g < G; ++g) centre[g] = samp_centre_row(cnt.data() + (size_t)g * S, E.data(), S);
+    HIPCHK(hipMemcpy(m->d_samp_centre, centre.data(), sizeof(double) * G, hipMemcpyHostToDevice));
+    const hipError_t e = launch_samp_build_kernel(m->d_counts, m->d_E, G, S, m->d_samp_centre, m->fit, m->d_samp, m->stream);
+    if (e != hipSuccess) return fail(PPCX_ERR_HIP, std::string("sample-table kernel: ") + hipGetErrorString(e));
   }
   HIPCHK(hipMemcpy(m->d_Sy, Sy.data(), sizeof(double) * G, hipMemcpyHostToDevice));
   HIPCHK(hipMemcpy(m->d_SyE, SyE.data(), sizeof(double) * G, hipMemcpyHostToDevice));
@@ -336,6 +373,7 @@
   }
   if (const char* e = getenv("PPCX_PIPELINE")) if (atoi(e) == 0) m->opt_pipelined = 0;
   if (const char* e = getenv("PPCX_STREAM_GROUPS")) { const int v = atoi(e); if (v >= 1) m->opt_stream_groups = v; }
+  if (const char* e = getenv("PPCX_SAMPLE_TABLES")) if (atoi(e) == 0) m->opt_sample_tables = 0;
   if (loglik_lds_bytes(m->d) > 160u * 1024u) {
     delete m;
     return fail(PPCX_ERR_LIMIT, "the per-sample constants (S * C doubles; S * (2 + C) for a design without a column of ones) do not fit the 160 KB of LDS of a compute unit beside the 20 KB of tables");
@@ -361,6 +399,15 @@
   MHIP(hipMalloc(&m->d_disp, sizeof(double) * (size_t)G * kDispGeneDoubles));
   MHIP(hipMalloc(&m->d_gflags, (size_t)G));
   disp_fit_init(m->fit);
+  {
+    const int nslope = C >= 2 ? K : 0;
+    const bool dealt = x0 && nslope > 0 && !x1b;
+    if (m->opt_sample_tables && x0 && !dealt && ((long)nslope + 63) / 64 * 64 < G && samp_build_lds_bytes(S) <= 160u * 1024u) {
+      if (hipMalloc(&m->d_samp, sizeof(double) * (size_t)G * kSampGeneDoubles) != hipSuccess) { (void)hipGetLastError(); m->d_samp = nullptr; }
+      else if (hipMalloc(&m->d_samp_centre, sizeof(double) * (size_t)G) != hipSuccess) { (void)hipGetLastError(); (void)hipFree(m->d_samp); m->d_samp = nullptr; m->d_samp_centre = nullptr; }
+      if (m->d_samp) m->d.raw_consts = 1;
+    }
+  }
   MHIP(hipMalloc(&m->d_Lg1, sizeof(double) * G));
   MHIP(hipMalloc(&m->d_logtab, sizeof(double) * 2 * kLogTabSize));
   { double tab[2 * kLogTabSize]; fill_log_table(tab); MHIP(hipMemcpy(m->d_logtab, tab, sizeof(tab), hipMemcpyHostToDevice)); }
@@ -449,7 +496,7 @@
   (void)hipSetDevice(m->device);
   drop_plans(m);
   (void)hipFree(m->d_counts); (void)hipFree(m->d_E); (void)hipFree(m->d_expo); (void)hipFree(m->d_X);
-  (void)hipFree(m->d_Sy); (void)hipFree(m->d_SyE); (void)hipFree(m->d_SyX); (void)hipFree(m->d_SX); (void)hipFree(m->d_ncell); (void)hipFree(m->d_disp); (void)hipFree(m->d_gflags); (void)hipFree(m->d_Lg1); (void)hipFree(m->d_logtab); (void)hipFree(m->d_wintab); (void)hipFree(m->d_order);
+  (void)hipFree(m->d_Sy); (void)hipFree(m->d_SyE); (void)hipFree(m->d_SyX); (void)hipFree(m->d_SX); (void)hipFree(m->d_ncell); (void)hipFree(m->d_disp); (void)hipFree(m->d_samp); (void)hipFree(m->d_samp_centre); (void)hipFree(m->d_gflags); (void)hipFree(m->d_Lg1); (void)hipFree(m->d_logtab); (void)hipFree(m->d_wintab); (void)hipFree(m->d_order);
   if (m->stream) (void)hipStreamDestroy(m->stream);
   delete m;
 }
@@ -568,7 +615,7 @@
   int rc = plan_launch(m, nact, reserve, &pl, w.shared_chip);
   if (rc != PPCX_OK) return rc;
   LoglikArgs& la = *out;
-  la.d = m->d; la.cd.counts = m->d_counts; la.cd.disp = m->d_disp; la.cd.gflags = m->d_gflags; la.cd.Sy = m->d_Sy; la.cd.ncell = m->d_ncell; la.cd.e_min = m->e_min; la.cd.e_max = m->e_max; la.sampleE = m->d_E; la.exposure = m->d_expo; la.X = m->d_X;
+  la.d = m->d; la.cd.counts = m->d_counts; la.cd.disp = m->d_disp; la.cd.gflags = m->d_gflags; la.cd.Sy = m->d_Sy; la.cd.ncell = m->d_ncell; la.cd.e_min = m->e_min; la.cd.e_max = m->e_max; la.cd.samp = m->d_samp; la.cd.samp_centre = m->d_samp_centre; la.tab_from = swept_positions(m); la.sampleE = m->d_E; la.exposure = m->d_expo; la.X = m->d_X;
   la.vecs = w.vecs; la.Dpad = w.Dpad; la.cmds = w.cmds[w.launches & 1]; la.sums = w.sums; la.logtab = m->d_logtab; la.wintab = m->d_wintab; la.order = m->d_order;
   la.lgL = 0; while ((1 << la.lgL) < m->L) ++la.lgL;
   la.nchains = nact; la.active = w.n_active > 0 ? w.active : nullptr; la.nbpc = pl.nbpc; la.bounds = pl.d_bounds;
@@ -922,6 +969,16 @@
   HIPCHK(hipMemcpy(out, m->d_disp, sizeof(double) * (size_t)m->d.G * kDispGeneDoubles, hipMemcpyDeviceToHost));
   return PPCX_OK;
 }
+extern "C" int ppcx_testing_get_sample_table(ppcx_model* m, double* table, double* centre, int* tab_from) {
+  if (!m) return fail(PPCX_ERR_ARG, "bad arguments");
+  if (!m->d_samp) return fail(PPCX_ERR_ARG, "the model has no sample tables");
+  HIPCHK(hipSetDevice(m->device));
+  HIPCHK(hipStreamSynchronize(m->stream));
+  if (table) HIPCHK(hipMemcpy(table, m->d_samp, sizeof(double) * (size_t)m->d.G * kSampGeneDoubles, hipMemcpyDeviceToHost));
+  if (centre) HIPCHK(hipMemcpy(centre, m->d_samp_centre, sizeof(double) * (size_t)m->d.G, hipMemcpyDeviceToHost));
+  if (tab_from) *tab_from = swept_positions(m);
+  return PPCX_OK;
+}
 extern "C" int ppcx_testing_bench_kernel(ppcx_model* m, int which, int nchains, int warm_rounds, int reps, int n_merge,
                                          double* ms_per_launch, int* cmd_type) {
   if (!m || nchains < 1 || reps < 1 || !ms_per_launch || which < 0 || which > PPCX_BENCH_GENE_NEW_TRANSITION) return fail(PPCX_ERR_ARG, "bad arguments");
diff --git a/ppcseq_amd/csrc/ppcx_gene.h b/ppcseq_amd/csrc/ppcx_gene.h
--- a/ppcseq_amd/csrc/ppcx_gene.h
+++ b/ppcseq_amd/csrc/ppcx_gene.h
@@ -1,5 +1,6 @@
 #pragma once
 #include "ppcx_nuts.h"
+#include "ppcx_sample.h"
 
 
 namespace ppcx {
@@ -63,6 +64,8 @@
   const double* Sy;
   const double* ncell;
   double e_min, e_max;
+  const double* samp = nullptr;
+  const double* samp_centre = nullptr;
 };
 
 struct GenePre { double phi, sigma, a0, Sy, n; int flags; };
@@ -73,6 +76,26 @@
   r.a0 = v.at(V_C0, d.off_intercept + g);
   r.Sy = m.Sy[g]; r.n = m.ncell[g]; r.flags = m.gflags[g];
   return r;
+}
+PPCX_HD bool table_gene_sums(const Dims& d, const VecRef& v, const CellData& m, int g, const GenePre& pre, double* lik, double* dph, double* Sr) {
+  const double t = v.at(V_C2, d.off_intercept + g) + pre.sigma;
+  const SampRef sr = samp_ref(t, m.samp_centre[g]);
+  const DispRef dr = disp_ref(pre.sigma);
+  const bool ok = sr.in && dr.in;
+  if (ok) {
+    const double* ps = m.samp + ((long)g * kSampPanels + sr.panel) * kSampPanelDoubles;
+    const double* pd = m.disp + ((long)g * kDispPanels + dr.panel) * 2 * kDispStride;
+    const double P = disp_horner(ps, sr.x), U = disp_horner(ps + kDispStride, sr.x), Q = disp_horner(ps + 2 * kDispStride, sr.x);
+#if defined(__HIP_DEVICE_COMPILE__)
+    __builtin_amdgcn_sched_barrier(0);
+#endif
+    const double R = disp_horner(ps + 3 * kDispStride, sr.x);
+    const double Fh = disp_horner(pd, dr.x), Dh = disp_horner(pd + kDispStride, dr.x);
+    *lik = Fh - fma(pre.phi, P, U);
+    *dph = Dh - P;
+    *Sr = fma(fast_rcp(pre.phi), R, Q);
+  }
+  return ok;
 }
 template <int L> struct DispDeal {
   static constexpr int NL = L >= 8 ? 4 : (L >= 4 ? 2 : 1);
diff --git a/ppcseq_amd/csrc/ppcx_kernels.h b/ppcseq_amd/csrc/ppcx_kernels.h
--- a/ppcseq_amd/csrc/ppcx_kernels.h
+++ b/ppcseq_amd/csrc/ppcx_kernels.h
@@ -23,6 +23,7 @@
   const int* active;
   int nbpc;
   const int* bounds;
+  int tab_from;
 #ifdef PPCX_TRACE
   unsigned long long* trace;
 #endif
@@ -143,6 +144,8 @@
 hipError_t launch_ppc_table_kernel(const double* draws, long n_draws, const Dims& d, double tc, double* T, hipStream_t st);
 hipError_t launch_ppc_wave_kernel(const PpcArgs& a, const double* T, int nblocks, hipStream_t st);
 hipError_t launch_disp_build_kernel(const int* counts, int G, int S, const int* genes, int n_genes, const DispFit& fit, double* table, hipStream_t st);
+hipError_t launch_samp_build_kernel(const int* counts, const double* sampleE, int G, int S, const double* centre, const DispFit& fit, double* table, hipStream_t st);
+size_t samp_build_lds_bytes(int S);
 hipError_t launch_gather_kernel(const double* draws, long n_rows, int D, const int* cols, int n_cols, double* out, hipStream_t st);
 hipError_t launch_fill_kernel(double* p, long n, double val, hipStream_t st);
 
diff --git a/ppcseq_amd/csrc/ppcx_kernels.hip b/ppcseq_amd/csrc/ppcx_kernels.hip
--- a/ppcseq_amd/csrc/ppcx_kernels.hip
+++ b/ppcseq_amd/csrc/ppcx_kernels.hip
@@ -43,9 +43,14 @@
   constexpr int L = 1 << LG, GPW = 64 >> LG;
   const Dims& d = a.d;
   const int sub = lane & (L - 1), gl = lane >> LG;
-  int g_cur = a.order[p0 + gl < p1 ? p0 + gl : p1 - 1];
-  int g_next = a.order[p0 + GPW + gl < p1 ? p0 + GPW + gl : p1 - 1];
-  GenePre pre_cur = gene_pre_load(d, v, a.cd, g_cur);
+  const int ps1 = p1 < a.tab_from ? p1 : a.tab_from;
+  int g_cur = 0, g_next = 0;
+  GenePre pre_cur = GenePre{1.0, 0.0, 1.0, 0.0, 0.0, 0};
+  if (p0 < ps1) {
+    g_cur = a.order[p0 + gl < ps1 ? p0 + gl : ps1 - 1];
+    g_next = a.order[p0 + GPW + gl < ps1 ? p0 + GPW + gl : ps1 - 1];
+    pre_cur = gene_pre_load(d, v, a.cd, g_cur);
+  }
 #ifdef PPCX_TRACE
   unsigned long long* tr = nullptr;
   if (a.trace && lane == 0 && (blockIdx.x % 16) == 0 && blockIdx.x / 16 < kTraceBlocks)
@@ -55,25 +60,52 @@
 #else
 #define PPCX_STAMP(k) ((void)0)
 #endif
-  for (int p = p0; p < p1; p += GPW) {
+  unsigned long long redo = 0; int redo_base = 0;
+  for (int pnext = p0;;) {
+    int p, pend; unsigned long long keep = ~0ull;
+    if (pnext < ps1) { p = pnext; pend = ps1; pnext += GPW; }
+    else {
+      if (redo == 0) {
+        if (pnext >= p1) break;
+        const int pos = pnext + lane;
+        const bool tact = pos < p1;
+        const int tg = a.order[tact ? pos : p1 - 1];
+        const GenePre tpre = gene_pre_load(d, v, a.cd, tg);
+        double t_lik = 0.0, t_dph = 0.0, t_sr = 0.0;
+        const bool ok = table_gene_sums(d, v, a.cd, tg, tpre, &t_lik, &t_dph, &t_sr);
+        if (tact && ok) { const long G = d.G; sums[0 * G + tg] = t_lik; sums[1 * G + tg] = t_dph; sums[2 * G + tg] = t_sr; }
+        redo = __ballot(tact && !ok);
+        redo_base = pnext;
+        pnext += 64;
+        if (redo == 0) continue;
+        PPCX_KEEP_BRANCH();
+      }
+      const int k = (__builtin_ctzll(redo) >> (6 - LG));
+      const unsigned long long gmask = (GPW == 64 ? ~0ull : ((1ull << GPW) - 1ull)) << (k * GPW);
+      keep = (redo & gmask) >> (k * GPW);
+      redo &= ~gmask;
+      p = redo_base + k * GPW; pend = p1;
+      g_cur = a.order[p + gl < p1 ? p + gl : p1 - 1];
+      pre_cur = gene_pre_load(d, v, a.cd, g_cur);
+    }
     PPCX_STAMP(0);
 #ifdef PPCX_TRACE
     if (tr && tpass < kTracePasses) tr[tpass * kTraceStamps + 7] = __builtin_amdgcn_s_memrealtime();
 #endif
 #ifdef PPCX_PRIO_BALANCE
     {
-      const int rem = (p1 - p + GPW - 1) / GPW;
+      const int rem = (pend - p + GPW - 1) / GPW;
       if (rem >= 4) __builtin_amdgcn_s_setprio(3); else if (rem == 3) __builtin_amdgcn_s_setprio(2); else if (rem == 2) __builtin_amdgcn_s_setprio(1); else __builtin_amdgcn_s_setprio(0);
     }
 #endif
-    const bool act = p + gl < p1;
+    const bool act = p + gl < pend && ((keep >> gl) & 1ull) != 0;
     const int g = g_cur;
     const GenePre pre = pre_cur;
-    if (p + GPW < p1) {
+    if (p + GPW < ps1) {
       g_cur = g_next;
       pre_cur = gene_pre_load(d, v, a.cd, g_next);
       const int pn = p + 2 * GPW + gl;
-      g_next = a.order[pn < p1 ? pn : p1 - 1];
+      g_next = a.order[pn < ps1 ? pn : ps1 - 1];
     }
     if (CM > 2 && d.x0_is_one && !PPCX_WAVE_ANY(g < d.K)) {
       GeneSumsV<2> o2;
@@ -1181,6 +1213,38 @@
   }
 }
 
+constexpr int kSampThreads = 384;
+__global__ __launch_bounds__(kSampThreads) void ppcx_samp_build_kernel(const int* counts, const double* sampleE, int G, int S, const double* centre,
+                                                                        DispFit fit, double* table) {
+  extern __shared__ double s_samp[];
+  const int g = blockIdx.x;
+  if (g >= G) return;
+  const int tid = threadIdx.x;
+  constexpr int NN = kSampPanels * kDispN;
+  double* s_E = s_samp;
+  double* s_val = s_E + S;
+  int* s_cnt = reinterpret_cast<int*>(s_val + kSampFn * NN);
+  for (int s = tid; s < S; s += kSampThreads) { s_cnt[s] = counts[(long)g * S + s]; s_E[s] = sampleE[s]; }
+  __syncthreads();
+  const double c = centre[g];
+  for (int t = tid; t < NN; t += kSampThreads) {
+    const int p = t / kDispN, k = t - p * kDispN;
+    double lo, v4[kSampFn];
+    const double tn = samp_node_t(fit, c, p, k, &lo);
+    samp_row(s_cnt, s_E, S, tn, lo, v4);
+#pragma unroll
+    for (int j = 0; j < kSampFn; ++j) s_val[(p * kSampFn + j) * kDispN + k] = v4[j];
+  }
+  __syncthreads();
+  for (int t = tid; t < kSampFn * kSampPanels; t += kSampThreads) {
+    double out[kDispStride];
+    disp_fit_panel(fit, s_val + t * kDispN, out);
+    double* dst = table + (long)g * kSampGeneDoubles + (long)t * kDispStride;
+#pragma unroll
+    for (int m = 0; m < kDispStride; ++m) dst[m] = out[m];
+  }
+}
+
 __global__ void ppcx_gather_kernel(const double* draws, long n_rows, int D, const int* cols, int n_cols, double* out) {
   const long i = (long)blockIdx.x * blockDim.x + threadIdx.x;
   if (i >= n_rows * n_cols) return;
@@ -1332,6 +1396,16 @@
   hipLaunchKernelGGL(ppcx_disp_build_kernel, dim3((unsigned)n_genes), dim3(kDispThreads), lds, st, counts, G, S, genes, n_genes, fit, table);
   return hipGetLastError();
 }
+size_t samp_build_lds_bytes(int S) { return sizeof(double) * ((size_t)S + (size_t)kSampFn * kSampPanels * kDispN) + sizeof(int) * (size_t)S; }
+hipError_t launch_samp_build_kernel(const int* counts, const double* sampleE, int G, int S, const double* centre, const DispFit& fit, double* table, hipStream_t st) {
+  const size_t lds = samp_build_lds_bytes(S);
+  if (lds > 64u * 1024u) {
+    hipError_t e = hipFuncSetAttribute((const void*)ppcx_samp_build_kernel, hipFuncAttributeMaxDynamicSharedMemorySize, (int)lds);
+    if (e != hipSuccess) return e;
+  }
+  hipLaunchKernelGGL(ppcx_samp_build_kernel, dim3((unsigned)G), dim3(kSampThreads), lds, st, counts, sampleE, G, S, centre, fit, table);
+  return hipGetLastError();
+}
 hipError_t launch_gather_kernel(const double* draws, long n_rows, int D, const int* cols, int n_cols, double* out, hipStream_t st) {
   const long n = n_rows * n_cols;
   hipLaunchKernelGGL(ppcx_gather_kernel, dim3((unsigned)((n + 255) / 256)), dim3(256), 0, st, draws, n_rows, D, cols, n_cols, out);
diff --git a/ppcseq_amd/csrc/ppcx_sample.h b/ppcseq_amd/csrc/ppcx_sample.h
--- /dev/null
+++ b/ppcseq_amd/csrc/ppcx_sample.h
@@ -0,0 +1,75 @@
+#pragma once
+#include "ppcx_disp.h"
+
+namespace ppcx {
+
+constexpr int kSampPanels = 32, kSampFn = 4;
+constexpr double kSampWidth = 0.25, kSampInvWidth = 4.0;
+constexpr double kSampHalfRange = 0.5 * kSampPanels * kSampWidth;
+constexpr long kSampPanelDoubles = (long)kSampFn * kDispStride;
+constexpr long kSampGeneDoubles = (long)kSampPanels * kSampPanelDoubles;
+
+inline double samp_centre_row(const int* row, const double* E, int S) {
+  double sy = 0.0, se = 0.0, e2 = 0.0;
+  for (int s = 0; s < S; ++s) if (row[s] >= 0) { sy += (double)row[s]; se += E[s]; e2 += E[s] * E[s]; }
+  if (!(se > 0.0)) return 0.0;
+  const double mu = (sy + 0.5) / se;
+  double res = 0.0;
+  for (int s = 0; s < S; ++s) if (row[s] >= 0) { const double r = (double)row[s] - mu * E[s]; res += r * r; }
+  double inv_phi = (res - mu * se) / (mu * mu * e2);
+  const double lo = 0.049787068367863944, hi = 20.085536923187668;
+  if (!(inv_phi >= lo)) inv_phi = lo;
+  if (inv_phi > hi) inv_phi = hi;
+  const double c = log(mu) + log(inv_phi);
+  if (!(c > -600.0 && c < 600.0)) return 0.0;
+  return floor(c * kSampInvWidth + 0.5) * kSampWidth;
+}
+
+PPCX_HD double samp_node_t(const DispFit& f, double centre, int panel, int k, double* lo) {
+  const double a = fma((double)panel, kSampWidth, centre - kSampHalfRange) + 0.5 * kSampWidth;
+  const double b = 0.5 * kSampWidth * f.xnode[k];
+  const double s = a + b;
+  const double bb = s - a;
+  const double err = (a - (s - bb)) + (b - bb);
+  *lo = err + 0.5 * kSampWidth * f.xnode_lo[k];
+  return s;
+}
+PPCX_HD void samp_row(const int* row, const double* E, int S, double t, double t_lo, double* out4) {
+  const double e0 = fast_exp(t);
+  const double et = fma(t_lo, e0, e0);
+  DispSum p, u, q, r;
+  for (int s = 0; s < S; ++s) {
+    const int y = row[s];
+    if (y < 0) continue;
+    const double yd = (double)y, z = E[s] * et;
+    const double l = log1p_acc(z), w = 1.0 / (1.0 + z);
+    p.add(l); u.add(yd * l); q.add(w); r.add(yd * w);
+  }
+  out4[0] = p.value(); out4[1] = u.value(); out4[2] = q.value(); out4[3] = r.value();
+}
+inline void samp_build_gene_host(const DispFit& f, const int* row, const double* E, int S, double centre, double* out ) {
+  for (int p = 0; p < kSampPanels; ++p) {
+    double fv[kSampFn][kDispN];
+    for (int k = 0; k < kDispN; ++k) {
+      double lo, v4[kSampFn];
+      const double t = samp_node_t(f, centre, p, k, &lo);
+      samp_row(row, E, S, t, lo, v4);
+      for (int j = 0; j < kSampFn; ++j) fv[j][k] = v4[j];
+    }
+    for (int j = 0; j < kSampFn; ++j) disp_fit_panel(f, fv[j], out + ((long)p * kSampFn + j) * kDispStride);
+  }
+}
+
+struct SampRef { int panel; bool in; double x; };
+PPCX_HD SampRef samp_ref(double t, double centre) {
+  SampRef r;
+  const double lo = centre - kSampHalfRange;
+  const double u = (t - lo) * kSampInvWidth;
+  r.in = u >= 0.0 && u < (double)kSampPanels;
+  const int pi = r.in ? (int)u : 0;
+  r.panel = pi;
+  r.x = fma(t - fma((double)pi, kSampWidth, lo), 2.0 * kSampInvWidth, -1.0);
+  return r;
+}
+
+}
diff --git a/ppcseq_amd/csrc/ppcx_testing.h b/ppcseq_amd/csrc/ppcx_testing.h
--- a/ppcseq_amd/csrc/ppcx_testing.h
+++ b/ppcseq_amd/csrc/ppcx_testing.h
@@ -21,6 +21,7 @@
        PPCX_MATH_CELL_WIN = 9, PPCX_MATH_CELL_Y = 10, PPCX_MATH_CELL_WIN_Y = 11, PPCX_MATH_COUNT = 12 };
 PPCX_API int ppcx_testing_eval_math(int fn, int n, const double* a, const double* b, const int* y, double* out0, double* out1);
 PPCX_API int ppcx_testing_get_disp_table(ppcx_model* m, double* out);
+PPCX_API int ppcx_testing_get_sample_table(ppcx_model* m, double* table, double* centre, int* tab_from);
 PPCX_API int ppcx_testing_psis(int n, int n_cols, const double* lr, const double* cols, double* khat);
 PPCX_API int ppcx_testing_loo(int n, int n_cols, const double* ll, const int32_t* excluded, const double* r_eff, double* out);
 PPCX_API int ppcx_testing_loo_mcse(int n, int n_cols, const double* ll, const int32_t* excluded, const double* r_eff, double* out);
```

Measured after the change: 274.6 ESS/s. -39.1%, worse.
